# tudoroancea/ihm2

Measured on AMD Instinct MI355X. Metric: NMPC RTI solves/s (batch), N=40, nx=8 (6-DOF bicycle), fkin6, higher is better.
Workload: dtype f64

## Files before the change

ihm2_amd/csrc/api.hip:

```cpp
#include <hip/hip_runtime.h>

#include <algorithm>
#include <cmath>
#include <cstdarg>
#include <cstdio>
#include <cstdlib>
#include <cstring>
#include <memory>
#include <string>
#include <vector>

#include "ihm2mpc_internal.h"
#include "qp_catalogue.hpp"
#include "sqp_body.hpp"

static thread_local std::string g_err;

int ihm2_fail(const char *fmt, ...)
{
    char buf[512];
    va_list ap;
    va_start(ap, fmt);
    vsnprintf(buf, sizeof buf, fmt, ap);
    va_end(ap);
    g_err = buf;
    return -1;
}

namespace {

#define fail(...) ihm2_fail(__VA_ARGS__)

#define HIP_TRY(expr)                                                                          \
    do {                                                                                       \
        hipError_t e_ = (expr);                                                                \
        if (e_ != hipSuccess) return fail("%s failed: %s (%s:%d)", #expr, hipGetErrorString(e_), __FILE__, __LINE__); \
    } while (0)

#define CHECK_H(h)                                        \
    do {                                                  \
        if (!(h)) return fail("null handle");             \
        HIP_TRY(hipSetDevice((h)->cfg.device));           \
    } while (0)

int alloc_all() { return 0; }

template <typename T, typename... Rest>
int alloc_all(DevBuf<T> &b, size_t n, Rest &&...rest)
{
    HIP_TRY(b.alloc(n));
    if (alloc_all(rest...)) { b.reset(); return -1; }
    return 0;
}

int upload(ihm2mpc_handle *h, const double *host, double *dev, int elems)
{
    HIP_TRY(hipMemcpyAsync(dev, host, (size_t)h->B * elems * sizeof(double), hipMemcpyHostToDevice, h->stream));
    HIP_TRY(hipStreamSynchronize(h->stream));
    return 0;
}

int download(ihm2mpc_handle *h, const double *dev, double *host, int elems)
{
    HIP_TRY(hipMemcpyAsync(host, dev, (size_t)h->B * elems * sizeof(double), hipMemcpyDeviceToHost, h->stream));
    HIP_TRY(hipStreamSynchronize(h->stream));
    return 0;
}

int upload_shared(ihm2mpc_handle *h, const double *host, double *dev, size_t n)
{
    HIP_TRY(hipMemcpyAsync(dev, host, n * sizeof(double), hipMemcpyHostToDevice, h->stream));
    HIP_TRY(hipStreamSynchronize(h->stream));
    return 0;
}

const char *row_name(int c)
{
    static const char *names[NC] = {"lbx/ubx[0]", "lbx/ubx[1]", "lbx/ubx[2]", "lbx/ubx[3]", "lbx/ubx[4]", "lbx/ubx[5]", "lbx/ubx[6]", "lbx/ubx[7]",
                                    "lbu/ubu[0]", "lbu/ubu[1]", "lg/ug[0]", "lg/ug[1]", "lh/uh[0]", "lh/uh[1]"};
    return (c >= 0 && c < NC) ? names[c] : "?";
}

int check_instance_pattern(const ihm2mpc_handle *h, const double *il, const double *iu)
{
    const ihm2::PatternMismatch m = ihm2::find_pattern_mismatch(h->rows, h->B, il, iu);
    if (!m.found) return 0;
    return fail("instance %d, stage %d, row %d (%s): the finite sides (%s, %s) differ from the batch-shared table's (%s, %s)", m.b, m.k, m.c,
                row_name(m.c), m.lower ? "lower" : "-", m.upper ? "upper" : "-", m.shared_lower ? "lower" : "-", m.shared_upper ? "upper" : "-");
}

int scatter_instance_bounds(ihm2mpc_handle *h)
{
    const int B = h->B;
    h->inst_b_ok = false;
    if (check_instance_pattern(h, h->ih_lb.data(), h->ih_ub.data())) return -1;
    const size_t n = h->slots.entries();
    if ((size_t)B * n > h->i_slot_lb.size()) {
        HIP_TRY(hipStreamSynchronize(h->stream));
        h->i_slot_lb.reset(); h->i_slot_ub.reset();
        if (alloc_all(h->i_slot_lb, (size_t)B * n, h->i_slot_ub, (size_t)B * n)) return -1;
    }
    std::vector<double> slb, sub, stl, stu;
    ihm2::scatter_slot_bounds(h->slots, B, h->NS, h->ih_lb.data(), h->ih_ub.data(), slb, sub);
    ihm2::scatter_stage_bounds(h->rows, B, h->ih_lb.data(), h->ih_ub.data(), stl, stu);
    if (n && (upload_shared(h, slb.data(), h->i_slot_lb, slb.size()) || upload_shared(h, sub.data(), h->i_slot_ub, sub.size()))) return -1;
    if (upload_shared(h, stl.data(), h->i_st_lb, stl.size()) || upload_shared(h, stu.data(), h->i_st_ub, stu.size())) return -1;
    h->inst_b_ok = true;
    return 0;
}

const QpTable qp_catalogue[] = {ihm2_qp_set0(), ihm2_qp_set1(), ihm2_qp_set2(), ihm2_qp_set3(), ihm2_qp_set4(), ihm2_qp_set5(), ihm2_qp_set6()};

int path_class(const ihm2mpc_handle *h) { return h->rows.alat_on ? 2 : h->path_on ? 1 : 0; }

const QpInst *find_inst(const QpKey &want)
{
    for (const QpTable &t : qp_catalogue)
        for (const QpInst *e = t.inst; e < t.inst + t.n; e++) {
            const QpKey &k = e->key;
            if (k.kind == want.kind && k.nsoft == want.nsoft && k.path == want.path && k.uni == want.uni && k.sqp == want.sqp &&
                k.irk == want.irk && k.dyn == want.dyn && k.sens == want.sens && k.nf == want.nf && k.nslot >= want.nslot)
                return e;
        }
    return nullptr;
}

int factor_form(const ihm2mpc_handle *h)
{
    static const int limit = [] { const char *e = getenv("IHM2MPC_QP_FORM"); return (e && e[0] == '0') ? 0 : (e && e[0] == '1') ? 1 : 2; }();
    if (limit == 0 || h->cfg.model == IHM2MPC_MODEL_FDYN6 || h->slots.m_act == 0) return 0;
    return (h->N == 40 && limit == 2) ? 40 : -1;
}

const QpInst *find_form(const ihm2mpc_handle *h, QpKey want)
{
    for (int nf = factor_form(h); nf != 0; nf = (nf > 0) ? -1 : 0) {
        want.nf = nf;
        if (const QpInst *e = find_inst(want)) return e;
    }
    want.nf = 0;
    return find_inst(want);
}

ihm2::QpLds qp_layout(const ihm2mpc_handle *h) { return ihm2::qp_lds(h->N, ihm2::qp_lds_class(path_class(h), h->uniform_H && h->uniform_CD)); }
size_t qp_lds_bytes(const ihm2mpc_handle *h) { return sizeof(double) * (size_t)qp_layout(h).total; }
ihm2::StepsLds steps_lds(const ihm2mpc_handle *h, int sens)
{
    const bool dyn_rk4 = h->cfg.model != IHM2MPC_MODEL_FKIN6 && h->cfg.integrator_type == IHM2MPC_INTEG_ERK;
    return ihm2::steps_lds_doubles(qp_layout(h).total, sens ? (int)(ihm2_sens_lds_bytes(h) / sizeof(double)) : 0, dyn_rk4);
}

const QpInst *select_qp(const ihm2mpc_handle *h, size_t lds)
{
    if (lds > 160 * 1024) return nullptr;
    const int uni = h->uniform_H && h->uniform_CD;
    if (h->block_qp && !h->inst_b && h->slots.per_blk >= 1 && h->B <= h->n_cu && h->slots.per_lane * 64 <= (h->N + 1) * 12)
        if (const QpInst *e = find_inst({QP_BLOCK, h->slots.per_blk, h->slots.nsoft, path_class(h), uni, 0, 0, 0})) return e;
    return find_form(h, {QP_WAVE, h->slots.per_lane, h->slots.nsoft, path_class(h), uni, 0, 0, 0});
}

const QpInst *select_steps(const ihm2mpc_handle *h, int sens = 0)
{
    const ihm2::StepsLds lds = steps_lds(h, sens);
    const bool sqp = h->cfg.nlp_solver_type == IHM2MPC_SQP;
    const int irk = ihm2_is_irk(h->cfg.integrator_type) ? 1 : (h->cfg.integrator_type == IHM2MPC_INTEG_ERK_LAG) ? 2 : 0;
    const bool dyn = h->cfg.model != IHM2MPC_MODEL_FKIN6;
    if (irk == 1 && (!h->irk_tab || (sqp && h->sqp_globalization && !h->ls_phi))) return nullptr;
    if (h->cfg.sim_integrator_type == IHM2MPC_INTEG_ERK_LAG && irk != 2) return nullptr;
    if (sqp && !h->ls_x) return nullptr;
    if (lds.total() * sizeof(double) > 160 * 1024) return nullptr;
    if (!lds.guests_fit()) return nullptr;
    if (sqp && !ihm2::qp_sweeps_inside(qp_layout(h), h->N, false, 0, 0)) return nullptr;
    return find_form(h, {QP_STEPS, h->slots.per_lane, h->slots.nsoft, path_class(h), h->uniform_H && h->uniform_CD, sqp, irk, dyn, sens});
}

void note_launch(ihm2mpc_handle *h, const QpKey &k, int per_step = 0)
{
    int32_t *r = h->launch_rec;
    const int form = (k.nf > 0) ? 2 : (k.nf < 0) ? 1 : 0;
    if (k.kind != QP_STEPS) {
        r[0] = k.kind; r[1] = k.nslot; r[2] = k.nsoft; r[3] = k.path; r[4] = k.uni;
        r[15] = (r[15] & ~0x300) | (form << 8);
    } else {
        r[15] = (r[15] & ~0x3000) | ((per_step ? 0 : form) << 12);
        r[5] = per_step ? 2 : 1; r[6] = k.nslot; r[7] = k.nsoft; r[8] = k.path; r[9] = k.uni; r[10] = k.sqp; r[11] = k.irk; r[12] = k.dyn;
        r[13] = per_step; r[14] = k.sens;
    }
}

QpArgs qp_args(ihm2mpc_handle *h)
{
    QpArgs a;
    a.B = h->B; a.N = h->N; a.iter_max = h->cfg.ipm_iter_max; a.nslots = h->slots.per_lane * 64; a.m_act = h->slots.m_act;
    a.nslots_can = h->slots.per_lane * 64;
    a.tol = h->cfg.ipm_tol; a.mu0 = h->cfg.ipm_mu0; a.tau0 = h->cfg.ipm_tau0;
    a.Hs = h->Hs; a.Gy = h->Gy; a.CD = h->CD; a.slot_lb = h->slot_lb; a.slot_ub = h->slot_ub; a.slot_kc = h->slot_kc;
    a.hs_bs = 0; a.hs_te = h->N * 100; a.gy_bs = 0; a.gy_te = h->N * 120; a.sl_bs = 0;
    if (h->inst_w) { a.Hs = h->iHs; a.Gy = h->iGy; a.hs_bs = 200; a.hs_te = 100; a.gy_bs = 240; a.gy_te = 120; }
    if (h->inst_b) { a.sl_bs = h->slots.per_lane * 64; a.slot_lb = h->i_slot_lb; a.slot_ub = h->i_slot_ub; }
    a.x = h->x; a.u = h->u; a.x0 = h->x0; a.yref = h->yref; a.yref_e = h->yref_e;
    a.pi = h->pi; a.lam = h->lam; a.res = h->res; a.qp_res = h->qp_res; a.u0 = h->u0; a.status = h->status; a.qp_iter = h->qp_iter;
    a.lin = h->lin; a.g = h->q_g; a.rg = h->q_rg; a.P = h->q_P; a.M = h->q_M + (size_t)QM_PAD * 64;
    a.slot_zw = h->slot_zw; a.slot_Zw = h->slot_Zw; a.slk = h->slk;
    a.track_id = h->track_id; a.widths = h->widths; a.car_L = h->car_L; a.car_W = h->car_W;
    a.lam_a = h->lam_a; a.slk_a = h->slk_a;
    a.symmetrize = (h->cfg.model == IHM2MPC_MODEL_FDYN6) ? 1 : 0;
    return a;
}

void launch_inst(ihm2mpc_handle *h, const QpInst *e, void **args, size_t lds)
{
    (void)hipFuncSetAttribute(e->kernel, hipFuncAttributeMaxDynamicSharedMemorySize, (int)lds);
    (void)hipLaunchKernel(e->kernel, dim3(h->B), dim3(e->threads), args, lds, h->stream);
    note_launch(h, e->key);
}

int launch_qp(ihm2mpc_handle *h)
{
    const size_t lds = qp_lds_bytes(h);
    const QpInst *e = select_qp(h, lds);
    if (!e) return 1;
    QpArgs a = qp_args(h);
    if (e->key.kind == QP_BLOCK) { a.slot_kc = h->slot_kc_blk; a.slot_lb = h->slot_lb_blk; a.slot_ub = h->slot_ub_blk; a.nslots = h->slots.per_blk * 256; }
    void *args[] = {&a};
    launch_inst(h, e, args, lds);
    return 0;
}

int launch_steps(ihm2mpc_handle *h, int model, int M_sim, double s_target, int n_steps, int freeze, double lap_stop, int sens = 0)
{
    const size_t lds = sizeof(double) * (size_t)steps_lds(h, sens).total();
    const QpInst *e = select_steps(h, sens);
    if (!e) return 1;
    const bool irk_plant = ihm2_is_irk(h->cfg.sim_integrator_type);
    if (irk_plant && ihm2_upload_sim_irk_tab(h, M_sim)) return 1;
    const bool sqp = e->key.sqp;
    QpArgs a = qp_args(h);
    StepArgs s;
    s.ocp_model = h->cfg.model;
    s.n_steps = n_steps; s.model = model; s.M_sim = M_sim; s.M = h->cfg.M; s.nknots = h->cfg.nknots; s.lap_wrap = h->lap_wrap ? 1 : 0;
    s.freeze = freeze; s.s_target = s_target; s.dt = h->cfg.dt; s.lap_stop = lap_stop;
    s.sqp_iters = sqp ? (h->cfg.nlp_solver_max_iter > 0 ? h->cfg.nlp_solver_max_iter : 1) : 0;
    s.s_ref = h->s_ref; s.kappa_ref = h->kappa_ref;
    s.x0 = h->x0; s.yref = h->yref; s.yref_e = h->yref_e; s.lin = h->lin;
    s.active = (freeze || h->active_set) ? h->active.get() : nullptr;
    s.hist_u0 = h->hist_u0; s.hist_x0 = h->hist_x0; s.hist_st = h->hist_st; s.hist_it = h->hist_it;
    s.irk_tab = h->irk_tab;
    s.sim_irk_tab = irk_plant ? h->sim_irk_tab.get() : nullptr;
    s.sens = sens ? (const SensArgs *)h->sens_args.get() : nullptr;
    s.sim_lag = h->cfg.sim_integrator_type == IHM2MPC_INTEG_ERK_LAG;
    std::memset(s.lag, 0, sizeof s.lag);
    if (e->key.irk == 2) {
        const LagFac lo = ihm2_lag_factors(h->cfg.dt / h->cfg.M), lp = ihm2_lag_factors(h->cfg.dt / M_sim);
        std::memcpy(s.lag[0], lo.f, sizeof lo.f); std::memcpy(s.lag[1], lp.f, sizeof lp.f);
    }
    static_assert(sizeof(StepArgs) <= 48 * sizeof(double), "step_args holds 384 bytes");
    static_assert(sizeof(ihm2::LsArgs) <= 64 * sizeof(double), "ls_args holds 512 bytes");
    static_assert(sizeof(SensArgs) <= 64 * sizeof(double), "sens_args holds 512 bytes");
    const int slot = (h->args_idx++) & 1;
    if (hipEventSynchronize(h->args_ev[slot]) != hipSuccess) return 1;
    char *stage = (char *)h->args_host[slot];
    std::memcpy(stage, &s, sizeof(StepArgs));
    if (hipMemcpyAsync(h->step_args, stage, sizeof(StepArgs), hipMemcpyHostToDevice, h->stream) != hipSuccess) return 1;
    if (sqp) {
        ihm2::LsArgs ls_host = ihm2::make_ls_args(h);
        if (e->key.irk) ls_host.phase = 3;
        std::memcpy(stage + 512, &ls_host, sizeof(ihm2::LsArgs));
        if (hipMemcpyAsync(h->ls_args, stage + 512, sizeof(ihm2::LsArgs), hipMemcpyHostToDevice, h->stream) != hipSuccess) return 1;
    }
    if (sens) {
        SensArgs sa;
        ihm2_sens_args(h, &sa);
        sa.hist = h->hist_k; sa.sweep_step = n_steps - 1;
        std::memcpy(stage + 512, &sa, sizeof(SensArgs));
        if (hipMemcpyAsync(h->sens_args, stage + 512, sizeof(SensArgs), hipMemcpyHostToDevice, h->stream) != hipSuccess) return 1;
    }
    if (hipEventRecord(h->args_ev[slot], h->stream) != hipSuccess) return 1;
    const StepArgs *sdev = (const StepArgs *)h->step_args.get();
    const ihm2::LsArgs *ls = (const ihm2::LsArgs *)h->ls_args.get();
    void *args[] = {&sdev, &a, &ls};
    launch_inst(h, e, args, lds);
    return 0;
}

int sens_snapshot(ihm2mpc_handle *h)
{
    if (!h->sens_mode || h->sens_quiet) return 0;
    HIP_TRY(hipMemcpyAsync(h->sens_xbar, h->x, (size_t)h->B * h->NS * NX * sizeof(double), hipMemcpyDeviceToDevice, h->stream));
    HIP_TRY(hipMemcpyAsync(h->sens_ubar, h->u, (size_t)h->B * h->N * NU * sizeof(double), hipMemcpyDeviceToDevice, h->stream));
    return 0;
}

void sens_after_qp(ihm2mpc_handle *h)
{
    if (!h->sens_mode || h->sens_quiet) return;
    ihm2_launch_sens(h);
    h->sens_state = 1;
}

int sens_readable(const ihm2mpc_handle *h)
{
    if (!h->sens_mode) return fail("x0 sensitivities are off: ihm2mpc_set_x0_sensitivities(h, 1 or 2) before the solve");
    if (h->sens_state == 2)
        return fail("the last step came from ihm2mpc_run_steps, which computes no x0 sensitivities (the persistent loop is left as it is): "
                    "call ihm2mpc_run_steps_sens, ihm2mpc_solve, ihm2mpc_compute_control or ihm2mpc_step");
    if (h->sens_state != 1) return fail("no solve has run since x0 sensitivities were set to mode %d: nothing to read yet", h->sens_mode);
    return 0;
}

int ready(ihm2mpc_handle *h)
{
    if (!h->tracks_set) return fail("ihm2mpc_set_tracks has not been called");
    if (!h->weights_set) return fail("ihm2mpc_set_weights has not been called");
    if (!h->bounds_set) return fail("ihm2mpc_set_bounds has not been called");
    if (h->inst_w && !h->uniform_CD) return fail("per-instance weights need stage-independent general rows C, D (the QP keeps one copy of them)");
    if (h->inst_b && !h->inst_b_ok) return fail("the per-instance bounds do not fit the batch-shared constraint pattern any more: set them again, or pass NULL");
    if (!h->slots_fit) {
        std::string hard = "none", soft;
        for (const auto &[S, NSL] : ihm2::slot_limits(path_class(h)))
            if (S == 0) hard = std::to_string(NSL);
            else soft += (soft.empty() ? "" : " or ") + std::to_string(NSL) + " of which " + std::to_string(S) + " soft";
        static const char *rows[3] = {"without track rows", "with track rows", "with track rows and the lateral-acceleration row"};
        return fail("the constraint rows fit no QP kernel: %s a lane of 64 takes at most %s slots when all sides are hard; with soft sides, %s "
                    "(a two-sided hard row is one slot, a row with a soft side two; a lane's one-sided slots lead it)", rows[path_class(h)],
                    hard.c_str(), soft.empty() ? "none" : soft.c_str());
    }
    if (h->rows.alat_on) {
        if (h->cfg.model != IHM2MPC_MODEL_FKIN6) return fail("the lateral-acceleration row is a row of the kinematic model (old/generate_acaods_interface.py:206: `[] if is_dynamic else [a_lat]`)");
        if (!h->path_on) return fail("the lateral-acceleration row comes with the track rows: enable ihm2mpc_set_path_constraints first");
        if (h->cfg.nlp_solver_type != IHM2MPC_SQP_RTI) return fail("the lateral-acceleration row is implemented for SQP_RTI (old/generate.py:21)");
        if (!(h->uniform_H && h->uniform_CD)) return fail("the lateral-acceleration row needs stage-independent weights and general rows (the reference's OCP has them)");
    }
    return 0;
}

struct FieldInfo { double *base; int per_stage; int nstages; };

int field_info(ihm2mpc_handle *h, const char *field, FieldInfo *fi)
{
    const std::string f(field ? field : "");
    if (f == "x") *fi = {h->x, NX, h->NS};
    else if (f == "u") *fi = {h->u, NU, h->N};
    else if (f == "yref") *fi = {h->yref, NY, h->N};
    else if (f == "yref_e") *fi = {h->yref_e, NX, 1};
    else if (f == "pi") *fi = {h->pi, NX, h->NS};
    else if (f == "lam") *fi = {h->lam, NLAM, h->NS};
    else if (f == "lbx" || f == "ubx" || f == "x0") *fi = {h->x0, NX, 1};
    else return fail("unknown field '%s'", f.c_str());
    return 0;
}

}

ihm2mpc_handle::~ihm2mpc_handle()
{
    for (hipStream_t s : {stream, stream2}) if (s) (void)hipStreamSynchronize(s);
    (void)ihm2mpc_comm_free(this);
    for (hipEvent_t e : {ev_fork, ev_join, ev[0], ev[1], ev[2], ev[3], args_ev[0], args_ev[1]}) if (e) (void)hipEventDestroy(e);
    for (void *p : args_host) if (p) (void)hipHostFree(p);
    for (hipStream_t s : {stream, stream2}) if (s) (void)hipStreamDestroy(s);
}

static bool rk4_unstable(double dt, int M) { return dt / M / 1e-3 >= 2.78; }
static int check_sim_substeps(const ihm2mpc_handle *h, int M_sim, const char *lags)
{
    if (M_sim < 1) return fail("M_sim must be >= 1");
    if (h->cfg.sim_integrator_type == IHM2MPC_INTEG_ERK && rk4_unstable(h->cfg.dt, M_sim))
        return fail("RK4 with M_sim = %d sub-steps of dt = %g is unstable on the %s: use M_sim >= %d", M_sim, h->cfg.dt, lags,
                    (int)ceil(h->cfg.dt / (2.78 * 1e-3)));
    return 0;
}
static int check_plant(const ihm2mpc_handle *h, int model, int M_sim)
{
    if (check_sim_substeps(h, M_sim, "actuator lags")) return -1;
    if (model < -2 || model > IHM2MPC_MODEL_FDYN6U) return fail("unknown plant model %d", model);
    if (h->cfg.sim_integrator_type != IHM2MPC_INTEG_ERK_LAG || model == IHM2MPC_MODEL_FKIN6) return 0;
    return fail("the plant integrator ERK_LAG (closed-form actuator lags) is implemented for the kinematic plant (model 0) only, not for plant "
                "model %d: create the handle with another sim_integrator_type", model);
}

extern "C" {

const char *ihm2mpc_last_error(void) { return g_err.c_str(); }
const char *ihm2mpc_version(void) { return "ihm2mpc 0.1 (gfx950)"; }

int ihm2mpc_lag_stage_factors(double h, double tau, double *out4)
{
    if (!out4) return fail("null argument");
    if (!(h > 0.0) || !(tau > 0.0) || !std::isfinite(h) || !std::isfinite(tau)) return fail("h and tau must be positive and finite");
    const double r = h / tau, e = exp(-r);
    double p1, p2;
    if (r < 1.0) {
        p1 = 0.0; p2 = 0.0;
        double t = 0.5;
        for (int k = 2; k < 40; k++) {
            p1 += ((k & 1) ? -1.0 : 1.0) * (k - 1) * t;
            if (k >= 3) p2 += ((k & 1) ? 1.0 : -1.0) * (double)((k - 1) * (k - 2)) * t / r;
            t *= r / (k + 1);
        }
    } else {
        p1 = (1.0 - e * (1.0 + r)) / (r * r);
        p2 = 2.0 * (1.0 - e * (1.0 + r + 0.5 * r * r)) / (r * r * r);
    }
    const double E1 = 6.0 * (p1 - p2), E2 = 12.0 * p2 - 6.0 * p1;
    out4[0] = 6.0 * (-expm1(-r) / r) - 4.0 * E1 - E2;
    out4[1] = E1;
    out4[2] = E2;
    out4[3] = e;
    return 0;
}

int ihm2mpc_create(const ihm2mpc_config *cfg, ihm2mpc_handle **out)
{
    if (!cfg || !out) return fail("null argument");
    if (cfg->batch < 1) return fail("batch must be >= 1");
    if (cfg->N < 2 || cfg->N > IHM2MPC_NMAX) return fail("N must be in [2, %d]", IHM2MPC_NMAX);
    if (cfg->M < 1) return fail("M must be >= 1");
    if (cfg->integrator_type < IHM2MPC_INTEG_ERK || cfg->integrator_type > IHM2MPC_INTEG_ERK_LAG || cfg->sim_integrator_type < IHM2MPC_INTEG_ERK ||
        cfg->sim_integrator_type > IHM2MPC_INTEG_ERK_LAG)
        return fail("unknown integrator type (%d, %d)", cfg->integrator_type, cfg->sim_integrator_type);
    if (cfg->integrator_type == IHM2MPC_INTEG_ERK_LAG && cfg->model != IHM2MPC_MODEL_FKIN6)
        return fail("the integrator ERK_LAG (closed-form actuator lags) is implemented for the kinematic OCP model IHM2MPC_MODEL_FKIN6 only, not for "
                    "the dynamic models (model %d): use ERK or IRK", cfg->model);
    if (cfg->integrator_type == IHM2MPC_INTEG_ERK_LAG && cfg->nlp_solver_type != IHM2MPC_SQP_RTI)
        return fail("the integrator ERK_LAG (closed-form actuator lags) is implemented for IHM2MPC_SQP_RTI only: the SQP mode's line-search "
                    "rollouts have no such integrator; use ERK or IRK");
    if (ihm2_is_irk(cfg->integrator_type) && cfg->M != 1)
        return fail("the IRK integrator of the shooting intervals takes one step per interval (sim_method_num_steps = 1, python/main.py:236); M = %d", cfg->M);
    if (cfg->integrator_type == IHM2MPC_INTEG_ERK && rk4_unstable(cfg->dt, cfg->M))
        return fail("RK4 with %d sub-step(s) of dt = %g is unstable on the actuator lags (t_T = 1e-3 s, t_delta = 0.02 s: |z| = dt / (M t) must stay "
                    "below 2.78): use M >= %d (the reference's sim_method_num_steps = 1 belongs to its IRK integrator, python/main.py:234-236)",
                    cfg->M, cfg->dt, (int)ceil(cfg->dt / (2.78 * 1e-3)));
    if (cfg->model < IHM2MPC_MODEL_FKIN6 || cfg->model > IHM2MPC_MODEL_FDYN6U) return fail("unknown OCP model %d", cfg->model);
    if (cfg->ntracks < 1 || cfg->nknots < 2) return fail("need at least one track table with >= 2 knots");
    if (!(cfg->dt > 0.0)) return fail("dt must be positive");
    int ndev = 0;
    HIP_TRY(hipGetDeviceCount(&ndev));
    if (cfg->device < 0 || cfg->device >= ndev) return fail("device %d out of range (%d devices)", cfg->device, ndev);
    HIP_TRY(hipSetDevice(cfg->device));
    hipDeviceProp_t prop;
    HIP_TRY(hipGetDeviceProperties(&prop, cfg->device));
    if (strncmp(prop.gcnArchName, "gfx950", 6) != 0)
        return fail("libihm2mpc is built for gfx950 (MI355X) only; device %d is %s", cfg->device, prop.gcnArchName);

    auto h = std::make_unique<ihm2mpc_handle>();
    h->cfg = *cfg;
    h->B = cfg->batch;
    h->N = cfg->N;
    h->NS = cfg->N + 1;
    h->n_cu = prop.multiProcessorCount;
    { const char *e = getenv("IHM2MPC_BLOCK_QP"); h->block_qp = !(e && e[0] == '0'); }
    const size_t B = h->B, N = h->N, NS = h->NS, nt = (size_t)cfg->ntracks * cfg->nknots;
    HIP_TRY(hipStreamCreateWithFlags(&h->stream, hipStreamNonBlocking));
    HIP_TRY(hipStreamCreateWithFlags(&h->stream2, hipStreamNonBlocking));
    HIP_TRY(hipEventCreateWithFlags(&h->ev_fork, hipEventDisableTiming));
    HIP_TRY(hipEventCreateWithFlags(&h->ev_join, hipEventDisableTiming));
    for (int i = 0; i < 4; i++) HIP_TRY(hipEventCreate(&h->ev[i]));
    for (int i = 0; i < 2; i++) {
        HIP_TRY(hipHostMalloc(&h->args_host[i], 1024, hipHostMallocDefault));
        HIP_TRY(hipEventCreateWithFlags(&h->args_ev[i], hipEventDisableTiming));
    }
    if (alloc_all(h->s_ref, nt, h->kappa_ref, nt, h->track_id, B, h->Hs, NS * 100, h->Gy, NS * 120, h->lbx, NS * 8, h->ubx, NS * 8,
                  h->lbu, N * 2, h->ubu, N * 2, h->CD, N * 20, h->lg, N * 2, h->ug, N * 2, h->slot_kc_blk, 1024, h->slot_lb_blk, 1024,
                  h->slot_ub_blk, 1024, h->slot_kc, MAX_SLOTS, h->slot_lb, MAX_SLOTS, h->slot_ub, MAX_SLOTS, h->slot_zw, MAX_SLOTS,
                  h->slot_Zw, MAX_SLOTS, h->slk, B * NS * NLAM, h->widths, (size_t)cfg->ntracks * 2, h->lam_a, B * NS * 2, h->slk_a, B * NS * 2,
                  h->X_ref, nt, h->Y_ref, nt, h->phi_ref, nt, h->xc, B * 8, h->s_guess, B, h->step_args, 48, h->Wd, N * 144 + 64,
                  h->st_lb, NS * NC, h->st_ub, NS * NC, h->st_sz, NS * NLAM, h->st_sZ, NS * NLAM, h->x, B * NS * 8, h->u, B * N * 2, h->x0, B * 8,
                  h->yref, B * N * 12, h->yref_e, B * 8, h->pi, B * NS * 8, h->lam, B * NS * NLAM, h->res, B * 4, h->qp_res, B * 4, h->status, B,
                  h->qp_iter, B, h->active, B, h->u0, B * 2,
                  h->lin, (B * N + B) * LIN_REC,
                  h->q_g, B * NS * 10, h->q_rg, B * NS * 10, h->q_P, B * NS * 64, h->q_M, (B * N + 2 * QM_PAD) * 64, h->scratch, B * 24))
        return -1;
    h->slots_fit = true;
    h->sqp_globalization = 0; h->sqp_use_suff = 0; h->sqp_full_step_dual = 0;
    h->sqp_alpha_min = 0.05; h->sqp_alpha_red = 0.7; h->sqp_eps = 1e-4;
    for (int i = 0; i < 4; i++) h->sqp_tol[i] = cfg->nlp_tol;
    h->rows = ihm2::ConstraintRows((int)NS);
    if (ihm2_upload_irk_tab(h.get())) return fail("could not upload the collocation tableau");
    *out = h.release();
    return 0;
}

int ihm2mpc_free(ihm2mpc_handle *h)
{
    if (!h) return 0;
    (void)hipSetDevice(h->cfg.device);
    delete h;
    return 0;
}

int ihm2mpc_synchronize(ihm2mpc_handle *h)
{
    CHECK_H(h);
    HIP_TRY(hipStreamSynchronize(h->stream));
    return 0;
}

int ihm2mpc_get_stream(ihm2mpc_handle *h, void **stream)
{
    CHECK_H(h);
    if (!stream) return fail("null argument");
    *stream = (void *)h->stream;
    return 0;
}

int ihm2mpc_set_tracks(ihm2mpc_handle *h, const double *s_ref, const double *kappa_ref)
{
    CHECK_H(h);
    if (!s_ref || !kappa_ref) return fail("null argument");
    const size_t n = (size_t)h->cfg.ntracks * h->cfg.nknots;
    for (int t = 0; t < h->cfg.ntracks; t++)
        for (int i = 1; i < h->cfg.nknots; i++)
            if (!(s_ref[(size_t)t * h->cfg.nknots + i] > s_ref[(size_t)t * h->cfg.nknots + i - 1]))
                return fail("s_ref of track %d is not strictly increasing at knot %d", t, i);
    if (upload_shared(h, s_ref, h->s_ref, n) || upload_shared(h, kappa_ref, h->kappa_ref, n)) return -1;
    h->tracks_set = true;
    return 0;
}

int ihm2mpc_build_tracks(ihm2mpc_handle *h, int32_t max_seg, const int32_t *nseg, const double *coeffs_X, const double *coeffs_Y)
{
    CHECK_H(h);
    if (!nseg || !coeffs_X || !coeffs_Y) return fail("null argument");
    if (h->cfg.nknots % 3 != 0) return fail("nknots = %d is not three laps of samples", h->cfg.nknots);
    if (max_seg < 2) return fail("max_seg must be >= 2");
    for (int t = 0; t < h->cfg.ntracks; t++)
        if (nseg[t] < 2 || nseg[t] > max_seg) return fail("track %d has %d spline segments (2 .. max_seg = %d)", t, nseg[t], max_seg);
    const size_t nc = (size_t)h->cfg.ntracks * max_seg;
    DevBuf<double> dev;
    DevBuf<int32_t> dseg;
    HIP_TRY(dev.alloc(nc * 9));
    if (dseg.alloc(h->cfg.ntracks) != hipSuccess) return fail("out of device memory");
    double *cX = dev, *cY = dev + nc * 4, *work = dev + nc * 8;
    if (hipMemcpyAsync(cX, coeffs_X, nc * 4 * sizeof(double), hipMemcpyHostToDevice, h->stream) != hipSuccess ||
        hipMemcpyAsync(cY, coeffs_Y, nc * 4 * sizeof(double), hipMemcpyHostToDevice, h->stream) != hipSuccess ||
        hipMemcpyAsync(dseg, nseg, h->cfg.ntracks * sizeof(int32_t), hipMemcpyHostToDevice, h->stream) != hipSuccess) return fail("upload of the spline coefficients failed");
    ihm2_launch_build_tracks(h, max_seg, dseg, cX, cY, work);
    if (hipGetLastError() != hipSuccess || hipStreamSynchronize(h->stream) != hipSuccess) return fail("track-table kernels failed");
    h->tracks_set = true; h->geometry_set = true;
    return 0;
}

int ihm2mpc_fit_tracks(ihm2mpc_handle *h, int32_t max_pts, const int32_t *npts, const double *xy, double curv_weight, double *coeffs_X, double *coeffs_Y)
{
    CHECK_H(h);
    if (!npts || !xy || !coeffs_X || !coeffs_Y) return fail("null argument");
    if (!(curv_weight >= 0.0)) return fail("curv_weight must be >= 0");
    if (max_pts < 3 || 7 * max_pts + 2 > 1280) return fail("max_pts must be in 3 .. 182 (the elimination lists the non-zeros of a row in LDS)");
    const int nt = h->cfg.ntracks;
    for (int t = 0; t < nt; t++)
        if (npts[t] < 3 || npts[t] > max_pts) return fail("track %d has %d centre-line points (3 .. max_pts = %d)", t, npts[t], max_pts);
    const size_t m = 7 * (size_t)max_pts, nwork = (size_t)nt * m * (m + 2), nxy = (size_t)nt * max_pts * 2, nc = (size_t)nt * max_pts * 4;
    DevBuf<double> dev;
    DevBuf<int32_t> di;
    HIP_TRY(dev.alloc(nwork + nxy + 2 * nc));
    if (di.alloc(2 * (size_t)nt) != hipSuccess) return fail("out of device memory");
    double *work = dev, *dxy = dev + nwork, *cX = dxy + nxy, *cY = cX + nc;
    std::vector<int32_t> flags(nt, 1);
    if (hipMemcpyAsync(dxy, xy, nxy * sizeof(double), hipMemcpyHostToDevice, h->stream) != hipSuccess ||
        hipMemcpyAsync(di, npts, nt * sizeof(int32_t), hipMemcpyHostToDevice, h->stream) != hipSuccess) return fail("upload of the centre lines failed");
    ihm2_launch_track_fit(h, max_pts, di, dxy, curv_weight, work, cX, cY, di + nt);
    if (hipGetLastError() != hipSuccess ||
        hipMemcpyAsync(coeffs_X, cX, nc * sizeof(double), hipMemcpyDeviceToHost, h->stream) != hipSuccess ||
        hipMemcpyAsync(coeffs_Y, cY, nc * sizeof(double), hipMemcpyDeviceToHost, h->stream) != hipSuccess ||
        hipMemcpyAsync(flags.data(), di + nt, nt * sizeof(int32_t), hipMemcpyDeviceToHost, h->stream) != hipSuccess ||
        hipStreamSynchronize(h->stream) != hipSuccess) return fail("spline-fit kernel failed");
    for (int t = 0; t < nt; t++)
        if (flags[t]) return fail("the spline fit of track %d is singular (coincident centre-line points?)", t);
    return 0;
}

int ihm2mpc_get_tracks(ihm2mpc_handle *h, double *s_ref, double *kappa_ref, double *X_ref, double *Y_ref, double *phi_ref)
{
    CHECK_H(h);
    if (!h->tracks_set) return fail("no track tables yet");
    const size_t n = (size_t)h->cfg.ntracks * h->cfg.nknots * sizeof(double);
    const double *src[5] = {h->s_ref, h->kappa_ref, h->X_ref, h->Y_ref, h->phi_ref};
    double *dst[5] = {s_ref, kappa_ref, X_ref, Y_ref, phi_ref};
    for (int i = 0; i < 5; i++)
        if (dst[i]) {
            if (i >= 2 && !h->geometry_set) return fail("ihm2mpc_set_track_geometry / ihm2mpc_build_tracks has not been called");
            HIP_TRY(hipMemcpyAsync(dst[i], src[i], n, hipMemcpyDeviceToHost, h->stream));
        }
    HIP_TRY(hipStreamSynchronize(h->stream));
    return 0;
}

int ihm2mpc_set_track_id(ihm2mpc_handle *h, const int32_t *track_id)
{
    CHECK_H(h);
    if (!track_id) return fail("null argument");
    for (int b = 0; b < h->B; b++)
        if (track_id[b] < 0 || track_id[b] >= h->cfg.ntracks) return fail("track_id[%d] = %d out of range", b, track_id[b]);
    HIP_TRY(hipMemcpyAsync(h->track_id, track_id, (size_t)h->B * sizeof(int32_t), hipMemcpyHostToDevice, h->stream));
    HIP_TRY(hipStreamSynchronize(h->stream));
    return 0;
}

int ihm2mpc_set_weights(ihm2mpc_handle *h, const double *W, const double *W_e)
{
    CHECK_H(h);
    if (!W || !W_e) return fail("null argument");
    const int N = h->N, NS = h->NS;
    std::vector<double> Hs((size_t)NS * 100, 0.0), Gy((size_t)NS * 120, 0.0);
    const double cs = h->cfg.cost_scale_stage;
    for (int k = 0; k < N; k++) ihm2::stage_weight_tables(W + (size_t)k * NY * NY, cs, &Hs[(size_t)k * 100], &Gy[(size_t)k * 120]);
    ihm2::terminal_weight_tables(W_e, &Hs[(size_t)N * 100], &Gy[(size_t)N * 120]);
    for (int k = 0; k < NS; k++)
        if (!ihm2::symmetric10(&Hs[(size_t)k * 100])) return fail("weight matrix of stage %d is not symmetric", k);
    const bool uni = ihm2::stages_equal(Hs.data(), N, 100) && ihm2::stages_equal(Gy.data(), N, 120);
    if (upload_shared(h, Hs.data(), h->Hs, Hs.size()) || upload_shared(h, Gy.data(), h->Gy, Gy.size())) return -1;
    if (upload_shared(h, W, h->Wd, (size_t)N * 144) || upload_shared(h, W_e, h->Wd + (size_t)N * 144, 64)) return -1;
    h->shared_uniform_H = uni;
    h->uniform_H = h->inst_w || uni;
    h->weights_set = true;
    return 0;
}

int ihm2mpc_set_instance_weights(ihm2mpc_handle *h, const double *W, const double *W_e)
{
    CHECK_H(h);
    if (!W && !W_e) {
        h->iHs.reset(); h->iGy.reset(); h->iWd.reset();
        h->inst_w = false;
        h->uniform_H = h->shared_uniform_H;
        return 0;
    }
    if (!W || !W_e) return fail("W and W_e must both be given, or both be NULL (batch-shared weights again)");
    if (!h->weights_set) return fail("ihm2mpc_set_weights has not been called (the batch-shared weights come first)");
    if (h->bounds_set && !h->uniform_CD) return fail("per-instance weights need stage-independent general rows C, D");
    const int B = h->B;
    std::vector<double> Hs((size_t)B * 200, 0.0), Gy((size_t)B * 240, 0.0), Wd((size_t)B * 208);
    const double cs = h->cfg.cost_scale_stage;
    for (int b = 0; b < B; b++) {
        const double *Wb = W + (size_t)b * 144, *Web = W_e + (size_t)b * 64;
        for (int i = 0; i < 144; i++) if (Wb[i] != Wb[i]) return fail("instance %d: W[%d][%d] is NaN", b, i / 12, i % 12);
        for (int i = 0; i < 64; i++) if (Web[i] != Web[i]) return fail("instance %d: W_e[%d][%d] is NaN", b, i / 8, i % 8);
        double *Hb = &Hs[(size_t)b * 200], *Gb = &Gy[(size_t)b * 240];
        ihm2::stage_weight_tables(Wb, cs, Hb, Gb);
        ihm2::terminal_weight_tables(Web, Hb + 100, Gb + 120);
        if (!ihm2::symmetric10(Hb)) return fail("instance %d: the weight matrix of the stages 0..%d is not symmetric", b, h->N - 1);
        if (!ihm2::symmetric10(Hb + 100)) return fail("instance %d: the weight matrix of stage %d (terminal) is not symmetric", b, h->N);
        std::memcpy(&Wd[(size_t)b * 208], Wb, 144 * sizeof(double));
        std::memcpy(&Wd[(size_t)b * 208 + 144], Web, 64 * sizeof(double));
    }
    if (!h->iHs && alloc_all(h->iHs, (size_t)B * 200, h->iGy, (size_t)B * 240, h->iWd, (size_t)B * 208)) return -1;
    if (upload_shared(h, Hs.data(), h->iHs, Hs.size()) || upload_shared(h, Gy.data(), h->iGy, Gy.size()) ||
        upload_shared(h, Wd.data(), h->iWd, Wd.size()))
        return -1;
    h->inst_w = true;
    h->uniform_H = true;
    return 0;
}

static int rebuild_slots(ihm2mpc_handle *h)
{
    ihm2::SlotTable t = ihm2::lay_out_slots(h->rows, ihm2::slot_limits(path_class(h)));
    h->slots_fit = t.fit;
    if (!t.fit) return 0;
    h->slots = std::move(t);
    const ihm2::SlotTable &s = h->slots;
    const ihm2::ConstraintRows &r = h->rows;
    if (s.per_blk) {
        HIP_TRY(hipMemcpyAsync(h->slot_kc_blk, s.kc_blk.data(), s.kc_blk.size() * sizeof(int32_t), hipMemcpyHostToDevice, h->stream));
        HIP_TRY(hipStreamSynchronize(h->stream));
        if (upload_shared(h, s.lb_blk.data(), h->slot_lb_blk, s.lb_blk.size()) || upload_shared(h, s.ub_blk.data(), h->slot_ub_blk, s.ub_blk.size())) return -1;
    }
    if (upload_shared(h, r.lb.data(), h->st_lb, r.lb.size()) || upload_shared(h, r.ub.data(), h->st_ub, r.ub.size()) ||
        upload_shared(h, r.sz.data(), h->st_sz, r.sz.size()) || upload_shared(h, r.sZ.data(), h->st_sZ, r.sZ.size()))
        return -1;
    if (const size_t n = s.entries()) {
        HIP_TRY(hipMemcpyAsync(h->slot_kc, s.kc.data(), n * sizeof(int32_t), hipMemcpyHostToDevice, h->stream));
        HIP_TRY(hipStreamSynchronize(h->stream));
        if (upload_shared(h, s.lb.data(), h->slot_lb, n) || upload_shared(h, s.ub.data(), h->slot_ub, n) ||
            upload_shared(h, s.zw.data(), h->slot_zw, n) || upload_shared(h, s.Zw.data(), h->slot_Zw, n))
            return -1;
    }
    if (h->inst_b) return scatter_instance_bounds(h);
    return 0;
}

int ihm2mpc_set_bounds(ihm2mpc_handle *h, const double *lbx, const double *ubx, const double *lbu, const double *ubu,
                       const double *C, const double *D, const double *lg, const double *ug)
{
    CHECK_H(h);
    if (!lbx || !ubx || !lbu || !ubu || !C || !D || !lg || !ug) return fail("null argument");
    const int N = h->N, NS = h->NS;
    for (int i = 0; i < NS * NX; i++) if (lbx[i] > ubx[i]) return fail("lbx > ubx at flat index %d", i);
    for (int i = 0; i < N * NU; i++) if (lbu[i] > ubu[i]) return fail("lbu > ubu at flat index %d", i);
    for (int i = 0; i < N * NG; i++) if (lg[i] > ug[i]) return fail("lg > ug at flat index %d", i);
    std::vector<double> CD((size_t)N * 20);
    for (int k = 0; k < N; k++)
        for (int r = 0; r < NG; r++) {
            for (int j = 0; j < NX; j++) CD[((size_t)k * 2 + r) * 10 + j] = C[((size_t)k * 2 + r) * NX + j];
            for (int j = 0; j < NU; j++) CD[((size_t)k * 2 + r) * 10 + 8 + j] = D[((size_t)k * 2 + r) * NU + j];
        }
    h->uniform_CD = ihm2::stages_equal(CD.data(), N, 20);
    h->rows.set_box_rows(lbx, ubx, lbu, ubu, lg, ug);
    if (rebuild_slots(h)) return -1;
    if (upload_shared(h, lbx, h->lbx, (size_t)NS * 8) || upload_shared(h, ubx, h->ubx, (size_t)NS * 8) ||
        upload_shared(h, lbu, h->lbu, (size_t)N * 2) || upload_shared(h, ubu, h->ubu, (size_t)N * 2) ||
        upload_shared(h, CD.data(), h->CD, CD.size()) || upload_shared(h, lg, h->lg, (size_t)N * 2) ||
        upload_shared(h, ug, h->ug, (size_t)N * 2))
        return -1;
    h->bounds_set = true;
    return 0;
}

int ihm2mpc_set_instance_bounds(ihm2mpc_handle *h, const double *lbx, const double *ubx, const double *lbu, const double *ubu,
                                const double *lg, const double *ug)
{
    CHECK_H(h);
    const bool none = !lbx && !ubx && !lbu && !ubu && !lg && !ug;
    if (none) {
        h->i_slot_lb.reset(); h->i_slot_ub.reset(); h->i_st_lb.reset(); h->i_st_ub.reset();
        h->i_lbu.reset(); h->i_ubu.reset(); h->i_lg.reset(); h->i_ug.reset();
        h->ih_lb = std::vector<double>(); h->ih_ub = std::vector<double>();
        h->inst_b = false; h->inst_b_ok = false;
        return 0;
    }
    if (!lbx || !ubx || !lbu || !ubu || !lg || !ug) return fail("lbx, ubx, lbu, ubu, lg, ug must all be given, or all be NULL (batch-shared bounds again)");
    if (!h->bounds_set) return fail("ihm2mpc_set_bounds has not been called (the batch-shared table gives the pattern)");
    const int B = h->B, N = h->N, NS = h->NS;
    std::vector<double> il((size_t)B * NS * 12), iu((size_t)B * NS * 12);
    for (int b = 0; b < B; b++) {
        const double *xl = lbx + (size_t)b * NS * 8, *xu = ubx + (size_t)b * NS * 8, *ul = lbu + (size_t)b * N * 2, *uu = ubu + (size_t)b * N * 2;
        const double *gl = lg + (size_t)b * N * 2, *gu = ug + (size_t)b * N * 2;
        for (int k = 0; k < NS; k++)
            for (int c = 0; c < 12; c++) {
                const auto [lb, ub] = ihm2::box_row(N, k, c, xl, xu, ul, uu, gl, gu);
                if (lb != lb || ub != ub) return fail("instance %d, stage %d, row %d (%s): bound is NaN", b, k, c, row_name(c));
                if (lb > ub) return fail("instance %d, stage %d, row %d (%s): lower bound %g > upper bound %g", b, k, c, row_name(c), lb, ub);
            }
        ihm2::box_rows(N, xl, xu, ul, uu, gl, gu, &il[(size_t)b * NS * 12], &iu[(size_t)b * NS * 12], 12);
    }
    if (check_instance_pattern(h, il.data(), iu.data())) return -1;
    const size_t nb = (size_t)B;
    if (!h->i_st_lb && alloc_all(h->i_st_lb, nb * NS * NC, h->i_st_ub, nb * NS * NC, h->i_lbu, nb * N * 2, h->i_ubu, nb * N * 2,
                                 h->i_lg, nb * N * 2, h->i_ug, nb * N * 2))
        return -1;
    h->ih_lb = std::move(il); h->ih_ub = std::move(iu);
    if (upload_shared(h, lbu, h->i_lbu, (size_t)B * N * 2) || upload_shared(h, ubu, h->i_ubu, (size_t)B * N * 2) ||
        upload_shared(h, lg, h->i_lg, (size_t)B * N * 2) || upload_shared(h, ug, h->i_ug, (size_t)B * N * 2))
        return -1;
    h->inst_b = true;
    if (scatter_instance_bounds(h)) return -1;
    return 0;
}

int ihm2mpc_set_soft(ihm2mpc_handle *h, const double *soft_z, const double *soft_Z)
{
    CHECK_H(h);
    const int n = h->NS * NLAM;
    if ((soft_z == nullptr) != (soft_Z == nullptr)) return fail("soft_z and soft_Z must both be given or both be NULL");
    for (int i = 0; i < n; i++) {
        const double Z = soft_Z ? soft_Z[i] : -1.0, z = soft_z ? soft_z[i] : 0.0;
        if (Z >= 0.0 && !(z >= 0.0)) return fail("soft_z < 0 at flat index %d (the slack penalty must be non-decreasing)", i);
        if (Z >= 0.0 && !(Z + z > 0.0)) return fail("soft side %d has neither a linear nor a quadratic penalty", i);
        h->rows.sz[i] = z; h->rows.sZ[i] = Z;
    }
    HIP_TRY(hipMemsetAsync(h->slk, 0, (size_t)h->B * h->NS * NLAM * sizeof(double), h->stream));
    if (h->bounds_set && rebuild_slots(h)) return -1;
    return 0;
}

int ihm2mpc_set_path_constraints(ihm2mpc_handle *h, int32_t enable, double car_length, double car_width, const double *widths,
                                 const double *lh, const double *uh)
{
    CHECK_H(h);
    if (enable) {
        if (!widths || !lh || !uh) return fail("null argument");
        if (!(car_length >= 0.0) || !(car_width >= 0.0)) return fail("car_length and car_width must be non-negative");
        for (int i = 0; i < NH; i++) if (lh[i] > uh[i]) return fail("lh > uh at row %d", i);
        for (int t = 0; t < h->cfg.ntracks * 2; t++) if (!(widths[t] > 0.0)) return fail("track width %d is not positive", t);
        if (upload_shared(h, widths, h->widths, (size_t)h->cfg.ntracks * 2)) return -1;
        h->car_L = car_length; h->car_W = car_width;
    }
    h->path_on = enable ? 1 : 0;
    h->rows.set_track_rows(enable != 0, lh, uh);
    if (h->bounds_set && rebuild_slots(h)) return -1;
    return 0;
}

int ihm2mpc_set_alat_constraint(ihm2mpc_handle *h, int32_t enable, double a_lat_min, double a_lat_max, const double *soft_z, const double *soft_Z)
{
    CHECK_H(h);
    if (enable) {
        if (a_lat_min != a_lat_min || a_lat_max != a_lat_max) return fail("a_lat bound is not a number");
        if (a_lat_min > a_lat_max) return fail("a_lat_min > a_lat_max");
        for (int i = 0; i < 2; i++) {
            const double z = soft_z ? soft_z[i] : 0.0, Z = soft_Z ? soft_Z[i] : -1.0;
            if (z != z || Z != Z) return fail("soft penalty of the a_lat row is not a number");
            if (Z >= 0.0 && !(z >= 0.0)) return fail("soft_z < 0 on the a_lat row (the slack penalty must be non-decreasing)");
            if (Z >= 0.0 && !(Z + z > 0.0)) return fail("a soft side of the a_lat row has neither a linear nor a quadratic penalty");
            h->rows.alat_sz[i] = z; h->rows.alat_sZ[i] = Z;
        }
        h->rows.alat_lb = ihm2::bound_or(a_lat_min, -INFINITY);
        h->rows.alat_ub = ihm2::bound_or(a_lat_max, INFINITY);
    }
    h->rows.alat_on = enable ? 1 : 0;
    HIP_TRY(hipMemsetAsync(h->lam_a, 0, (size_t)h->B * h->NS * 2 * sizeof(double), h->stream));
    HIP_TRY(hipMemsetAsync(h->slk_a, 0, (size_t)h->B * h->NS * 2 * sizeof(double), h->stream));
    if (h->bounds_set && rebuild_slots(h)) return -1;
    return 0;
}

int ihm2mpc_set_alat_multipliers(ihm2mpc_handle *h, const double *lam, const double *slk)
{
    CHECK_H(h);
    if (lam) { if (upload(h, lam, h->lam_a, h->NS * 2)) return -1; }
    else HIP_TRY(hipMemsetAsync(h->lam_a, 0, (size_t)h->B * h->NS * 2 * sizeof(double), h->stream));
    if (slk) { if (upload(h, slk, h->slk_a, h->NS * 2)) return -1; }
    else HIP_TRY(hipMemsetAsync(h->slk_a, 0, (size_t)h->B * h->NS * 2 * sizeof(double), h->stream));
    return 0;
}

int ihm2mpc_get_alat_multipliers(ihm2mpc_handle *h, double *lam, double *slk)
{
    CHECK_H(h);
    if (lam && download(h, h->lam_a, lam, h->NS * 2)) return -1;
    if (slk && download(h, h->slk_a, slk, h->NS * 2)) return -1;
    return 0;
}

#define SETTER(name, field, elems)                                   \
    int ihm2mpc_set_##name(ihm2mpc_handle *h, const double *v)       \
    {                                                                \
        CHECK_H(h);                                                  \
        if (!v) return fail("null argument");                        \
        return upload(h, v, h->field, (elems));                      \
    }
SETTER(x0, x0, NX)
SETTER(x, x, h->NS * NX)
SETTER(u, u, h->N * NU)
SETTER(yref, yref, h->N * NY)
SETTER(yref_e, yref_e, NX)
#undef SETTER

int ihm2mpc_set_multipliers(ihm2mpc_handle *h, const double *pi, const double *lam)
{
    CHECK_H(h);
    if (pi) { if (upload(h, pi, h->pi, h->NS * NX)) return -1; }
    else HIP_TRY(hipMemsetAsync(h->pi, 0, (size_t)h->B * h->NS * NX * sizeof(double), h->stream));
    if (lam) { if (upload(h, lam, h->lam, h->NS * NLAM)) return -1; }
    else {
        HIP_TRY(hipMemsetAsync(h->lam, 0, (size_t)h->B * h->NS * NLAM * sizeof(double), h->stream));
        HIP_TRY(hipMemsetAsync(h->lam_a, 0, (size_t)h->B * h->NS * 2 * sizeof(double), h->stream));
    }
    return 0;
}

int ihm2mpc_set_slacks(ihm2mpc_handle *h, const double *sl)
{
    CHECK_H(h);
    if (sl) return upload(h, sl, h->slk, h->NS * NLAM);
    HIP_TRY(hipMemsetAsync(h->slk, 0, (size_t)h->B * h->NS * NLAM * sizeof(double), h->stream));
    HIP_TRY(hipMemsetAsync(h->slk_a, 0, (size_t)h->B * h->NS * 2 * sizeof(double), h->stream));
    return 0;
}

int ihm2mpc_set_stage(ihm2mpc_handle *h, int32_t instance, int32_t stage, const char *field, const double *value, int32_t n)
{
    CHECK_H(h);
    FieldInfo fi;
    if (field_info(h, field, &fi)) return -1;
    if (!value) return fail("null argument");
    if (instance < 0 || instance >= h->B) return fail("instance %d out of range", instance);
    const std::string f(field);
    if ((f == "lbx" || f == "ubx") && stage != 0)
        return fail("per-instance '%s' exists at stage 0 only (the initial state); stage bounds are shared: ihm2mpc_set_bounds", field);
    if (f == "yref_e") stage = 0;
// ... 634 lines not shown
```

ihm2_amd/csrc/ihm2mpc_internal.h:

```cpp
#pragma once

#include <hip/hip_runtime.h>
#include <stdint.h>

#include <vector>

#include "../../include/ihm2mpc.h"
#include "ihm2_dims.h"

#pragma clang fp contract(fast)

#include "qp_tables.hpp"

#define QM_PAD 24
#define LIN_REC 96

static inline bool ihm2_is_irk(int type) { return type == IHM2MPC_INTEG_IRK_GL4 || type == IHM2MPC_INTEG_IRK_RADAU4; }
struct LagFac { double f[8]; };
LagFac ihm2_lag_factors(double h);

struct ihm2mpc_comm;
namespace ihm2 { struct IrkTab; }

template <typename T>
class DevBuf {
public:
    DevBuf() = default;
    DevBuf(const DevBuf &) = delete;
    DevBuf &operator=(const DevBuf &) = delete;
    ~DevBuf() { reset(); }
    hipError_t alloc(size_t n)
    {
        reset();
        void *q = nullptr;
        hipError_t e = hipMalloc(&q, n * sizeof(T));
        if (e == hipSuccess) e = hipMemset(q, 0, n * sizeof(T));
        if (e == hipSuccess) e = hipStreamSynchronize(nullptr);
        if (e != hipSuccess) { (void)hipFree(q); return e; }
        p_ = (T *)q; n_ = n;
        return hipSuccess;
    }
    void reset()
    {
        if (p_) (void)hipFree(p_);
        p_ = nullptr; n_ = 0;
    }
    size_t size() const { return n_; }
    T *get() const { return p_; }
    operator T *() const { return p_; }
private:
    T *p_ = nullptr;
    size_t n_ = 0;
};

struct ihm2mpc_handle {
    ~ihm2mpc_handle();

    ihm2mpc_config cfg;
    ihm2mpc_comm *comm;
    int B, N, NS;
    int n_cu;
    hipStream_t stream;
    hipStream_t stream2;
    hipEvent_t ev_fork, ev_join;
    hipEvent_t ev[4];
    bool tracks_set, weights_set, bounds_set;
    bool uniform_H, uniform_CD;

    DevBuf<double> s_ref, kappa_ref;
    DevBuf<int32_t> track_id;
    DevBuf<double> Hs;
    DevBuf<double> Gy;
    DevBuf<double> lbx, ubx;
    DevBuf<double> lbu, ubu;
    DevBuf<double> CD;
    DevBuf<double> lg, ug;
    ihm2::ConstraintRows rows;
    ihm2::SlotTable slots;
    bool slots_fit;
    DevBuf<int32_t> slot_kc;
    DevBuf<double> slot_lb, slot_ub;
    DevBuf<double> slot_zw, slot_Zw;
    DevBuf<int32_t> slot_kc_blk;
    DevBuf<double> slot_lb_blk, slot_ub_blk;
    bool block_qp;
    int path_on;
    double car_L, car_W, lh[NH], uh[NH];
    DevBuf<double> widths;
    bool geometry_set;
    DevBuf<double> X_ref, Y_ref, phi_ref;
    DevBuf<double> xc;
    DevBuf<double> s_guess;

    DevBuf<double> x;
    DevBuf<double> u;
    DevBuf<double> x0;
    DevBuf<double> yref;
    DevBuf<double> yref_e;
    DevBuf<double> pi;
    DevBuf<double> lam;
    DevBuf<double> slk;
    DevBuf<double> lam_a, slk_a;
    DevBuf<double> res;
    DevBuf<double> ls_phi;
    DevBuf<ihm2::IrkTab> irk_tab;
    DevBuf<ihm2::IrkTab> sim_irk_tab;
    int sim_irk_M;
    DevBuf<double> dyn10;
    DevBuf<double> qp_res;
    DevBuf<int32_t> status, qp_iter;
    DevBuf<int32_t> active;
    bool active_set;
    bool freeze_armed;
    bool lap_wrap;
    DevBuf<double> u0;

    DevBuf<double> lin;
    DevBuf<double> q_g;
    DevBuf<double> q_rg;
    DevBuf<double> q_P;
    DevBuf<double> q_M;
    DevBuf<double> scratch;

    int sqp_globalization, sqp_use_suff, sqp_full_step_dual;
    double sqp_alpha_min, sqp_alpha_red, sqp_eps, sqp_tol[4];
    DevBuf<double> Wd;
    DevBuf<double> st_lb, st_ub;
    DevBuf<double> st_sz, st_sZ;
    DevBuf<double> ls_x, ls_u, ls_pi, ls_lam, ls_slk, ls_wpi, ls_wlam, ls_alpha;
    DevBuf<int32_t> ls_done, ls_status, ls_iter, ls_qp_acc;
    DevBuf<int32_t> ls_pending;
    DevBuf<double> ls_args;
    DevBuf<double> step_args;
    void *args_host[2];
    hipEvent_t args_ev[2];
    int args_idx;

    bool inst_w, inst_b;
    bool inst_b_ok;
    bool shared_uniform_H;
    DevBuf<double> iHs, iGy, iWd;
    std::vector<double> ih_lb, ih_ub;
    DevBuf<double> i_slot_lb, i_slot_ub;
    DevBuf<double> i_st_lb, i_st_ub;
    DevBuf<double> i_lbu, i_ubu, i_lg, i_ug;

    DevBuf<double> hist_u0, hist_x0;
    DevBuf<int32_t> hist_st, hist_it;

    int32_t launch_rec[16];

    int sens_mode;
    int sens_state;
    bool sens_quiet;
    DevBuf<double> sens_xbar, sens_ubar;
    DevBuf<double> sens_u0;
    DevBuf<double> sens_args;
    DevBuf<double> sens_x, sens_u;
    DevBuf<double> hist_k;

    DevBuf<double> adj_sx, adj_su;
    DevBuf<double> adj_gx0, adj_gy, adj_gye;
    DevBuf<double> adj_gW, adj_gWe;
};

void ihm2_launch_prepare(ihm2mpc_handle *h, double s_target, int mode, hipStream_t stream);
void ihm2_launch_build_tracks(ihm2mpc_handle *h, int max_seg, const int32_t *nseg, const double *cX, const double *cY, double *work);
void ihm2_launch_track_fit(ihm2mpc_handle *h, int max_pts, const int32_t *npts, const double *xy, double curv_weight, double *work, double *cX, double *cY,
                           int32_t *fail_flag);
void ihm2_launch_sim_dyn10(ihm2mpc_handle *h, int M, const double *x, const double *u, double *xn, hipStream_t stream);
void ihm2_launch_sim_dyn10_irk(ihm2mpc_handle *h, int integ, int M, int newton_iter, const double *x, const double *u, double *xn, hipStream_t stream);
void ihm2_launch_wrap_lap(ihm2mpc_handle *h);
void ihm2_launch_init_guess(ihm2mpc_handle *h, double v_ref_scale, int only_failed);
void ihm2_launch_linearize(ihm2mpc_handle *h);
void ihm2_launch_linearize_irk(ihm2mpc_handle *h);
int ihm2_upload_sim_irk_tab(ihm2mpc_handle *h, int M_sim);
int ihm2_upload_irk_tab(ihm2mpc_handle *h);
void ihm2_launch_rollout_irk(ihm2mpc_handle *h, int j_begin, int j_end, double *phi, const int32_t *pending);
void ihm2_launch_sim_irk(ihm2mpc_handle *h, int model, int M_sim, const double *x, const double *u, double *xn, hipStream_t stream,
                         const int32_t *active);
void ihm2_launch_copy_iterate(ihm2mpc_handle *h);
void ihm2_launch_line_search(ihm2mpc_handle *h, int it, int last, int phase = 0, int j_limit = 0);
void ihm2_launch_sim(ihm2mpc_handle *h, int model, int M_sim, const double *x, const double *u, double *xn, hipStream_t stream,
                     const int32_t *active);
void ihm2_launch_sim_cart(ihm2mpc_handle *h, int model, int M, double dt, int n_steps, double v_dyn, const double *x, const double *u,
                          double *xn, hipStream_t stream);
void ihm2_launch_project(ihm2mpc_handle *h, double s_tol, const double *xc, double *s_guess, double *xf, hipStream_t stream);
void ihm2_launch_sens(ihm2mpc_handle *h);
size_t ihm2_sens_lds_bytes(const ihm2mpc_handle *h);
void ihm2_launch_adj(ihm2mpc_handle *h, int n_seeds, const double *seed_x, const double *seed_u, int unit_u0, int weights);

namespace {

struct QpArgs {
    int B, N, iter_max, nslots, m_act;
    int nslots_can;
    double tol, mu0, tau0;
    const double *Hs, *Gy, *CD, *slot_lb, *slot_ub, *slot_zw, *slot_Zw;
    const int32_t *slot_kc;
    int hs_bs, hs_te, gy_bs, gy_te, sl_bs;
    double *x, *u;
    const double *x0, *yref, *yref_e;
    double *pi, *lam, *res, *qp_res, *u0;
    int32_t *status, *qp_iter;
    const double *lin;
    double *g, *rg, *P, *M, *slk;
    const int32_t *track_id;
    const double *widths;
    double car_L, car_W;
    double *lam_a, *slk_a;
    int symmetrize;
};

struct SensArgs {
    int B, N, mode, nslots, path, alat;
    double tau;
    const double *Hs;
    int hs_bs, hs_te, hs_ks;
    const double *CD;
    const int32_t *slot_kc;
    const double *slot_lb, *slot_ub, *slot_zw, *slot_Zw;
    int sl_bs;
    const int32_t *track_id;
    const double *widths;
    double car_L, car_W;
    const double *lin, *xbar, *ubar, *x, *u, *lam, *slk, *lam_a, *slk_a;
    const int32_t *status;
    double *sens_u0, *sens_x, *sens_u;
    double *hist;
    int sweep_step;
};

struct StepArgs {
    int n_steps, model, M_sim, M, nknots, lap_wrap, freeze;
    int ocp_model;
    int sqp_iters;
    double s_target, dt, lap_stop;
    const double *s_ref, *kappa_ref;
    double *x0, *yref, *yref_e, *lin;
    int32_t *active;
    double *hist_u0, *hist_x0;
    int32_t *hist_st, *hist_it;
    const ihm2::IrkTab *irk_tab;
    const ihm2::IrkTab *sim_irk_tab;
    const SensArgs *sens;
    double lag[2][8];
    int sim_lag;
};

}

void ihm2_sens_args(const ihm2mpc_handle *h, void *out);

enum { QP_WAVE = 1, QP_BLOCK = 2, QP_STEPS = 3 };
struct QpKey { int kind, nslot, nsoft, path, uni, sqp, irk, dyn, sens, nf; };
struct QpInst { QpKey key; int threads; const void *kernel; };
struct QpTable { const QpInst *inst; int n; };
QpTable ihm2_qp_set0(), ihm2_qp_set1(), ihm2_qp_set2(), ihm2_qp_set3(), ihm2_qp_set4(), ihm2_qp_set5(), ihm2_qp_set6();
```

ihm2_amd/csrc/kernels_qp.hip:

```cpp
#include <cstring>

#include "ihm2mpc_internal.h"
#include "device_steps.hpp"
#include "sqp_body.hpp"
#include "irk_body.hpp"
#include "riccati_mfma.hpp"
#include "sens_body.hpp"
#include "qp_lds.hpp"
#include "qp_catalogue.hpp"
#include "wave_sync.hpp"

using namespace ihm2;

namespace {

#define INF_BOUND 1e20
#ifndef RIC_RING
#define RIC_RING 4
#endif
#ifndef SWEEP_RING
#define SWEEP_RING 4
#endif
#define SWEEP_DL ((SWEEP_RING >= 8) ? 4 : 2)

__device__ __forceinline__ bool fin(double v) { return fabs(v) < INF_BOUND; }

template <typename OP>
__device__ __forceinline__ double wave_reduce(double v, OP op)
{
    v = op(v, dpp_mov<0xB1>(v));
    v = op(v, dpp_mov<0x4E>(v));
    v = op(v, dpp_mov<0x141>(v));
    v = op(v, dpp_mov<0x128>(v));
    int lo = __double2loint(v), hi = __double2hiint(v);
    auto a16 = __builtin_amdgcn_permlane16_swap(lo, lo, false, false);
    auto b16 = __builtin_amdgcn_permlane16_swap(hi, hi, false, false);
    v = op(__hiloint2double(b16[0], a16[0]), __hiloint2double(b16[1], a16[1]));
    lo = __double2loint(v); hi = __double2hiint(v);
    auto a32 = __builtin_amdgcn_permlane32_swap(lo, lo, false, false);
    auto b32 = __builtin_amdgcn_permlane32_swap(hi, hi, false, false);
    return op(__hiloint2double(b32[0], a32[0]), __hiloint2double(b32[1], a32[1]));
}
__device__ __forceinline__ double nanmax(double a, double b) { return (a != a || b != b) ? NAN : fmax(a, b); }
__device__ __forceinline__ double wave_max(double v) { return wave_reduce(v, [](double a, double b) { return fmax(a, b); }); }
__device__ __forceinline__ double wave_min(double v) { return wave_reduce(v, [](double a, double b) { return fmin(a, b); }); }
__device__ __forceinline__ double wave_sum(double v) { return wave_reduce(v, [](double a, double b) { return a + b; }); }
__device__ __forceinline__ double wave_nanmax(double v) { return wave_reduce(v, [](double a, double b) { return nanmax(a, b); }); }

__device__ __forceinline__ double sum8(double v)
{
    v += dpp_mov<0xB1>(v);
    v += dpp_mov<0x4E>(v);
    v += dpp_mov<0x141>(v);
    return v;
}

__device__ __forceinline__ double sum_stride8(double v)
{
    v += dpp_mov<0x128>(v);
    int lo = __double2loint(v), hi = __double2hiint(v);
    auto a16 = __builtin_amdgcn_permlane16_swap(lo, lo, false, false);
    auto b16 = __builtin_amdgcn_permlane16_swap(hi, hi, false, false);
    v = __hiloint2double(b16[0], a16[0]) + __hiloint2double(b16[1], a16[1]);
    lo = __double2loint(v); hi = __double2hiint(v);
    auto a32 = __builtin_amdgcn_permlane32_swap(lo, lo, false, false);
    auto b32 = __builtin_amdgcn_permlane32_swap(hi, hi, false, false);
    return __hiloint2double(b32[0], a32[0]) + __hiloint2double(b32[1], a32[1]);
}

template <int DIR, int D, int DL, bool BUF = true, typename P, typename F>
__device__ __forceinline__ void stream_rows(const double *rows, int N, int e_even, int e_odd, P &&pre, F &&body)
{
    static_assert(D % 2 == 0 && DL % 2 == 0 && D % DL == 0 && 3 * D <= QM_PAD, "the element index alternates with the step parity");
    double r[2][D], x0[DL], x1[DL];
    const __amdgpu_buffer_rsrc_t rsrc = __builtin_amdgcn_make_buffer_rsrc(const_cast<double *>(rows) - (size_t)QM_PAD * 64, 0, (N + 2 * QM_PAD) * 512, 0x00020000);
    const unsigned ve = (unsigned)e_even * 8u, vo = (unsigned)e_odd * 8u;
    typedef unsigned int u2_t __attribute__((ext_vector_type(2)));
    const double *p_even = rows + (size_t)((DIR < 0) ? N - 1 : 0) * 64 + e_even, *p_odd = rows + (size_t)((DIR < 0) ? N - 1 : 0) * 64 + e_odd;
    auto load_row = [&](const int step, const bool odd) -> double {
        if constexpr (BUF) {
            const int row = (DIR < 0) ? N - 1 - step : step;
            const u2_t v = __builtin_amdgcn_raw_buffer_load_b64(rsrc, odd ? vo : ve, (QM_PAD + row) * 512, 0);
            return __hiloint2double((int)v.y, (int)v.x);
        } else
            return (odd ? p_odd : p_even)[(ptrdiff_t)DIR * step * 64];
    };
#pragma unroll
    for (int d = 0; d < D; d++) {
        r[0][d] = load_row(d, (d & 1) != 0);
        __builtin_amdgcn_sched_barrier(0);
        if (d < DL) pre((DIR < 0) ? N - 1 - d : d, (d & 1) != 0, x0[d], x1[d]);
    }
    for (int s0 = 0; s0 < N; s0 += 2 * D) {
#pragma unroll
        for (int h = 0; h < 2; h++) {
#pragma unroll
            for (int d = 0; d < D; d++) {
                const int s = s0 + h * D + d;
                const int k = (DIR < 0) ? N - 1 - s : s;
                const double v = r[h][d], y0 = x0[d % DL], y1 = x1[d % DL];
                r[h ^ 1][d] = load_row(s + D, (d & 1) != 0);
                pre((DIR < 0) ? k - DL : k + DL, (d & 1) != 0, x0[d % DL], x1[d % DL]);
                if (s < N) body(k, v, (d & 1) != 0, y0, y1);
            }
        }
    }
}
template <int DIR, int D, int DL, typename P, typename F>
__device__ __forceinline__ void stream_rows_v1(const double *rows, int N, int e_even, int e_odd, P &&pre, F &&body)
{
    stream_rows<DIR, D, DL, false>(rows, N, e_even, e_odd, pre, body);
}

template <int NSLOT, int NSOFT, int PATH, int UNI, int NW = 1, int LEAN = 1, int NF = 0>
__device__ __forceinline__ void qp_wave_body(const QpArgs &a, const int b, double *sm, const bool want_res = true)
{
    static_assert(NF == 0 || NW == 1, "the straight-line factor sweep parks its idle lanes' stores in the tile the block reductions use");
    constexpr int NT = 64 * NW;
    const int tid = threadIdx.x, lane = tid & 63, wv = tid >> 6;
#define BSYNC() do { if (NW == 1) WSYNC(); else __syncthreads(); } while (0)
    const int N = (NF > 0) ? NF : a.N, NS = N + 1;
    constexpr QpLdsClass CLS = qp_lds_class(PATH, UNI != 0);
    constexpr int NCK = CLS.nck;
    const double *Hs0 = a.Hs + (size_t)b * a.hs_bs, *HsT = Hs0 + a.hs_te;
    const double *Gy0 = a.Gy + (size_t)b * a.gy_bs, *GyT = Gy0 + a.gy_te;
    const double *slot_lbb = a.slot_lb + (size_t)b * a.sl_bs, *slot_ubb = a.slot_ub + (size_t)b * a.sl_bs;
    constexpr bool ALAT = PATH == 2;
    constexpr bool HL = CLS.hl, CL = CLS.cl;
    static_assert(qp_factor_inside(qp_lds(40, CLS), 40, NCK) && qp_factor_inside(qp_lds(2, CLS), 2, NCK), "factor stage / block reductions leave their LDS");
    static_assert(qp_sweeps_inside(qp_lds(40, CLS), 40, LEAN != 0, SWEEP_RING, SWEEP_DL) && (LEAN == 0 || qp_sweeps_inside(qp_lds(2, CLS), 2, true, SWEEP_RING, SWEEP_DL)),
                  "the sweeps' unclamped LDS prefetch leaves the block (the earlier form does below N = 4: api.hip refuses those launches)");
    static_assert(NW <= 4, "qp_factor_inside checks the block reductions for four waves");
#define LEN(id) qp_lds_len(id, N, NS, CLS)
    double *z = sm, *gt = z + LEN(QP_Z), *pi = gt + LEN(QP_GT), *pv = pi + LEN(QP_PI), *rb = pv + LEN(QP_PV), *gam = rb + LEN(QP_RB), *cf = gam + LEN(QP_GAM), *dz = cf + LEN(QP_CF);
    double *kff = dz + LEN(QP_DZ), *Kl = kff + LEN(QP_KFF), *Ginv = Kl + LEN(QP_KL), *Prb = Ginv + LEN(QP_GINV), *tile = Prb + LEN(QP_PRB), *hc = tile + LEN(QP_TILE), *ha = hc + LEN(QP_HC);
    double *Hl = ha + LEN(QP_HA), *CDl = Hl + LEN(QP_HL), *spv = CDl + LEN(QP_CDL);
    int *spc = reinterpret_cast<int *>(spv + 60);
#undef LEN
#define HS(k, i, l) (HL ? Hl[(((k) == N) ? 100 : 0) + (i) * 10 + (l)] : ((k) == N ? HsT : Hs0 + (UNI ? 0 : (k)) * 100)[(i) * 10 + (l)])
#define CDV(k, r, j) (CL ? CDl[(r) * 10 + (j)] : a.CD[((k) * 2 + (r)) * 10 + (j)])

    auto blk_reduce = [&](double v, auto op) -> double {
        v = wave_reduce(v, op);
        if (NW > 1) {
            __syncthreads();
            if (lane == 0) tile[wv] = v;
            __syncthreads();
            v = tile[0];
#pragma unroll
            for (int w = 1; w < NW; w++) v = op(v, tile[w]);
        }
        return v;
    };
    auto blk_max = [&](double v) { return blk_reduce(v, [](double x, double y) { return fmax(x, y); }); };
    auto blk_min = [&](double v) { return blk_reduce(v, [](double x, double y) { return fmin(x, y); }); };
    auto blk_sum = [&](double v) { return blk_reduce(v, [](double x, double y) { return x + y; }); };
    auto blk_nanmax = [&](double v) { return blk_reduce(v, [](double x, double y) { return nanmax(x, y); }); };

    const double *xb = a.x + (size_t)b * NS * 8;
    const double *ub = a.u + (size_t)b * N * 2;
    const double *linb = a.lin + (size_t)b * N * LIN_REC;
    double *gb = a.g + (size_t)b * NS * 10;
    double *rgb = a.rg + (size_t)b * NS * 10;
    double *Pg = a.P + (size_t)b * NS * 64;
    double *Mg = a.M + (size_t)b * N * 64;
    double *pib = a.pi + (size_t)b * NS * 8;
    double *lamb = a.lam + (size_t)b * NS * 28;
    double *slkb = a.slk + (size_t)b * NS * 28;
    double *lamab = ALAT ? a.lam_a + (size_t)b * NS * 2 : nullptr;
    double *slkab = ALAT ? a.slk_a + (size_t)b * NS * 2 : nullptr;
    auto alat_slot = [](int j) -> int { return (j == 3) ? 0 : (j == 4) ? 1 : (j == 6) ? 2 : (j == 7) ? 3 : -1; };

    if (HL) for (int e = tid; e < 200; e += NT) Hl[e] = (e < 100) ? Hs0[e] : HsT[e - 100];
    if (CL && tid < 20) CDl[tid] = a.CD[tid];
    if (UNI) BSYNC();
    bool h_sparse = false;
    if (HL) {
        int cnt = 0;
        if (tid < 20) {
#pragma unroll
            for (int l = 0; l < 10; l++) {
                const double v = Hl[tid * 10 + l];
                if (v != 0.0) { if (cnt < 3) { spv[tid * 3 + cnt] = v; spc[tid * 3 + cnt] = l; } cnt++; }
            }
            for (int q = cnt; q < 3; q++) { spv[tid * 3 + q] = 0.0; spc[tid * 3 + q] = 0; }
        }
        h_sparse = __ballot(cnt > 3) == 0ull;
        if (NW > 1) h_sparse = blk_max((wv == 0 && !h_sparse) ? 1.0 : 0.0) == 0.0;
        BSYNC();
    }
    double sg = 1.0, sb = 1.0, r_stat = 0.0, r_eq = 0.0;
    double w_R = 0.0, w_L = 0.0;
    if (PATH) {
        const int trk = a.track_id[b];
        w_R = a.widths[trk * 2 + 0]; w_L = a.widths[trk * 2 + 1];
        for (int k = tid; k < NS; k += NT) {
            const double psi = xb[k * 8 + 2], sgn = (psi > 0.0) - (psi < 0.0);
            const double dfoot = -0.5 * a.car_L * cos(fabs(psi)) * sgn, dlat = -0.5 * a.car_W * sin(psi);
            hc[k * 2 + 0] = (k >= 1) ? dfoot + dlat : 0.0;
            hc[k * 2 + 1] = (k >= 1) ? -dfoot + dlat : 0.0;
            if (ALAT) {
                double g4[4];
                alat_eval(xb[k * 8 + 3], xb[k * 8 + 4], xb[k * 8 + 6], xb[k * 8 + 7], g4);
#pragma unroll
                for (int q = 0; q < 4; q++) ha[k * 4 + q] = (k >= 1 && k < N) ? g4[q] : 0.0;
            }
        }
        BSYNC();
    }
    for (int e = tid; e < NS * 10; e += NT) {
        const int k = e / 10, j = e % 10;
        double acc = 0.0;
#pragma unroll
        for (int l = 0; l < 8; l++) acc = fma(HS(k, j, l), xb[k * 8 + l], acc);
        if (k < N) {
            acc = fma(HS(k, j, 8), ub[k * 2 + 0], acc);
            acc = fma(HS(k, j, 9), ub[k * 2 + 1], acc);
            const double *yr = a.yref + ((size_t)b * N + k) * 12;
#pragma unroll
            for (int l = 0; l < 12; l++) acc = fma(-Gy0[((UNI ? 0 : k) * 10 + j) * 12 + l], yr[l], acc);
        } else {
            const double *yr = a.yref_e + (size_t)b * 8;
#pragma unroll
            for (int l = 0; l < 8; l++) acc = fma(-GyT[j * 12 + l], yr[l], acc);
        }
        gb[e] = acc;
        const bool counted = !((k == 0 && j < 8) || (k == N && j >= 8));
        if (j < 8 || k < N) sg = fmax(sg, fabs(acc));
        if (!want_res) continue;
        double st = acc;
        if (k < N) {
            const double *rec = linb + (size_t)k * LIN_REC;
#pragma unroll
            for (int l = 0; l < 8; l++) st = fma((j < 8) ? rec[l * 8 + j] : rec[64 + l * 2 + (j - 8)], pib[(k + 1) * 8 + l], st);
        }
        if (j < 8) st -= pib[k * 8 + j];
        st -= lamb[k * 28 + j] - lamb[k * 28 + 14 + j];
        if (k < N) {
            st = fma(-CDV(k, 0, j), lamb[k * 28 + 10] - lamb[k * 28 + 24], st);
            st = fma(-CDV(k, 1, j), lamb[k * 28 + 11] - lamb[k * 28 + 25], st);
        }
        if (PATH && (j == 1 || j == 2)) {
            const double l12 = lamb[k * 28 + 12] - lamb[k * 28 + 26], l13 = lamb[k * 28 + 13] - lamb[k * 28 + 27];
            st -= (j == 1) ? l12 - l13 : hc[k * 2] * l12 + hc[k * 2 + 1] * l13;
        }
        if (ALAT && alat_slot(j) >= 0) st -= ha[k * 4 + alat_slot(j)] * (lamab[k * 2] - lamab[k * 2 + 1]);
        if (counted) r_stat = fmax(r_stat, fabs(st));
    }
    for (int e = tid; e < N * 8; e += NT) {
        const double bl = linb[(size_t)(e / 8) * LIN_REC + 80 + (e % 8)];
        sb = fmax(sb, fabs(bl));
        r_eq = fmax(r_eq, fabs(bl));
    }
    if (tid < 8) {
        const double d = a.x0[(size_t)b * 8 + tid] - xb[tid];
        sb = fmax(sb, fabs(d));
        r_eq = fmax(r_eq, fabs(d));
    }
    sg = blk_max(sg); sb = blk_max(sb);

    int s_kc[NSLOT];
    double s_dl[NSLOT], s_du[NSLOT];
    double lam_l[NSLOT], lam_u[NSLOT], t_l[NSLOT], t_u[NSLOT];
    constexpr int NSO = (NSOFT > 0) ? NSOFT : 1;
    double so_zw[NSO], so_Zw[NSO], so_s[NSO], so_ls[NSO], so_rs[NSO], so_ds[NSO], so_dls[NSO], so_pa[NSO];
#pragma unroll
    for (int r = 0; r < NSO; r++) { so_zw[r] = 0.0; so_Zw[r] = -1.0; so_s[r] = 1.0; so_ls[r] = 0.0; so_rs[r] = 0.0; so_ds[r] = so_dls[r] = so_pa[r] = 0.0; }
#define IS_SOFT(r) ((r) < NSOFT && so_Zw[(r) < NSOFT ? (r) : 0] >= 0.0)
#define ONE_SIDED(r) (NSOFT > 0 && PATH != 2 && (r) < NSOFT)
#define HAS_L(r) (ONE_SIDED(r) ? true : fin(s_dl[r]))
#define HAS_U(r) (ONE_SIDED(r) ? false : fin(s_du[r]))
#define ROW_DOT(r, v) (ONE_SIDED(r) ? s_sg[(r) < NSOFT ? (r) : 0] * row_dot(s_kc[r], (v)) : row_dot(s_kc[r], (v)))
#define ROW_SIGN(r, c) (ONE_SIDED(r) ? s_sg[(r) < NSOFT ? (r) : 0] * (c) : (c))
    double s_sg[NSO];
#pragma unroll
    for (int r = 0; r < NSO; r++) s_sg[r] = 1.0;
#define SLOT_ACC(dst, v) do { if (NSOFT > 0) (dst) += (v); else (dst) = (v); } while (0)
    double r_ineq = 0.0, r_comp = 0.0;
#pragma unroll
    for (int r = 0; r < NSLOT; r++) {
        const int s = tid + NT * r;
        s_kc[r] = -1; s_dl[r] = -INFINITY; s_du[r] = INFINITY;
        lam_l[r] = lam_u[r] = 0.0; t_l[r] = t_u[r] = 1.0;
        const int kc = (s < a.nslots) ? a.slot_kc[s] : -1;
        if (kc >= 0) {
            const int k = kc >> 4, c = kc & 15;
            s_kc[r] = k * NCK + c;
            double cz;
            if (c < 8) cz = xb[k * 8 + c];
            else if (c < 10) cz = ub[k * 2 + c - 8];
            else if (ALAT && c == 14) {
                double g4[4];
                cz = alat_eval(xb[k * 8 + 3], xb[k * 8 + 4], xb[k * 8 + 6], xb[k * 8 + 7], g4);
            } else if (c >= 12) {
                const double n = xb[k * 8 + 1], psi = xb[k * 8 + 2];
                const double foot = -0.5 * a.car_L * sin(fabs(psi)), lat = 0.5 * a.car_W * cos(psi);
                cz = (c == 12) ? n + foot + lat - w_R : -n - foot + lat - w_L;
            } else {
                cz = 0.0;
#pragma unroll
                for (int j = 0; j < 8; j++) cz = fma(CDV(k, c - 10, j), xb[k * 8 + j], cz);
                cz = fma(CDV(k, c - 10, 8), ub[k * 2 + 0], cz);
                cz = fma(CDV(k, c - 10, 9), ub[k * 2 + 1], cz);
            }
            const double lb = slot_lbb[s], ubd = slot_ubb[s];
            bool soft = false;
            if (r < NSOFT) { so_zw[r < NSOFT ? r : 0] = a.slot_zw[s]; so_Zw[r < NSOFT ? r : 0] = a.slot_Zw[s]; soft = a.slot_Zw[s] >= 0.0; }
#define LAM_IN(up) ((ALAT && c == 14) ? lamab[k * 2 + (up)] : lamb[k * 28 + 14 * (up) + c])
            if (fin(lb)) { s_dl[r] = lb - cz; if (want_res && !soft) { r_ineq = fmax(r_ineq, s_dl[r]); r_comp = fmax(r_comp, fabs(LAM_IN(0) * s_dl[r])); } }
            if (fin(ubd)) { s_du[r] = ubd - cz; if (want_res && !soft) { r_ineq = fmax(r_ineq, -s_du[r]); r_comp = fmax(r_comp, fabs(LAM_IN(1) * s_du[r])); } }
#undef LAM_IN
            if (ONE_SIDED(r) && fin(ubd)) { s_sg[r < NSOFT ? r : 0] = -1.0; s_dl[r] = -s_du[r]; }
        }
    }
    if (want_res) { r_stat = blk_max(r_stat); r_eq = blk_max(r_eq); r_ineq = blk_max(r_ineq); r_comp = blk_max(r_comp); }
    if (want_res && tid == 0) {
        double *rs = a.res + (size_t)b * 4;
        rs[0] = r_stat; rs[1] = r_eq; rs[2] = r_ineq; rs[3] = r_comp;
    }

    const double tol_g = a.tol * sg, tol_b = a.tol * sb, tol_d = a.tol * sb, tol_m = a.tol * sg;
    const double mu_floor = 0.1 * tol_m;
    const double mu0 = a.mu0 * sg;
    const double inv_m = (a.m_act > 0) ? 1.0 / a.m_act : 0.0;

    auto row_dot = [&](int kc, const double *v) -> double {
        const int k = kc / NCK, c = kc % NCK;
        if (c < 10) return v[k * 10 + c];
        if (ALAT && c == 14) return ha[k * 4] * v[k * 10 + 3] + ha[k * 4 + 1] * v[k * 10 + 4] + ha[k * 4 + 2] * v[k * 10 + 6] + ha[k * 4 + 3] * v[k * 10 + 7];
        if (PATH && c >= 12) return (c == 12) ? v[k * 10 + 1] + hc[k * 2] * v[k * 10 + 2] : -v[k * 10 + 1] + hc[k * 2 + 1] * v[k * 10 + 2];
        double acc = 0.0;
#pragma unroll
        for (int j = 0; j < 10; j++) acc = fma(CDV(k, c - 10, j), v[k * 10 + j], acc);
        return acc;
    };

    for (int e = tid; e < NS * 10; e += NT) z[e] = (e < 8) ? a.x0[(size_t)b * 8 + e] - xb[e] : 0.0;
    for (int e = tid; e < NS * 8; e += NT) pi[e] = 0.0;
    BSYNC();
#pragma unroll
    for (int r = 0; r < NSLOT; r++) {
        if (s_kc[r] < 0) continue;
        const double rz = ROW_DOT(r, z);
        const bool al = HAS_L(r), au = HAS_U(r);
        double tau_c = a.tau0;
        if (al && au) tau_c = fmin(a.tau0, 0.25 * (s_du[r] - s_dl[r]));
        if (IS_SOFT(r)) {
            const double slack = al ? rz - s_dl[r] : s_du[r] - rz;
            const double s0 = fmax(a.tau0, a.tau0 - slack);
            so_s[r < NSOFT ? r : 0] = s0;
            so_ls[r < NSOFT ? r : 0] = mu0 / s0;
            if (al) { t_l[r] = slack + s0; lam_l[r] = mu0 / t_l[r]; } else { t_u[r] = slack + s0; lam_u[r] = mu0 / t_u[r]; }
            continue;
        }
        if (al) { t_l[r] = fmax(rz - s_dl[r], tau_c); lam_l[r] = mu0 / t_l[r]; }
        if (au) { t_u[r] = fmax(s_du[r] - rz, tau_c); lam_u[r] = mu0 / t_u[r]; }
    }

    int qstatus = 1, it = 0;
    bool exact_mode = false;
    double res_g = 0, res_b = 0, res_d = 0, res_m = 0, mu = 0;
    double fol_g = 0.0, fol_b = 0.0;
    double rd_l[NSLOT], rd_u[NSLOT], dlam_l[NSLOT], dlam_u[NSLOT], dt_l[NSLOT], dt_u[NSLOT];
    double pa_l[NSLOT], pa_u[NSLOT];
    for (it = 0;; it++) {
        bool exact = (it == 0) || exact_mode, finished = false;
        auto multipliers_to_cf = [&]() {
            for (int e = tid; e < NS * NCK; e += NT) cf[e] = 0.0;
            BSYNC();
#pragma unroll
            for (int r = 0; r < NSLOT; r++) {
                if (s_kc[r] < 0) continue;
                const bool al = HAS_L(r), au = HAS_U(r);
                SLOT_ACC(cf[s_kc[r]], ROW_SIGN(r, (al ? lam_l[r] : 0.0) - (au ? lam_u[r] : 0.0)));
            }
            BSYNC();
        };
        if (LEAN != 0) { if (exact) multipliers_to_cf(); }
        else {
            for (int e = tid; e < NS * NCK; e += NT) cf[e] = 0.0;
            BSYNC();
        }
        double mu_acc = 0.0, res_gs = 0.0;
        res_d = 0.0; res_m = 0.0;
#pragma unroll
        for (int r = 0; r < NSLOT; r++) {
            rd_l[r] = rd_u[r] = 0.0;
            if (s_kc[r] < 0) continue;
            const double rz = ROW_DOT(r, z);
            const bool al = HAS_L(r), au = HAS_U(r);
            const double sv = IS_SOFT(r) ? so_s[r < NSOFT ? r : 0] : 0.0;
            double pl = 0.0, pu = 0.0;
            if (al) { rd_l[r] = rz - t_l[r] - s_dl[r] + sv; pl = __dmul_rn(lam_l[r], t_l[r]); res_m = nanmax(res_m, fabs(pl)); }
            if (au) { rd_u[r] = s_du[r] - rz - t_u[r] + sv; pu = __dmul_rn(lam_u[r], t_u[r]); res_m = nanmax(res_m, fabs(pu)); }
            mu_acc = __dadd_rn(mu_acc, __dadd_rn(pl, pu));
            res_d = nanmax(res_d, nanmax(fabs(rd_l[r]), fabs(rd_u[r])));
            if (IS_SOFT(r)) {
                const int q = r < NSOFT ? r : 0;
                so_rs[q] = so_Zw[q] * so_s[q] + so_zw[q] - (al ? lam_l[r] : lam_u[r]) - so_ls[q];
                res_gs = nanmax(res_gs, fabs(so_rs[q]));
                mu_acc += so_ls[q] * so_s[q]; res_m = nanmax(res_m, fabs(so_ls[q] * so_s[q]));
            }
            if (LEAN == 0) SLOT_ACC(cf[s_kc[r]], ROW_SIGN(r, (al ? lam_l[r] : 0.0) - (au ? lam_u[r] : 0.0)));
        }
        if constexpr (NW > 1) {
#pragma unroll
            for (int r = 0; r < NSLOT; r++) {
                const int sidx = tid + NT * r;
                if (sidx >= a.nslots_can) continue;
                const bool on = s_kc[r] >= 0;
                gam[sidx] = __dadd_rn((on && fin(s_dl[r])) ? __dmul_rn(lam_l[r], t_l[r]) : 0.0, (on && fin(s_du[r])) ? __dmul_rn(lam_u[r], t_u[r]) : 0.0);
            }
            __syncthreads();
            mu_acc = 0.0;
            for (int sidx = lane; sidx < a.nslots_can; sidx += 64) mu_acc = __dadd_rn(mu_acc, gam[sidx]);
            __syncthreads();
        }
        if (LEAN == 0) BSYNC();
        for (int rpass = 0; rpass < 2; rpass++) {
            if (exact) {
                for (int e = tid; e < NS * 10; e += NT) {
                    const int k = e / 10, j = e % 10;
                    double acc = gb[e];
                    if (HL && h_sparse) {
                        const int row = ((k == N) ? 10 : 0) + j;
#pragma unroll
                        for (int q = 0; q < 3; q++) acc = fma(spv[row * 3 + q], z[k * 10 + spc[row * 3 + q]], acc);
                    } else {
#pragma unroll
                        for (int l = 0; l < 10; l++) acc = fma(HS(k, j, l), z[k * 10 + l], acc);
                    }
                    if (k < N) {
                        acc = fma(-CDV(k, 0, j), cf[k * NCK + 10], acc);
                        acc = fma(-CDV(k, 1, j), cf[k * NCK + 11], acc);
                    }
                    if (j < 8) acc -= pi[k * 8 + j];
                    acc -= cf[k * NCK + j];
                    if (PATH && (j == 1 || j == 2)) {
                        const double l12 = cf[k * NCK + 12], l13 = cf[k * NCK + 13];
                        acc -= (j == 1) ? l12 - l13 : hc[k * 2] * l12 + hc[k * 2 + 1] * l13;
                    }
                    if (ALAT && alat_slot(j) >= 0) acc -= ha[k * 4 + alat_slot(j)] * cf[k * NCK + 14];
                    gt[e] = acc;
                }
                BSYNC();
                dyn_residual<4, NT>(N, tid, const_cast<double *>(linb), z, pi, gt, rb, LIN_REC);
                BSYNC();
            }
            res_g = 0.0; res_b = 0.0;
            if (exact || LEAN == 0) {
                for (int e = tid; e < NS * 10; e += NT) {
                    const int k = e / 10, j = e % 10;
                    double v = gt[e];
                    if ((k == 0 && j < 8) || (k == N && j >= 8)) { v = 0.0; gt[e] = 0.0; }
                    if (exact) rgb[e] = v;
                    res_g = nanmax(res_g, fabs(v));
                }
                for (int e = tid; e < N * 8; e += NT) res_b = nanmax(res_b, fabs(rb[e]));
            } else { res_g = fol_g; res_b = fol_b; }
            res_g = nanmax(res_g, res_gs);
            res_g = blk_nanmax(res_g); res_b = blk_nanmax(res_b);
            if (rpass == 0) { res_d = blk_nanmax(res_d); res_m = blk_nanmax(res_m); mu = ((NW == 1) ? blk_sum(mu_acc) : wave_sum(mu_acc)) * inv_m; }
            if (!(res_g == res_g) || !(res_b == res_b) || !(res_d == res_d) || !(res_m == res_m)) { qstatus = (it == 0) ? 3 : 4; finished = true; break; }
            const bool conv = res_g <= tol_g && res_b <= tol_b && res_d <= tol_d && res_m <= tol_m;
            if (conv && exact) { qstatus = 0; finished = true; break; }
            if ((conv || it >= a.iter_max) && !exact) {
                exact = true; exact_mode = true;
                if (LEAN != 0) multipliers_to_cf();
                continue;
            }
            break;
        }
        if (finished) break;
        if (it >= a.iter_max) { qstatus = 1; break; }
        BSYNC();
        double alpha = 1.0, alpha_d = 1.0, sigma = 0.0;
        auto slot_coeffs = [&](int pass) {
            for (int e = tid; e < NS * NCK; e += NT) { cf[e] = 0.0; if (pass == 0) gam[e] = 0.0; }
            BSYNC();
            const double mu_t = fmax(sigma * mu, mu_floor);
#pragma unroll
            for (int r = 0; r < NSLOT; r++) {
                if (s_kc[r] < 0) continue;
                const bool al = HAS_L(r), au = HAS_U(r);
                double c = 0.0;
                if (IS_SOFT(r)) {
                    const int q = r < NSOFT ? r : 0;
                    const double lm = al ? lam_l[r] : lam_u[r], tt = al ? t_l[r] : t_u[r], rdv = al ? rd_l[r] : rd_u[r];
                    const double gm = lm / tt, gs = so_ls[q] / so_s[q], D = so_Zw[q] + gm + gs;
                    double c1, c2, rsv;
                    if (pass == 0) { c1 = (lm * tt + lm * rdv) / tt; c2 = so_ls[q]; rsv = so_rs[q]; gam[s_kc[r]] += gm * (so_Zw[q] + gs) / D; }
                    else { c1 = ((al ? pa_l[r] : pa_u[r]) - mu_t) / tt; c2 = (so_pa[q] - mu_t) / so_s[q]; rsv = 0.0; }
                    c = c1 - gm * (rsv + c1 + c2) / D;
                    cf[s_kc[r]] += ONE_SIDED(r) ? ROW_SIGN(r, c) : (al ? c : -c);
                    continue;
                }
                if (pass == 0) {
                    const double gl = al ? lam_l[r] / t_l[r] : 0.0, gu = au ? lam_u[r] / t_u[r] : 0.0;
                    if (al) c += fma(gl, rd_l[r], lam_l[r]);
                    if (au) c -= fma(gu, rd_u[r], lam_u[r]);
                    SLOT_ACC(gam[s_kc[r]], gl + gu);
                } else {
                    if (al) c += (pa_l[r] - mu_t) / t_l[r];
                    if (au) c -= (pa_u[r] - mu_t) / t_u[r];
                }
                SLOT_ACC(cf[s_kc[r]], ROW_SIGN(r, c));
            }
            BSYNC();
        };
        auto add_coeffs = [&]() {
            for (int e = tid; e < NS * 10; e += NT) {
                const int k = e / 10, j = e % 10;
                double acc = gt[e] + cf[k * NCK + j];
                if (k < N) {
                    acc = fma(CDV(k, 0, j), cf[k * NCK + 10], acc);
                    acc = fma(CDV(k, 1, j), cf[k * NCK + 11], acc);
                }
                if (PATH && (j == 1 || j == 2)) {
                    const double c12 = cf[k * NCK + 12], c13 = cf[k * NCK + 13];
                    acc += (j == 1) ? c12 - c13 : hc[k * 2] * c12 + hc[k * 2 + 1] * c13;
                }
                if (ALAT && alat_slot(j) >= 0) acc += ha[k * 4 + alat_slot(j)] * cf[k * NCK + 14];
                gt[e] = acc;
            }
            BSYNC();

        };
        slot_coeffs(0);
        add_coeffs();
        __builtin_amdgcn_s_waitcnt(0x0F70);
        if (wv == 0) {
            RicLds L;
            const QpRic o = qp_lds_ric(N, NS, NCK);
            L.gt = o.gt; L.pv = o.pv; L.gam = o.gam; L.dz = o.dz; L.kff = o.kff; L.Kl = o.Kl;
            L.Ginv = o.Ginv; L.hv = o.Prb; L.tile = o.tile; L.hc = o.hc; L.ha = o.ha;
            if constexpr (NF != 0)
                riccati_sweep_mfma<NCK, PATH != 0, UNI != 0, RIC_RING, ALAT, true, (NF > 0) ? NF : 0>(N, lane, linb, Hs0, HsT, a.CD, L, Pg, Mg, LIN_REC, false, false);
            else
            riccati_sweep_mfma<NCK, PATH != 0, UNI != 0, RIC_RING, ALAT>(N, lane, linb, Hs0, HsT, a.CD, L, Pg, Mg, LIN_REC, a.m_act == 0, a.symmetrize != 0);
            if (lane < 8) dz[lane] = 0.0;
        }
        BSYNC();
        for (int pass = 0; pass < 2; pass++) {
            const double mu_t = fmax(sigma * mu, mu_floor);
            if (pass == 1) slot_coeffs(1);
            if (pass == 1) {
            add_coeffs();
            for (int e = tid; e < NS * 8; e += NT) {
                const int k = e >> 3, j = e & 7;
                double v = gt[k * 10 + j];
                if (k < N) v -= Kl[k * 16 + j] * gt[k * 10 + 8] + Kl[k * 16 + 8 + j] * gt[k * 10 + 9];
                pv[e] = v;
            }
            BSYNC();
            if constexpr (LEAN != 0) {
            if (wv == 0) {
                const int g = lane >> 3, w = lane & 7;
                double pw = pv[N * 8 + w], pg = 0.0;
                const int se2 = (w == 0) ? 16 : 0, so2 = (g == 0) ? 16 : 0;
                const double *be = (w == 0) ? pv + (N - 1) * 8 + g : dz, *bo = (g == 0) ? pv + (N - 2) * 8 + w : dz;
                const double *qe = Prb + (N - 1) * 8 + w, *qo = Prb + (N - 2) * 8 + g;
                double *oe = pv + (N - 1) * 8 + g, *oo = pv + (N - 2) * 8 + w;
                stream_rows<-1, SWEEP_RING, SWEEP_DL>(Mg, N, RIC_IDX(w, g), RIC_IDX(g, w),
                    [&](int k, bool odd, double &prb, double &base) {
                        if (odd) { prb = *qo; qo -= 16; base = *bo; bo -= so2; } else { prb = *qe; qe -= 16; base = *be; be -= se2; }
                    },
                    [&](int k, double m, bool odd, double prb, double base) {
                        if (!odd) {
                            pg = sum8(fma(m, pw, fma(m, prb, base)));
                            *oe = pg; oe -= 16;
                        } else {
                            pw = sum_stride8(fma(m, pg, fma(m, prb, base)));
                            *oo = pw; oo -= 16;
                        }
                    });
            }
            } else {
            if (wv == 0) {
                const int g = lane >> 3, w = lane & 7;
                double pw = pv[N * 8 + w], pg = 0.0;
                stream_rows_v1<-1, QP_V1_RING, QP_V1_DL>(Mg, N, RIC_IDX(w, g), RIC_IDX(g, w),
                    [&](int k, bool odd, double &prb, double &base) { prb = Prb[k * 8 + (odd ? g : w)]; base = pv[k * 8 + (odd ? w : g)]; },
                    [&](int k, double m, bool odd, double prb, double base) {
                        if (!odd) {
                            const double off = fma(m, prb, (w == 0) ? base : 0.0);
                            pg = sum8(fma(m, pw, off));
                            if (w == 0) pv[k * 8 + g] = pg;
                        } else {
                            const double off = fma(m, prb, (g == 0) ? base : 0.0);
                            pw = sum_stride8(fma(m, pg, off));
                            if (g == 0) pv[k * 8 + w] = pw;
                        }
                    });
            }
            }
            BSYNC();
            for (int k = tid; k < N; k += NT) {
                const double *rec = linb + (size_t)k * LIN_REC;
                double g0 = gt[k * 10 + 8], g1 = gt[k * 10 + 9];
                double Bk[16];
#pragma unroll
                for (int l = 0; l < 16; l++) Bk[l] = rec[64 + l];
#pragma unroll
                for (int l = 0; l < 8; l++) {
                    const double h = Prb[k * 8 + l] + pv[(k + 1) * 8 + l];
                    g0 = fma(Bk[l * 2 + 0], h, g0);
                    g1 = fma(Bk[l * 2 + 1], h, g1);
                }
                const double kf0 = Ginv[k * 8 + 0] * g0 + Ginv[k * 8 + 1] * g1;
                const double kf1 = Ginv[k * 8 + 1] * g0 + Ginv[k * 8 + 2] * g1;
                kff[k * 4 + 0] = kf0;
                kff[k * 4 + 1] = kf1;
#pragma unroll
                for (int i = 0; i < 8; i++) dz[(k + 1) * 10 + i] = rb[k * 8 + i] - Bk[i * 2] * kf0 - Bk[i * 2 + 1] * kf1;
            }
            if (tid < 8) dz[tid] = 0.0;
            BSYNC();
            }

            if constexpr (LEAN != 0) {
            if (wv == 0) {
                const int g = lane >> 3, w = lane & 7;
                double dxw = dz[w], dxg = 0.0;
                const int se2 = (w == 0) ? 20 : 0, so2 = (g == 0) ? 20 : 0;
                const double *ce = (w == 0) ? dz + 10 + g : dz, *co = (g == 0) ? dz + 20 + w : dz;
                stream_rows<+1, SWEEP_RING, SWEEP_DL>(Mg, N, RIC_IDX(g, w), RIC_IDX(w, g),
                    [&](int k, bool odd, double &c, double &unused) {
                        if (odd) { c = *co; co += so2; } else { c = *ce; ce += se2; }
                        unused = 0.0;
                    },
                    [&](int k, double m, bool odd, double c, double) {
                        if (!odd) {
                            dxg = sum8(fma(m, dxw, c));
                            dz[(k + 1) * 10 + g] = dxg;
                        } else {
                            dxw = sum_stride8(fma(m, dxg, c));
                            dz[(k + 1) * 10 + w] = dxw;
                        }
                    });
            }
            } else {
            if (wv == 0) {
                const int g = lane >> 3, w = lane & 7;
                double dxw = dz[w], dxg = 0.0;
                stream_rows_v1<+1, QP_V1_RING, QP_V1_DL>(Mg, N, RIC_IDX(g, w), RIC_IDX(w, g),
                    [&](int k, bool odd, double &c, double &unused) { c = dz[(k + 1) * 10 + (odd ? w : g)]; unused = 0.0; },
                    [&](int k, double m, bool odd, double c, double) {
                        if (!odd) {
                            dxg = sum8(fma(m, dxw, (w == 0) ? c : 0.0));
                            if (w == 0) dz[(k + 1) * 10 + g] = dxg;
                        } else {
                            dxw = sum_stride8(fma(m, dxg, (g == 0) ? c : 0.0));
                            if (g == 0) dz[(k + 1) * 10 + w] = dxw;
                        }
                    });
            }
            }
            BSYNC();
            const bool want_dpi = (pass == 1) || (a.m_act == 0);
            for (int e = tid; e < NS * 2; e += NT) {
                const int k = e >> 1, aa = e & 1;
                double acc = 0.0;
                if (k < N) {
                    acc = -kff[k * 4 + aa];
#pragma unroll
                    for (int l = 0; l < 8; l++) acc = fma(-Kl[k * 16 + aa * 8 + l], dz[k * 10 + l], acc);
                }
                dz[k * 10 + 8 + aa] = acc;
            }
            if (want_dpi) {
                const int n = NS * 8;
                for (int base = 0; base < n; base += 3 * NT) {
                    double2 pr[3][4];
#pragma unroll
                    for (int q = 0; q < 3; q++) {
                        const int e = min(base + NT * q + tid, n - 1), k = e >> 3, i = e & 7;
#pragma unroll
                        for (int l = 0; l < 4; l++) pr[q][l] = *reinterpret_cast<const double2 *>(Pg + (size_t)k * 64 + RIC_IDX(l, i));
                    }
#pragma unroll
                    for (int q = 0; q < 3; q++) {
                        const int e = base + NT * q + tid, ec = min(e, n - 1), k = ec >> 3;
                        double acc = pv[ec];
#pragma unroll
                        for (int l = 0; l < 4; l++) { acc = fma(pr[q][l].x, dz[k * 10 + l], acc); acc = fma(pr[q][l].y, dz[k * 10 + l + 4], acc); }
                        if (e < n) pv[e] = acc;
                    }
                }
            }
            BSYNC();

            double amax = 1.0, amax_d = 1.0, mu_aff = 0.0, rmax = 1.0, rmax_d = 1.0;
#pragma unroll
            for (int r = 0; r < NSLOT; r++) {
                dlam_l[r] = dlam_u[r] = dt_l[r] = dt_u[r] = 0.0;
                if (s_kc[r] < 0) continue;
                const double drz = ROW_DOT(r, dz);
                if (IS_SOFT(r)) {
                    const int q = r < NSOFT ? r : 0;
                    const bool al = HAS_L(r);
                    const double lm = al ? lam_l[r] : lam_u[r], tt = al ? t_l[r] : t_u[r], rdv = al ? rd_l[r] : rd_u[r];
                    const double y = al ? drz : -drz;
                    const double gm = lm / tt, gs = so_ls[q] / so_s[q], D = so_Zw[q] + gm + gs;
                    const double rm1 = (pass == 0) ? lm * tt : lm * tt + (al ? pa_l[r] : pa_u[r]) - mu_t;
                    const double rm2 = (pass == 0) ? so_ls[q] * so_s[q] : so_ls[q] * so_s[q] + so_pa[q] - mu_t;
                    const double c1 = (rm1 + lm * rdv) / tt, c2 = rm2 / so_s[q];
                    const double dsv = -(so_rs[q] + c1 + c2) / D - gm / D * y;
                    const double dlsv = -(rm2 + so_ls[q] * dsv) / so_s[q];
                    const double dtv = y + dsv + rdv;
                    const double dlv = -(rm1 + lm * dtv) / tt;
                    so_ds[q] = dsv; so_dls[q] = dlsv;
                    if (al) { dt_l[r] = dtv; dlam_l[r] = dlv; } else { dt_u[r] = dtv; dlam_u[r] = dlv; }
                    if (dsv < 0.0) amax = fmin(amax, -so_s[q] / dsv);
                    if (dlsv < 0.0) amax_d = fmin(amax_d, -so_ls[q] / dlsv);
                    if (dtv < 0.0) amax = fmin(amax, -tt / dtv);
                    if (dlv < 0.0) amax_d = fmin(amax_d, -lm / dlv);
                    continue;
                }
                if (HAS_L(r)) {
                    const double rm = (pass == 0) ? lam_l[r] * t_l[r] : lam_l[r] * t_l[r] + pa_l[r] - mu_t;
                    dt_l[r] = drz + rd_l[r];
                    if (NSOFT == 0) {
                        const double it = 1.0 / t_l[r];
                        dlam_l[r] = -(rm + lam_l[r] * dt_l[r]) * it;
                        rmax = fmax(rmax, -dt_l[r] * it);
                        rmax_d = fmax(rmax_d, -dlam_l[r] / lam_l[r]);
                    } else {
                        dlam_l[r] = -(rm + lam_l[r] * dt_l[r]) / t_l[r];
                        if (dt_l[r] < 0.0) amax = fmin(amax, -t_l[r] / dt_l[r]);
                        if (dlam_l[r] < 0.0) amax_d = fmin(amax_d, -lam_l[r] / dlam_l[r]);
                    }
                }
                if (HAS_U(r)) {
                    const double rm = (pass == 0) ? lam_u[r] * t_u[r] : lam_u[r] * t_u[r] + pa_u[r] - mu_t;
                    dt_u[r] = -drz + rd_u[r];
                    if (NSOFT == 0) {
                        const double it = 1.0 / t_u[r];
                        dlam_u[r] = -(rm + lam_u[r] * dt_u[r]) * it;
                        rmax = fmax(rmax, -dt_u[r] * it);
                        rmax_d = fmax(rmax_d, -dlam_u[r] / lam_u[r]);
                    } else {
                        dlam_u[r] = -(rm + lam_u[r] * dt_u[r]) / t_u[r];
                        if (dt_u[r] < 0.0) amax = fmin(amax, -t_u[r] / dt_u[r]);
                        if (dlam_u[r] < 0.0) amax_d = fmin(amax_d, -lam_u[r] / dlam_u[r]);
                    }
                }
            }
            if (NSOFT == 0) { amax = fmin(amax, 1.0 / rmax); amax_d = fmin(amax_d, 1.0 / rmax_d); }
            amax = blk_min(amax); amax_d = blk_min(amax_d);
            if (pass == 0) {
                if (a.m_act == 0) { alpha = alpha_d = 1.0; break; }
#pragma unroll
                for (int r = 0; r < NSLOT; r++) {
                    pa_l[r] = dlam_l[r] * dt_l[r]; pa_u[r] = dlam_u[r] * dt_u[r];
                    if (s_kc[r] < 0) continue;
                    mu_aff = __dadd_rn(mu_aff, __dadd_rn(HAS_L(r) ? __dmul_rn(fma(amax_d, dlam_l[r], lam_l[r]), fma(amax, dt_l[r], t_l[r])) : 0.0,
                                                         HAS_U(r) ? __dmul_rn(fma(amax_d, dlam_u[r], lam_u[r]), fma(amax, dt_u[r], t_u[r])) : 0.0));
                    if (IS_SOFT(r)) {
                        const int q = r < NSOFT ? r : 0;
                        so_pa[q] = so_dls[q] * so_ds[q];
                        mu_aff += (so_ls[q] + amax_d * so_dls[q]) * (so_s[q] + amax * so_ds[q]);
                    }
                }
                if constexpr (NW > 1) {
#pragma unroll
                    for (int r = 0; r < NSLOT; r++) {
                        const int sidx = tid + NT * r;
                        if (sidx >= a.nslots_can) continue;
                        const bool on = s_kc[r] >= 0;
                        gam[sidx] = __dadd_rn((on && fin(s_dl[r])) ? __dmul_rn(fma(amax_d, dlam_l[r], lam_l[r]), fma(amax, dt_l[r], t_l[r])) : 0.0,
                                              (on && fin(s_du[r])) ? __dmul_rn(fma(amax_d, dlam_u[r], lam_u[r]), fma(amax, dt_u[r], t_u[r])) : 0.0);
                    }
                    __syncthreads();
                    mu_aff = 0.0;
                    for (int sidx = lane; sidx < a.nslots_can; sidx += 64) mu_aff = __dadd_rn(mu_aff, gam[sidx]);
                    __syncthreads();
                    mu_aff = wave_sum(mu_aff) * inv_m;
                } else
                mu_aff = blk_sum(mu_aff) * inv_m;
                const double ratio = (mu > 0.0) ? mu_aff / mu : 0.0;
                sigma = ratio * ratio * ratio;
            } else {
                alpha = fmin(1.0, IHM2MPC_IPM_STEP_FRACTION * amax); alpha_d = fmin(1.0, IHM2MPC_IPM_STEP_FRACTION * amax_d);
            }
            BSYNC();
        }
        if (fmin(alpha, alpha_d) < 1e-12) { qstatus = 2; break; }
        if (!exact_mode) {
            const double cd = 1.0 - alpha_d, cp = alpha - alpha_d, cb = 1.0 - alpha;
            const int n10 = NS * 10;
            fol_g = 0.0; fol_b = 0.0;
            for (int base = 0; base < n10; base += 4 * NT) {
                double ro[4];
#pragma unroll
                for (int q = 0; q < 4; q++) ro[q] = rgb[min(base + NT * q + tid, n10 - 1)];
#pragma unroll
                for (int q = 0; q < 4; q++) {
                    const int e = base + NT * q + tid, ec = min(e, n10 - 1), k = ec / 10, j = ec % 10;
                    double hdz = 0.0;
                    if (HL && h_sparse) {
                        const int row = ((k == N) ? 10 : 0) + j;
#pragma unroll
                        for (int l = 0; l < 3; l++) hdz = fma(spv[row * 3 + l], dz[k * 10 + spc[row * 3 + l]], hdz);
                    } else {
#pragma unroll
                        for (int l = 0; l < 10; l++) hdz = fma(HS(k, j, l), dz[k * 10 + l], hdz);
                    }
                    const bool masked = (k == 0 && j < 8) || (k == N && j >= 8);
                    const double v = masked ? 0.0 : fma(cp, hdz, cd * ro[q]);
                    if (e < n10) { rgb[e] = v; gt[e] = v; if (LEAN != 0) fol_g = nanmax(fol_g, fabs(v)); }
                }
            }
            for (int e = tid; e < N * 8; e += NT) {
                const double v = cb * rb[e];
                rb[e] = v;
                if (LEAN != 0) fol_b = nanmax(fol_b, fabs(v));
                const_cast<double *>(linb)[(size_t)(e >> 3) * LIN_REC + RIC_REC_RB + (e & 7)] = v;
            }
        }
        for (int e = tid; e < NS * 10; e += NT) z[e] = fma(alpha, dz[e], z[e]);
        for (int e = tid; e < NS * 8; e += NT) pi[e] = fma(alpha_d, pv[e], pi[e]);
#pragma unroll
        for (int r = 0; r < NSLOT; r++) {
            if (s_kc[r] < 0) continue;
            if (HAS_L(r)) { lam_l[r] = fma(alpha_d, dlam_l[r], lam_l[r]); t_l[r] = fma(alpha, dt_l[r], t_l[r]); }
            if (HAS_U(r)) { lam_u[r] = fma(alpha_d, dlam_u[r], lam_u[r]); t_u[r] = fma(alpha, dt_u[r], t_u[r]); }
            if (IS_SOFT(r)) { const int q = r < NSOFT ? r : 0; so_s[q] = fma(alpha, so_ds[q], so_s[q]); so_ls[q] = fma(alpha_d, so_dls[q], so_ls[q]); }
        }
        BSYNC();
    }
    if (qstatus == 1 && !(res_g <= 1e4 * tol_g && res_b <= 1e4 * tol_b && res_d <= 1e4 * tol_d && res_m <= 1e4 * tol_m)) qstatus = 4;

    int st = 0;
    if (qstatus == 3) st = 1;
    else if (qstatus == 2 || qstatus == 4) st = 4;
    BSYNC();
    if (st == 0) {
        double bad = 0.0;
        for (int e = tid; e < NS * 10; e += NT) bad = fmax(bad, isfinite(z[e]) ? 0.0 : 1.0);
        if (blk_max(bad) > 0.0) st = 1;
    }
    double *xw = a.x + (size_t)b * NS * 8, *uw = a.u + (size_t)b * N * 2;
    if (NSOFT > 0) {
        for (int e = tid; e < NS * 28; e += NT) slkb[e] = 0.0;
        if (ALAT) for (int e = tid; e < NS * 2; e += NT) slkab[e] = 0.0;
    }
    if (st == 0) {
        for (int e = tid; e < NS * 10; e += NT) {
            const int k = e / 10, j = e % 10;
            if (j < 8) xw[k * 8 + j] += z[e];
            else if (k < N) uw[k * 2 + j - 8] += z[e];
        }
        for (int e = tid; e < NS * 8; e += NT) pib[e] = (e < 8) ? 0.0 : pi[e];
        for (int e = tid; e < NS * 28; e += NT) lamb[e] = 0.0;
        if (ALAT) for (int e = tid; e < NS * 2; e += NT) lamab[e] = 0.0;
        __syncthreads();
#pragma unroll
        for (int r = 0; r < NSLOT; r++) {
            if (s_kc[r] < 0) continue;
            const int k = s_kc[r] / NCK, c = s_kc[r] % NCK;
            if (ONE_SIDED(r)) {
                const int up = (s_sg[r < NSOFT ? r : 0] < 0.0) ? 1 : 0;
                if (ALAT && c == 14) { lamab[k * 2 + up] = lam_l[r]; if (IS_SOFT(r)) slkab[k * 2 + up] = so_s[r < NSOFT ? r : 0]; }
                else { lamb[k * 28 + 14 * up + c] = lam_l[r]; if (IS_SOFT(r)) slkb[k * 28 + 14 * up + c] = so_s[r < NSOFT ? r : 0]; }
                continue;
            }
            if (ALAT && c == 14) {
                if (fin(s_dl[r])) lamab[k * 2] = lam_l[r];
                if (fin(s_du[r])) lamab[k * 2 + 1] = lam_u[r];
                if (IS_SOFT(r)) slkab[k * 2 + (fin(s_dl[r]) ? 0 : 1)] = so_s[r < NSOFT ? r : 0];
                continue;
            }
            if (fin(s_dl[r])) lamb[k * 28 + c] = lam_l[r];
            if (fin(s_du[r])) lamb[k * 28 + 14 + c] = lam_u[r];
            if (IS_SOFT(r)) slkb[k * 28 + (fin(s_dl[r]) ? c : 14 + c)] = so_s[r < NSOFT ? r : 0];
        }
    }
    __syncthreads();
    if (tid < 2) a.u0[(size_t)b * 2 + tid] = uw[tid];
    if (tid == 0) {
        a.status[b] = st; a.qp_iter[b] = it;
        double *q = a.qp_res + (size_t)b * 4;
        q[0] = res_g / tol_g * a.tol; q[1] = res_b / tol_b * a.tol; q[2] = res_d / tol_d * a.tol; q[3] = res_m / tol_m * a.tol;
    }
}

#undef BSYNC

template <int NSLOT, int NSOFT, int PATH, int UNI, int NF = 0>
__global__ __launch_bounds__(64) void k_qp_wave(QpArgs a)
{
    extern __shared__ double sm[];
    if ((int)blockIdx.x >= a.B) return;
    if (NF > 0 && a.N != NF) return;
    qp_wave_body<NSLOT, NSOFT, PATH, UNI, 1, 1, NF>(a, blockIdx.x, sm);
}

template <int NSLOT, int UNI, int NW>
__global__ __launch_bounds__(64 * NW) void k_qp_block(QpArgs a)
{
    extern __shared__ double sm[];
    if ((int)blockIdx.x >= a.B) return;
    qp_wave_body<NSLOT, 0, 0, UNI, NW>(a, blockIdx.x, sm);
}

__device__ __noinline__ void call_integrate_fkin6(const double *xk, const double *uk, const double *x_next, int tid, int M, double dt, int nknots,
                                                  const double *s_ref, const double *kappa_ref, double *rec, double *xn_out)
{
    dev_integrate_sens_fkin6(xk, uk, x_next, tid, M, dt, nknots, s_ref, kappa_ref, rec, xn_out);
}
__device__ __noinline__ void call_integrate_fkin6_lag(const double *xk, const double *uk, const double *x_next, int tid, int M, double dt, int nknots,
                                                      const double *s_ref, const double *kappa_ref, double *rec, double *xn_out, const double *lagf)
{
    dev_integrate_sens_fkin6_lag(xk, uk, x_next, tid, M, dt, nknots, s_ref, kappa_ref, rec, xn_out, lagf);
}
template <int MODEL>
__device__ __noinline__ void call_integrate_dyn(const double *xk, const double *uk, const double *x_next, int tid, int M, double dt, int nknots,
                                                const double *s_ref, const double *kappa_ref, double *rec, double *Sl)
{
    dev_integrate_sens_dyn<MODEL>(xk, uk, x_next, tid, M, dt, nknots, s_ref, kappa_ref, rec, Sl);
}
template <int MODEL>
__device__ __noinline__ void call_linearize_irk(const IrkTab *tab, int b, int base, int N, int nknots, const double *s_ref, const double *kappa_ref, int tid,
                                                const double *x, const double *u, double *lin)
{
    const int st = threadIdx.x & 3, q = base + ((int)threadIdx.x >> 2), k = min(q, N - 1);
    const IrkRows rows = irk_rows_from(tab, st);
    irk_linearize_quad<MODEL>(st, rows, x + ((size_t)b * (N + 1) + k) * 8, u + ((size_t)b * N + k) * 2, tid, nknots, s_ref, kappa_ref,
                              lin + ((size_t)b * N + k) * LIN_REC, q < N);
}
__device__ __noinline__ void call_sim_step(int b, int q, int model, int M, double dt, int nknots, const double *s_ref, const double *kappa_ref,
                                           const int32_t *track_id, const double *xs, const double *us, double *xn)
{
    dev_sim_step(b, q, model, M, dt, nknots, s_ref, kappa_ref, track_id, xs, us, xn, nullptr);
}

__device__ __noinline__ void call_sim_irk(const IrkTab *tab, int b, int model, int M, int nknots, const double *s_ref, const double *kappa_ref,
                                          const int32_t *track_id, const double *u0, double *x0)
{
    const int st = threadIdx.x & 3;
    double x[8];
#pragma unroll
    for (int a = 0; a < 8; a++) x[a] = x0[(size_t)b * 8 + a];
    const double u_T = u0[(size_t)b * 2], u_d = u0[(size_t)b * 2 + 1];
    const int tid = track_id[b];
    TrackSeg trk;
    trk.init(s_ref + (size_t)tid * nknots, kappa_ref + (size_t)tid * nknots, nknots, x[0]);
    const IrkRows rows = irk_rows_from(tab, st);
    irk_sim_quad(st, rows, model, M, x, u_T, u_d, trk);
    __syncthreads();
    if (threadIdx.x == 0)
#pragma unroll
        for (int a = 0; a < 8; a++) x0[(size_t)b * 8 + a] = x[a];
}

template <int MODEL, bool ROLL>
__device__ __noinline__ void call_line_search(const LsArgs &ls, int b, int it, int last)
{
    line_search_body<MODEL, ROLL>(ls, b, it, last);
}

template <int NSLOT, int NSOFT, int PATH, int UNI, int SQP, int IRK = 0, int DYN = 0, int SENS = 0, int NF = 0>
__global__ __launch_bounds__(64) void k_steps(const StepArgs *sp, QpArgs a, const LsArgs *lsp)
{
    static_assert(DYN == 0 || s_count(1) == QP_DYN_RK4_WORDS, "the dynamic models' RK4 integrator parks s_count(1) words per lane in the QP's LDS (qp_lds.hpp: steps_lds_doubles)");
    const StepArgs &s = *sp;
    const LsArgs &ls = *lsp;
    extern __shared__ double sm[];
    const int b = blockIdx.x, lane = threadIdx.x;
    if (b >= a.B) return;
    if (NF > 0 && a.N != NF) return;
    const int N = (NF > 0) ? NF : a.N;
    const size_t B = a.B;
    auto stop_from = [&](int step) {
        if (s.active && lane == 0) s.active[b] = 0;
        for (int t = step; t < s.n_steps; t++) {
            if (s.hist_u0 && lane < 2) s.hist_u0[((size_t)t * B + b) * 2 + lane] = 0.0;
            if (s.hist_x0 && lane < 8) s.hist_x0[((size_t)t * B + b) * 8 + lane] = s.x0[(size_t)b * 8 + lane];
            if (s.hist_st && lane == 0) s.hist_st[(size_t)t * B + b] = a.status[b];
            if (s.hist_it && lane == 0) s.hist_it[(size_t)t * B + b] = 0;
        }
        if constexpr (SENS != 0) {
            const SensArgs &sa = *s.sens;
            const int NS = N + 1;
            if (sa.hist && lane < 16)
                for (int t = step; t < s.n_steps; t++) sa.hist[((size_t)t * B + b) * 16 + lane] = NAN;
            if (lane < 16) sa.sens_u0[(size_t)b * 16 + lane] = NAN;
            if (sa.mode == 2) {
                for (int e = lane; e < NS * 64; e += 64) sa.sens_x[(size_t)b * NS * 64 + e] = NAN;
                for (int e = lane; e < N * 16; e += 64) sa.sens_u[(size_t)b * N * 16 + e] = NAN;
            }
        }
    };
    for (int step = 0; step < s.n_steps; step++) {
        bool act = s.active ? s.active[b] != 0 : true;
        if (s.freeze && act) {
            const int st = a.status[b];
            if (st != 0 && st != 2) act = false;
        }
        if (!act && s.freeze) { stop_from(step); return; }
        if (s.lap_wrap) { dev_wrap_lap(b, lane, N, s.nknots, s.s_ref, a.track_id, s.x0, a.x); __syncthreads(); }
        const double x_old = (lane < 8) ? s.x0[(size_t)b * 8 + lane] : 0.0;
        const bool irk_plant = s.sim_irk_tab != nullptr;
        const bool kin_plant = (IRK == 2 ? s.sim_lag != 0 : !IRK) && !irk_plant && s.model == IHM2MPC_MODEL_FKIN6;
        double *spare = s.lin + (size_t)B * N * LIN_REC;
        if (!kin_plant && act) {
            if (irk_plant) call_sim_irk(s.sim_irk_tab, b, s.model, s.M_sim, s.nknots, s.s_ref, s.kappa_ref, a.track_id, a.u0, s.x0);
            else if (lane < 4) call_sim_step(b, lane, s.model, s.M_sim, s.dt, s.nknots, s.s_ref, s.kappa_ref, a.track_id, s.x0, a.u0, s.x0);
            __syncthreads();
        }
        dev_prepare(b, lane, N, s.s_target, 2, s.x0, a.x, a.u, s.yref, s.yref_e);
        const int n_it = SQP ? s.sqp_iters : 1;
        if (SQP && lane == 0) { ls.done[b] = 0; ls.sqp_iter[b] = 0; ls.qp_acc[b] = 0; }
        __syncthreads();
        for (int it = 0; it < n_it; it++) {
            if (SQP) {
                const int NS = N + 1;
                for (int e = lane; e < NS * 8; e += 64) {
                    ((double *)ls.xp)[(size_t)b * NS * 8 + e] = a.x[(size_t)b * NS * 8 + e];
                    ((double *)ls.pip)[(size_t)b * NS * 8 + e] = a.pi[(size_t)b * NS * 8 + e];
                }
                for (int e = lane; e < N * 2; e += 64) ((double *)ls.up)[(size_t)b * N * 2 + e] = a.u[(size_t)b * N * 2 + e];
                for (int e = lane; e < NS * 28; e += 64) {
                    ((double *)ls.lamp)[(size_t)b * NS * 28 + e] = a.lam[(size_t)b * NS * 28 + e];
                    ((double *)ls.slkp)[(size_t)b * NS * 28 + e] = a.slk[(size_t)b * NS * 28 + e];
                }
            }
            {
                const int tid = a.track_id[b];
                const bool with_plant = kin_plant && it == 0 && act;
                const int om = DYN ? s.ocp_model : IHM2MPC_MODEL_FKIN6;
                if (IRK == 1) {
                    for (int base = 0; base < N; base += 16) {
                        if constexpr (!DYN) call_linearize_irk<IHM2MPC_MODEL_FKIN6>(s.irk_tab, b, base, N, s.nknots, s.s_ref, s.kappa_ref, tid, a.x, a.u, s.lin);
                        else {
                            if (om == IHM2MPC_MODEL_FDYN6U) call_linearize_irk<IHM2MPC_MODEL_FDYN6U>(s.irk_tab, b, base, N, s.nknots, s.s_ref, s.kappa_ref, tid, a.x, a.u, s.lin);
                            else call_linearize_irk<IHM2MPC_MODEL_FDYN6>(s.irk_tab, b, base, N, s.nknots, s.s_ref, s.kappa_ref, tid, a.x, a.u, s.lin);
                        }
                    }
                } else
                for (int k = lane; k < N + (with_plant ? 1 : 0); k += 64) {
                    const bool plant = k == N;
                    const double *xk = plant ? s.x0 + (size_t)b * 8 : a.x + ((size_t)b * (N + 1) + k) * 8;
                    const double *uk = plant ? a.u0 + (size_t)b * 2 : a.u + ((size_t)b * N + k) * 2;
                    double *rec = plant ? spare + (size_t)b * LIN_REC : s.lin + ((size_t)b * N + k) * LIN_REC;
                    if constexpr (IRK == 2)
                        call_integrate_fkin6_lag(xk, uk, plant ? xk : xk + 8, tid, plant ? s.M_sim : s.M, s.dt, s.nknots, s.s_ref, s.kappa_ref, rec,
                                                 plant ? s.x0 + (size_t)b * 8 : nullptr, s.lag[plant ? 1 : 0]);
                    else if (!DYN || plant)
                        call_integrate_fkin6(xk, uk, plant ? xk : xk + 8, tid, plant ? s.M_sim : s.M, s.dt, s.nknots, s.s_ref, s.kappa_ref, rec,
                                             plant ? s.x0 + (size_t)b * 8 : nullptr);
                    else if constexpr (DYN != 0) {
                        if (om == IHM2MPC_MODEL_FDYN6U)
                            call_integrate_dyn<IHM2MPC_MODEL_FDYN6U>(xk, uk, xk + 8, tid, s.M, s.dt, s.nknots, s.s_ref, s.kappa_ref, rec, sm + lane);
                        else
                            call_integrate_dyn<IHM2MPC_MODEL_FDYN6>(xk, uk, xk + 8, tid, s.M, s.dt, s.nknots, s.s_ref, s.kappa_ref, rec, sm + lane);
                    }
                }
            }
            __syncthreads();
            if constexpr (SENS != 0) {
                const SensArgs &sa = *s.sens;
                const int NS = N + 1;
                for (int e = lane; e < NS * 8; e += 64) ((double *)sa.xbar)[(size_t)b * NS * 8 + e] = a.x[(size_t)b * NS * 8 + e];
                for (int e = lane; e < N * 2; e += 64) ((double *)sa.ubar)[(size_t)b * N * 2 + e] = a.u[(size_t)b * N * 2 + e];
            }
            if (it == 0) {
                if (s.freeze) {
                    const double v = (lane < 8) ? s.x0[(size_t)b * 8 + lane] : 0.0;
                    if (__any(v != v)) {
                        if (lane < 8) s.x0[(size_t)b * 8 + lane] = x_old;
                        __syncthreads();
                        stop_from(step);
                        return;
                    }
                }
                dev_prepare(b, lane, N, s.s_target, 1, s.x0, a.x, a.u, s.yref, s.yref_e);
                __syncthreads();
            }
            qp_wave_body<NSLOT, NSOFT, PATH, UNI, 1, SQP ? 0 : 1, NF>(a, b, sm, SQP || step + 1 == s.n_steps);
            __syncthreads();
            if constexpr (SENS != 0) {
                sens_body(*s.sens, b, sm, step);
                __syncthreads();
            }
            if (SQP) {
                const int last = it == n_it - 1;
                if constexpr (!DYN) call_line_search<IHM2MPC_MODEL_FKIN6, IRK != 0>(ls, b, it, last);
                else {
                    if (s.ocp_model == IHM2MPC_MODEL_FDYN6U) call_line_search<IHM2MPC_MODEL_FDYN6U, IRK != 0>(ls, b, it, last);
                    else call_line_search<IHM2MPC_MODEL_FDYN6, IRK != 0>(ls, b, it, last);
                }
                __syncthreads();
            }
        }
        if (s.hist_u0 && lane < 2) s.hist_u0[((size_t)step * B + b) * 2 + lane] = a.u0[(size_t)b * 2 + lane];
        if (s.hist_x0 && lane < 8) s.hist_x0[((size_t)step * B + b) * 8 + lane] = s.x0[(size_t)b * 8 + lane];
        if (s.hist_st && lane == 0) s.hist_st[(size_t)step * B + b] = a.status[b];
        if (s.hist_it && lane == 0) s.hist_it[(size_t)step * B + b] = a.qp_iter[b];
        if (s.freeze && s.x0[(size_t)b * 8] > s.lap_stop) {
            if (s.active && lane == 0) s.active[b] = 0;
            __syncthreads();
        }
    }
}

}

#ifndef QP_SET
#error "compile with -DQP_SET=0 (all-hard instantiations), -DQP_SET=1 (soft / track-row instantiations), -DQP_SET=2 (dynamic OCP models in the persistent loop), -DQP_SET=3 (the persistent loop with x0 sensitivities), -DQP_SET=4 (the benchmarked all-hard pair with the straight-line factor sweep), -DQP_SET=5 or -DQP_SET=6 (the all-hard RTI loops with the closed-form actuator lags: general form / straight-line factor sweep)"
#endif
#define QP_INSTANCES_(n) QP_INSTANCES_##n
#define QP_INSTANCES_OF(n) QP_INSTANCES_(n)
#define QP_INSTANCES QP_INSTANCES_OF(QP_SET)

#if QP_SET == 4 || QP_SET == 6
#define WAVE(NS, NO, PT, UN)                                                                          \
    {{QP_WAVE, NS, NO, PT, UN, 0, 0, 0, 0, 40}, 64, (const void *)k_qp_wave<NS, NO, PT, UN, 40>},     \
    {{QP_WAVE, NS, NO, PT, UN, 0, 0, 0, 0, -1}, 64, (const void *)k_qp_wave<NS, NO, PT, UN, -1>},
#define STEPS(NS, NO, PT, UN, IR, DY)                                                                                    \
    {{QP_STEPS, NS, NO, PT, UN, 0, IR, DY, 0, 40}, 64, (const void *)k_steps<NS, NO, PT, UN, 0, IR, DY, 0, 40>},         \
    {{QP_STEPS, NS, NO, PT, UN, 0, IR, DY, 0, -1}, 64, (const void *)k_steps<NS, NO, PT, UN, 0, IR, DY, 0, -1>},
#else
#define WAVE(NS, NO, PT, UN) {{QP_WAVE, NS, NO, PT, UN, 0, 0, 0}, 64, (const void *)k_qp_wave<NS, NO, PT, UN>},
#define BLOCK(NS, UN, NW) {{QP_BLOCK, NS, 0, 0, UN, 0, 0, 0}, 64 * NW, (const void *)k_qp_block<NS, UN, NW>},
#if QP_SET == 3
#define STEPS(NS, NO, PT, UN, IR, DY) {{QP_STEPS, NS, NO, PT, UN, 0, IR, DY, 1}, 64, (const void *)k_steps<NS, NO, PT, UN, 0, IR, DY, 1>},
#elif QP_SET == 5
#define STEPS(NS, NO, PT, UN, IR, DY) {{QP_STEPS, NS, NO, PT, UN, 0, IR, DY}, 64, (const void *)k_steps<NS, NO, PT, UN, 0, IR, DY>},
#else
#define STEPS(NS, NO, PT, UN, IR, DY)                                                                  \
    {{QP_STEPS, NS, NO, PT, UN, 0, IR, DY}, 64, (const void *)k_steps<NS, NO, PT, UN, 0, IR, DY>}, \
    {{QP_STEPS, NS, NO, PT, UN, 1, IR, DY}, 64, (const void *)k_steps<NS, NO, PT, UN, 1, IR, DY>},
#endif
#endif
#define QP_TABLE_(n) ihm2_qp_set##n
#define QP_TABLE(n) QP_TABLE_(n)
QpTable QP_TABLE(QP_SET)()
{
    static const QpInst inst[] = {QP_INSTANCES(WAVE, BLOCK, STEPS)};
    return {inst, (int)(sizeof(inst) / sizeof(inst[0]))};
}
```

ihm2_amd/csrc/qp_catalogue.hpp:

```cpp
#pragma once

#include <utility>
#include <vector>

#define QP_INSTANCES_0(WAVE, BLOCK, STEPS)                                                                                                \
    BLOCK(2, 0, 4) BLOCK(2, 1, 4)                                                                                                         \
    WAVE(5, 0, 0, 0) WAVE(5, 0, 0, 1) WAVE(8, 0, 0, 0) WAVE(8, 0, 0, 1) WAVE(10, 0, 0, 0) WAVE(10, 0, 0, 1)                               \
    STEPS(5, 0, 0, 0, 0, 0) STEPS(5, 0, 0, 1, 0, 0) STEPS(5, 0, 0, 1, 1, 0)                                                               \
    STEPS(8, 0, 0, 0, 0, 0) STEPS(8, 0, 0, 1, 0, 0) STEPS(8, 0, 0, 1, 1, 0)                                                               \
    STEPS(10, 0, 0, 1, 0, 0) STEPS(10, 0, 0, 1, 1, 0)
#define QP_INSTANCES_1(WAVE, BLOCK, STEPS)                                                                                                \
    WAVE(8, 2, 0, 0) WAVE(8, 2, 0, 1) WAVE(10, 4, 0, 0) WAVE(10, 4, 0, 1)                                                                 \
    WAVE(8, 0, 1, 0) WAVE(8, 0, 1, 1) WAVE(8, 3, 1, 0) WAVE(8, 3, 1, 1) WAVE(10, 4, 1, 0) WAVE(10, 4, 1, 1)                               \
    WAVE(8, 0, 2, 1) WAVE(10, 4, 2, 1)                                                                                                    \
    STEPS(8, 2, 0, 1, 0, 0) STEPS(8, 2, 0, 1, 1, 0) STEPS(10, 4, 0, 1, 0, 0) STEPS(10, 4, 0, 1, 1, 0)                                     \
    STEPS(8, 0, 1, 1, 0, 0) STEPS(8, 0, 1, 1, 1, 0) STEPS(8, 3, 1, 1, 0, 0) STEPS(8, 3, 1, 1, 1, 0)                                       \
    STEPS(10, 4, 1, 1, 0, 0) STEPS(10, 4, 1, 1, 1, 0)
#define QP_INSTANCES_2(WAVE, BLOCK, STEPS)                                                                                                \
    STEPS(5, 0, 0, 1, 0, 1) STEPS(5, 0, 0, 1, 1, 1) STEPS(8, 0, 0, 1, 0, 1) STEPS(8, 0, 0, 1, 1, 1)                                       \
    STEPS(8, 2, 0, 1, 0, 1) STEPS(8, 2, 0, 1, 1, 1) STEPS(10, 4, 0, 1, 0, 1) STEPS(10, 4, 0, 1, 1, 1)                                     \
    STEPS(8, 0, 1, 1, 0, 1) STEPS(8, 0, 1, 1, 1, 1) STEPS(8, 3, 1, 1, 0, 1) STEPS(8, 3, 1, 1, 1, 1)                                       \
    STEPS(10, 4, 1, 1, 0, 1) STEPS(10, 4, 1, 1, 1, 1)
#define QP_INSTANCES_3(WAVE, BLOCK, STEPS)                                                                                                \
    STEPS(5, 0, 0, 0, 0, 0) STEPS(5, 0, 0, 1, 0, 0) STEPS(5, 0, 0, 1, 1, 0)                                                               \
    STEPS(8, 0, 0, 0, 0, 0) STEPS(8, 0, 0, 1, 0, 0) STEPS(8, 0, 0, 1, 1, 0)                                                               \
    STEPS(10, 0, 0, 1, 0, 0) STEPS(10, 0, 0, 1, 1, 0)                                                                                     \
    STEPS(8, 2, 0, 1, 0, 0) STEPS(8, 2, 0, 1, 1, 0) STEPS(10, 4, 0, 1, 0, 0) STEPS(10, 4, 0, 1, 1, 0)                                     \
    STEPS(8, 0, 1, 1, 0, 0) STEPS(8, 0, 1, 1, 1, 0) STEPS(8, 3, 1, 1, 0, 0) STEPS(8, 3, 1, 1, 1, 0)                                       \
    STEPS(10, 4, 1, 1, 0, 0) STEPS(10, 4, 1, 1, 1, 0)
#define QP_INSTANCES_4(WAVE, BLOCK, STEPS) WAVE(5, 0, 0, 1) STEPS(5, 0, 0, 1, 0, 0)
#define QP_INSTANCES_5(WAVE, BLOCK, STEPS)                                                                                                \
    STEPS(5, 0, 0, 0, 2, 0) STEPS(5, 0, 0, 1, 2, 0) STEPS(8, 0, 0, 0, 2, 0) STEPS(8, 0, 0, 1, 2, 0) STEPS(10, 0, 0, 1, 2, 0)
#define QP_INSTANCES_6(WAVE, BLOCK, STEPS) STEPS(5, 0, 0, 1, 2, 0)

namespace ihm2 {

inline std::vector<std::pair<int, int>> slot_limits(int path)
{
    struct Wave { int nslot, nsoft, path; };
#define IHM2_CATALOGUE_WAVE(NS, NO, PT, UN) {NS, NO, PT},
#define IHM2_CATALOGUE_SKIP(...)
#define IHM2_CATALOGUE_SET(n) QP_INSTANCES_##n(IHM2_CATALOGUE_WAVE, IHM2_CATALOGUE_SKIP, IHM2_CATALOGUE_SKIP)
    static const Wave waves[] = {IHM2_CATALOGUE_SET(0) IHM2_CATALOGUE_SET(1) IHM2_CATALOGUE_SET(2) IHM2_CATALOGUE_SET(3)
                                 IHM2_CATALOGUE_SET(4) IHM2_CATALOGUE_SET(5) IHM2_CATALOGUE_SET(6)};
#undef IHM2_CATALOGUE_SET
#undef IHM2_CATALOGUE_SKIP
#undef IHM2_CATALOGUE_WAVE
    std::vector<std::pair<int, int>> v;
    for (const Wave &w : waves) {
        if (w.path != path) continue;
        auto p = v.begin();
        while (p != v.end() && p->first != w.nsoft) ++p;
        if (p == v.end()) v.push_back({w.nsoft, w.nslot});
        else if (w.nslot > p->second) p->second = w.nslot;
    }
    return v;
}

}
```

ihm2_amd/csrc/qp_lds.hpp:

```cpp
#pragma once

#ifdef __HIPCC__
#define QP_LDS_FN __host__ __device__ constexpr
#else
#define QP_LDS_FN constexpr
#endif

namespace ihm2 {

constexpr int QP_TILE_ROW = 17, QP_TILE_WORDS = 8 * QP_TILE_ROW;
constexpr int QP_V1_RING = 8, QP_V1_DL = 4;
constexpr int QP_DYN_RK4_WORDS = 55;

struct QpLdsClass { int nck; bool hc, ha, hl, cl; };
QP_LDS_FN QpLdsClass qp_lds_class(int path, bool uni) { return {path == 2 ? 15 : path ? 14 : 12, path != 0, path == 2, uni && !path, uni}; }

struct QpArr {
    int off, len;
    QP_LDS_FN operator int() const { return off; }
    QP_LDS_FN int end() const { return off + len; }
};

struct QpLds {
    QpArr z;
    QpArr gt;
    QpArr pi;
    QpArr pv;
    QpArr rb;
    QpArr gam;
    QpArr cf;
    QpArr dz;
    QpArr kff;
    QpArr Kl;
    QpArr Ginv;
    QpArr Prb;
    QpArr tile;
    QpArr hc;
    QpArr ha;
    QpArr Hl;
    QpArr CDl;
    QpArr spv;
    QpArr spc;
    int total;
};
constexpr int QP_LDS_ARRAYS = 19;
QP_LDS_FN QpArr qp_lds_array(const QpLds &l, int i)
{
    const QpArr a[QP_LDS_ARRAYS] = {l.z, l.gt, l.pi, l.pv, l.rb, l.gam, l.cf, l.dz, l.kff, l.Kl, l.Ginv, l.Prb, l.tile, l.hc, l.ha, l.Hl, l.CDl, l.spv, l.spc};
    return a[i];
}

enum QpArrId { QP_Z, QP_GT, QP_PI, QP_PV, QP_RB, QP_GAM, QP_CF, QP_DZ, QP_KFF, QP_KL, QP_GINV, QP_PRB, QP_TILE, QP_HC, QP_HA, QP_HL, QP_CDL, QP_SPV, QP_SPC };
QP_LDS_FN int qp_lds_len(int id, int N, int NS, QpLdsClass c)
{
    switch (id) {
    case QP_Z: case QP_GT: case QP_DZ: return NS * 10;
    case QP_PI: case QP_PV: return NS * 8;
    case QP_GAM: case QP_CF: return NS * c.nck;
    case QP_RB: case QP_GINV: case QP_PRB: return N * 8;
    case QP_KFF: return N * 4;
    case QP_KL: return N * 16;
    case QP_TILE: return QP_TILE_WORDS;
    case QP_HC: return c.hc ? NS * 2 : 0;
    case QP_HA: return c.ha ? NS * 4 : 0;
    case QP_HL: return c.hl ? 200 : 0;
    case QP_CDL: return c.cl ? 20 : 0;
    case QP_SPV: return c.hl ? 60 : 0;
    default: return c.hl ? 30 : 0;
    }
}

QP_LDS_FN QpLds qp_lds(int N, QpLdsClass c)
{
    QpLds l = {};
    QpArr *const a[QP_LDS_ARRAYS] = {&l.z, &l.gt, &l.pi, &l.pv, &l.rb, &l.gam, &l.cf, &l.dz, &l.kff, &l.Kl, &l.Ginv, &l.Prb, &l.tile, &l.hc, &l.ha, &l.Hl, &l.CDl, &l.spv, &l.spc};
    for (int id = 0; id < QP_LDS_ARRAYS; id++) {
        *a[id] = {l.total, qp_lds_len(id, N, N + 1, c)};
        l.total += a[id]->len;
    }
    return l;
}

struct QpRic { int gt, pv, gam, dz, kff, Kl, Ginv, Prb, tile, hc, ha; };
QP_LDS_FN QpRic qp_lds_ric(int N, int NS, int nck)
{
    QpRic L = {};
    L.gt = NS * 10; L.pv = NS * 28; L.gam = NS * 36 + N * 8; L.dz = L.gam + 2 * NS * nck; L.kff = L.dz + NS * 10; L.Kl = L.kff + N * 4;
    L.Ginv = L.Kl + N * 16; L.Prb = L.Ginv + N * 8; L.tile = L.Prb + N * 8; L.hc = L.tile + QP_TILE_WORDS; L.ha = L.hc + NS * 2;
    return L;
}
QP_LDS_FN bool qp_lds_ric_agrees(int N, QpLdsClass c)
{
    const QpLds l = qp_lds(N, c);
    const QpRic o = qp_lds_ric(N, N + 1, c.nck);
    return o.gt == l.gt && o.pv == l.pv && o.gam == l.gam && o.dz == l.dz && o.kff == l.kff && o.Kl == l.Kl && o.Ginv == l.Ginv && o.Prb == l.Prb &&
           o.tile == l.tile && o.hc == l.hc && (!c.hc || o.ha == l.ha);
}
QP_LDS_FN bool qp_lds_ric_agrees(int N)
{
    return qp_lds_ric_agrees(N, qp_lds_class(0, false)) && qp_lds_ric_agrees(N, qp_lds_class(0, true)) && qp_lds_ric_agrees(N, qp_lds_class(1, false)) &&
           qp_lds_ric_agrees(N, qp_lds_class(1, true)) && qp_lds_ric_agrees(N, qp_lds_class(2, true));
}
static_assert(qp_lds_ric_agrees(40) && qp_lds_ric_agrees(2), "the factor sweep's offsets are not the layout's");

struct QpReach { int lo, hi; };
QP_LDS_FN bool qp_inside(QpReach r, int lo, int hi) { return lo <= r.lo && r.lo <= r.hi && r.hi <= hi; }

QP_LDS_FN int qp_sweep_fetches(int N, int d, int dl) { return dl + (N + 2 * d - 1) / (2 * d) * 2 * d; }
QP_LDS_FN QpReach qp_reach_lean_vector(const QpLds &l, int N, int d, int dl)
{
    return {l.pv + (N - 2) * 8 - 16 * (qp_sweep_fetches(N, d, dl) / 2 - 1), l.Prb + N * 8};
}
QP_LDS_FN QpReach qp_reach_lean_forward(const QpLds &l, int N, int d, int dl)
{
    return {l.dz, l.dz + 20 + 20 * (qp_sweep_fetches(N, d, dl) / 2 - 1) + 8};
}
QP_LDS_FN QpReach qp_reach_v1_vector(const QpLds &l, int N)
{
    return {l.pv + (N - qp_sweep_fetches(N, QP_V1_RING, QP_V1_DL)) * 8, l.Prb + N * 8};
}
QP_LDS_FN QpReach qp_reach_v1_forward(const QpLds &l, int N)
{
    return {l.dz, l.dz + qp_sweep_fetches(N, QP_V1_RING, QP_V1_DL) * 10 + 8};
}
QP_LDS_FN QpReach qp_reach_plain_parking(const QpLds &l) { return {l.tile, l.tile + 63 + 4 + 1}; }
QP_LDS_FN QpReach qp_reach_plain_operand(const QpLds &l, int N, int nck) { return {l.gt - 10, l.gam + N * nck}; }
QP_LDS_FN QpReach qp_reach_block_reduce(const QpLds &l, int nw) { return {l.tile, l.tile + nw}; }

QP_LDS_FN bool qp_sweeps_inside(const QpLds &l, int N, bool lean, int d, int dl)
{
    return lean ? qp_inside(qp_reach_lean_vector(l, N, d, dl), 0, l.total) && qp_inside(qp_reach_lean_forward(l, N, d, dl), 0, l.total)
                : qp_inside(qp_reach_v1_vector(l, N), 0, l.total) && qp_inside(qp_reach_v1_forward(l, N), 0, l.total);
}
QP_LDS_FN bool qp_factor_inside(const QpLds &l, int N, int nck)
{
    return qp_inside(qp_reach_plain_parking(l), l.tile, l.tile.end()) && qp_inside(qp_reach_block_reduce(l, 4), l.tile, l.tile.end()) &&
           qp_inside(qp_reach_plain_operand(l, N, nck), 0, l.total);
}

struct StepsLds {
    int qp, sens, dyn_rk4;
    QP_LDS_FN int total() const { return qp > sens ? qp : sens; }
    QP_LDS_FN bool guests_fit() const { return dyn_rk4 <= total(); }
};
QP_LDS_FN StepsLds steps_lds_doubles(int qp_total, int sens_doubles, bool dyn_rk4) { return {qp_total, sens_doubles, dyn_rk4 ? QP_DYN_RK4_WORDS * 64 : 0}; }

}
```

ihm2_amd/csrc/qp_tables.hpp:

```cpp
#pragma once

#include <algorithm>
#include <cmath>
#include <cstddef>
#include <cstdint>
#include <cstring>
#include <utility>
#include <vector>

#include "ihm2_dims.h"

namespace ihm2 {


inline double bound_or(double v, double absent) { return (std::fabs(v) < 1e20) ? v : absent; }

struct Bounds { double lb, ub; };
inline Bounds box_row(int N, int k, int c, const double *lbx, const double *ubx, const double *lbu, const double *ubu, const double *lg, const double *ug)
{
    if (c < 8) return (k >= 1) ? Bounds{lbx[k * 8 + c], ubx[k * 8 + c]} : Bounds{-INFINITY, INFINITY};
    if (k >= N) return {-INFINITY, INFINITY};
    return (c < 10) ? Bounds{lbu[k * 2 + c - 8], ubu[k * 2 + c - 8]} : Bounds{lg[k * 2 + c - 10], ug[k * 2 + c - 10]};
}

// ... 19 lines not shown
    explicit ConstraintRows(int ns) : NS(ns), lb(ns * NC, -INFINITY), ub(ns * NC, INFINITY), sz(ns * NLAM, 0.0), sZ(ns * NLAM, -1.0) {}

    void set_box_rows(const double *lbx, const double *ubx, const double *lbu, const double *ubu, const double *lg, const double *ug)
    {
        box_rows(NS - 1, lbx, ubx, lbu, ubu, lg, ug, lb.data(), ub.data(), NC);
    }
    void set_track_rows(bool enable, const double *lh, const double *uh)
    {
        for (int k = 0; k < NS; k++)
            for (int i = 0; i < NH; i++) {
                const bool on = enable && k >= 1;
                lb[k * NC + 12 + i] = on ? bound_or(lh[i], -INFINITY) : -INFINITY;
                ub[k * NC + 12 + i] = on ? bound_or(uh[i], INFINITY) : INFINITY;
            }
    }
};


struct SlotTable {
    bool fit = false;
    int per_lane = 0;
    int nsoft = 0;
    int total = 0;
    int m_act = 0;
    std::vector<int32_t> kc;
    std::vector<double> lb, ub, zw, Zw;
    int per_blk = 0;
    std::vector<int32_t> kc_blk;
    std::vector<double> lb_blk, ub_blk;

    size_t entries() const { return kc.size(); }
};

namespace slot_detail {

struct Slot { int kc; double lb, ub, zw, Zw; };
const Slot PADDING = {-1, -INFINITY, INFINITY, 0.0, -1.0};

struct Row {
    int kc;
    double lb, ub, szl, sZl, szu, sZu;
    bool fl, fu, sl, su;
    bool soft() const { return sl || su; }
    bool two_sided() const { return fl && fu; }
    int nsoft() const { return (int)sl + (int)su; }
};

inline std::vector<Row> finite_rows(const ConstraintRows &c)
{
    std::vector<Row> rows;
    for (int k = 0; k < c.NS; k++)
        for (int r = 0; r < NC + 1; r++) {
            const bool extra = r == NC;
            if (extra && !(c.alat_on && k >= 1 && k < c.NS - 1)) continue;
            Row row;
            row.kc = k * 16 + r;
            row.lb = extra ? c.alat_lb : c.lb[k * NC + r]; row.ub = extra ? c.alat_ub : c.ub[k * NC + r];
            row.fl = std::isfinite(row.lb); row.fu = std::isfinite(row.ub);
            if (!row.fl && !row.fu) continue;
            row.szl = extra ? c.alat_sz[0] : c.sz[k * NLAM + r]; row.sZl = extra ? c.alat_sZ[0] : c.sZ[k * NLAM + r];
            row.szu = extra ? c.alat_sz[1] : c.sz[k * NLAM + NC + r]; row.sZu = extra ? c.alat_sZ[1] : c.sZ[k * NLAM + NC + r];
            row.sl = row.fl && row.sZl >= 0.0; row.su = row.fu && row.sZu >= 0.0;
            rows.push_back(row);
        }
    return rows;
}

struct Lane {
    std::vector<Slot> ones, twos;
    int nsoft = 0;
    int size() const { return (int)(ones.size() + twos.size()); }
    int tail(int S) const { return (int)twos.size() + std::max(0, (int)ones.size() - S); }
    std::pair<int, int> cost(const Row &r, int S) const
    {
        if (r.soft()) return {nsoft, size()};
        const bool leads = S > 0 && !r.two_sided() && (int)ones.size() < S;
        return {0, tail(S) - (leads ? 1 : 0)};
    }
    void take(const Row &r, int S)
    {
        if (!r.soft()) {
            (S > 0 && !r.two_sided() ? ones : twos).push_back({r.kc, r.lb, r.ub, 0.0, -1.0});
            return;
        }
        const Slot lo = {r.kc, r.lb, INFINITY, r.sl ? r.szl : 0.0, r.sl ? r.sZl : -1.0}, up = {r.kc, -INFINITY, r.ub, r.su ? r.szu : 0.0, r.su ? r.sZu : -1.0};
        if (r.sl) ones.push_back(lo);
        if (r.su) ones.push_back(up);
        if (r.fl && !r.sl) ones.push_back(lo);
        if (r.fu && !r.su) ones.push_back(up);
        nsoft += r.nsoft();
    }
    std::vector<Slot> entries(int S) const
    {
        std::vector<Slot> lead = ones;
        std::stable_partition(lead.begin(), lead.end(), [](const Slot &s) { return s.Zw >= 0.0; });
        std::vector<Slot> e(lead.begin(), lead.begin() + std::min(S, (int)lead.size()));
        if (tail(S) > 0) e.resize(S, PADDING);
        if ((int)lead.size() > S) e.insert(e.end(), lead.begin() + S, lead.end());
        e.insert(e.end(), twos.begin(), twos.end());
        return e;
    }
};

}

inline SlotTable lay_out_slots(const ConstraintRows &c, const std::vector<std::pair<int, int>> &limits)
{
    using namespace slot_detail;
    const std::vector<Row> rows = finite_rows(c);
    SlotTable t;
    int soft_total = 0;
    for (const Row &r : rows) { soft_total += r.nsoft(); t.m_act += (int)r.fl + (int)r.fu + r.nsoft(); }
    for (const auto &lim : limits) {
        const int S = lim.first, NSL = lim.second;
        if ((S == 0) != (soft_total == 0)) continue;
        Lane lanes[64];
        for (const bool soft : {true, false})
            for (const Row &r : rows) {
                if (r.soft() != soft) continue;
                Lane *best = &lanes[0];
                for (Lane &l : lanes)
                    if (l.cost(r, S) < best->cost(r, S)) best = &l;
                best->take(r, S);
            }
        int per_lane = 0, soft_max = 0;
        for (const Lane &l : lanes) { per_lane = std::max(per_lane, S + l.tail(S)); soft_max = std::max(soft_max, l.nsoft); }
        if (soft_max > S || per_lane > NSL) continue;
        per_lane = 0;
        std::vector<Slot> entries[64];
        for (int l = 0; l < 64; l++) { entries[l] = lanes[l].entries(S); per_lane = std::max(per_lane, (int)entries[l].size()); }
        if (per_lane * 64 > MAX_SLOTS) break;
        t.fit = true; t.per_lane = per_lane; t.nsoft = S;
        const size_t n = (size_t)per_lane * 64;
        t.kc.assign(n, PADDING.kc); t.lb.assign(n, PADDING.lb); t.ub.assign(n, PADDING.ub); t.zw.assign(n, PADDING.zw); t.Zw.assign(n, PADDING.Zw);
        for (int l = 0; l < 64; l++)
            for (size_t r = 0; r < entries[l].size(); r++) {
                const Slot &s = entries[l][r];
                const size_t e = l + 64 * r;
                t.kc[e] = s.kc; t.lb[e] = s.lb; t.ub[e] = s.ub; t.zw[e] = s.zw; t.Zw[e] = s.Zw;
                t.total += s.kc >= 0;
            }
        if (S == 0 && t.total > 0 && t.total <= 1024) {
            t.per_blk = ((int)n + 255) / 256;
            const size_t nb = (size_t)t.per_blk * 256;
            t.kc_blk = t.kc; t.lb_blk = t.lb; t.ub_blk = t.ub;
            t.kc_blk.resize(nb, PADDING.kc); t.lb_blk.resize(nb, PADDING.lb); t.ub_blk.resize(nb, PADDING.ub);
        }
        break;
    }
    if (!t.fit) t.m_act = 0;
    return t;
}


struct PatternMismatch {
    bool found;
    int b, k, c;
    bool lower, upper, shared_lower, shared_upper;
};
inline PatternMismatch find_pattern_mismatch(const ConstraintRows &rows, int B, const double *il, const double *iu)
{
    const int NS = rows.NS;
    for (int b = 0; b < B; b++)
        for (int k = 0; k < NS; k++)
            for (int c = 0; c < 12; c++) {
                const size_t i = ((size_t)b * NS + k) * 12 + c;
                const bool lo = std::isfinite(il[i]), up = std::isfinite(iu[i]);
                const bool slo = std::isfinite(rows.lb[k * NC + c]), sup = std::isfinite(rows.ub[k * NC + c]);
                if (lo != slo || up != sup) return {true, b, k, c, lo, up, slo, sup};
            }
    return {false, 0, 0, 0, false, false, false, false};
}

inline void scatter_slot_bounds(const SlotTable &t, int B, int NS, const double *il, const double *iu, std::vector<double> &slb, std::vector<double> &sub)
{
    const size_t n = t.entries();
    slb.resize((size_t)B * n); sub.resize((size_t)B * n);
    for (int b = 0; b < B; b++) {
        const double *l = il + (size_t)b * NS * 12, *u = iu + (size_t)b * NS * 12;
        for (size_t e = 0; e < n; e++) {
            const int kc = t.kc[e], k = kc >> 4, c = kc & 15;
            double lo = t.lb[e], up = t.ub[e];
            if (kc >= 0 && c < 12) {
                if (std::isfinite(lo)) lo = l[k * 12 + c];
                if (std::isfinite(up)) up = u[k * 12 + c];
            }
            slb[(size_t)b * n + e] = lo; sub[(size_t)b * n + e] = up;
        }
    }
}

inline void scatter_stage_bounds(const ConstraintRows &rows, int B, const double *il, const double *iu, std::vector<double> &stl, std::vector<double> &stu)
{
    const int NS = rows.NS;
    stl.resize((size_t)B * NS * NC); stu.resize((size_t)B * NS * NC);
    for (int b = 0; b < B; b++)
        for (int k = 0; k < NS; k++)
            for (int c = 0; c < NC; c++) {
                const size_t i = ((size_t)b * NS + k) * 12 + c, o = ((size_t)b * NS + k) * NC + c;
                stl[o] = (c < 12) ? il[i] : rows.lb[k * NC + c];
                stu[o] = (c < 12) ? iu[i] : rows.ub[k * NC + c];
            }
}


inline void cost_selector(double V[NY][NZ])
{
    memset(V, 0, sizeof(double) * NY * NZ);
    for (int i = 0; i < NX; i++) V[i][i] = 1.0;
    V[10][6] = 1.0; V[11][7] = 1.0;
    V[8][8] = 1.0; V[9][9] = 1.0;
    V[10][8] = -1.0; V[11][9] = -1.0;
}

inline void stage_weight_tables(const double *Wk, double cs, double *Hk, double *Gk)
{
    double V[NY][NZ];
    cost_selector(V);
    double VtW[NZ][NY];
    for (int i = 0; i < NZ; i++)
        for (int j = 0; j < NY; j++) {
            double acc = 0;
            for (int l = 0; l < NY; l++) acc += V[l][i] * Wk[l * NY + j];
            VtW[i][j] = acc;
            Gk[i * 12 + j] = cs * acc;
        }
    for (int i = 0; i < NZ; i++)
        for (int j = 0; j < NZ; j++) {
            double acc = 0;
            for (int l = 0; l < NY; l++) acc += VtW[i][l] * V[l][j];
            Hk[i * 10 + j] = cs * acc;
        }
}

inline void terminal_weight_tables(const double *W_e, double *HN, double *GN)
{
    for (int i = 0; i < NX; i++)
        for (int j = 0; j < NX; j++) {
            HN[i * 10 + j] = W_e[i * NX + j];
            GN[i * 12 + j] = W_e[i * NX + j];
        }
    HN[8 * 10 + 8] = 1.0;
    HN[9 * 10 + 9] = 1.0;
}

inline bool symmetric10(const double *Hk)
{
    for (int i = 0; i < NZ; i++)
        for (int j = 0; j < i; j++)
            if (fabs(Hk[i * 10 + j] - Hk[j * 10 + i]) > 1e-12 * (1 + fabs(Hk[i * 10 + j]))) return false;
    return true;
}

inline bool stages_equal(const double *T, int N, int per_stage)
{
    for (int k = 1; k < N; k++)
        for (int i = 0; i < per_stage; i++)
            if (T[(size_t)k * per_stage + i] != T[i]) return false;
    return true;
}

}
```

ihm2_amd/solver.py:

```python
from __future__ import annotations

import ctypes as C

import numpy as np

from . import _lib
from .constants import NG, NLAM, NU, NX, NY
from .ocp import AcadosOcp, AcadosOcpOptions, OcpData

_SOLVER_TYPE = {"SQP_RTI": 0, "SQP": 1}
_GLOBALIZATION = {"FIXED_STEP": 0, "MERIT_BACKTRACKING": 1}


def _f64(a, shape=None, name="array"):
    a = np.ascontiguousarray(a, dtype=np.float64)
    if shape is not None and a.shape != tuple(shape):
        raise ValueError(f"{name} must have shape {tuple(shape)}, got {a.shape}")
    return a


def _ptr(a):
    return a.ctypes.data_as(_lib.c_double_p)


# ... 199 lines not shown
            a = np.empty(shape, dtype=dtype) if v is True else v
            if a.shape != shape or a.dtype != dtype or not a.flags.c_contiguous:
                raise ValueError(f"{name} must be a C-contiguous {np.dtype(dtype).name} array of shape {shape}")
            out[name] = a
            return a
        u = buf(u0_hist, (n, self.B, NU), np.float64, "u0"); x = buf(x0_hist, (n, self.B, NX), np.float64, "x0")
        st = buf(status_hist, (n, self.B), np.int32, "status"); it = buf(qp_iter_hist, (n, self.B), np.int32, "qp_iter")
        hists = (None if u is None else _ptr(u), None if x is None else _ptr(x),
                 None if st is None else st.ctypes.data_as(_lib.c_int32_p), None if it is None else it.ctypes.data_as(_lib.c_int32_p))
        if sens_u0_hist is None or sens_u0_hist is False:
            _lib.check(self.lib.ihm2mpc_run_steps(self._h, int(model), int(M_sim), float(s_target), n, int(bool(freeze)), float(lap_stop), *hists))
        else:
            k = buf(sens_u0_hist, (n, self.B, NU, NX), np.float64, "sens_u0")
            _lib.check(self.lib.ihm2mpc_run_steps_sens(self._h, int(model), int(M_sim), float(s_target), n, int(bool(freeze)), float(lap_stop),
                                                       *hists, _ptr(k)))
        if wait:
            self.synchronize()
        return out

    def set_sqp_options(self, globalization="MERIT_BACKTRACKING", alpha_min=0.05, alpha_reduction=0.7, eps_sufficient_descent=1e-4,
                        use_sufficient_descent=False, full_step_dual=False, tol=None):
        t = None if tol is None else np.ascontiguousarray(np.broadcast_to(_f64(tol), (4,)))
        _lib.check(self.lib.ihm2mpc_set_sqp_options(self._h, _GLOBALIZATION[globalization], float(alpha_min), float(alpha_reduction),
                                                     float(eps_sufficient_descent), int(bool(use_sufficient_descent)), int(bool(full_step_dual)),
                                                     None if t is None else _ptr(t)))

    def get_sqp_stats(self):
        it = np.empty(self.B, dtype=np.int32); alpha = np.empty(self.B)
        _lib.check(self.lib.ihm2mpc_get_sqp_stats(self._h, it.ctypes.data_as(_lib.c_int32_p), _ptr(alpha)))
        return {"sqp_iter": it, "alpha": alpha}

    def synchronize(self):
        _lib.check(self.lib.ihm2mpc_synchronize(self._h))

    def linearize(self):
        _lib.check(self.lib.ihm2mpc_linearize(self._h))

    def get_linearization(self):
        A = np.empty((self.B, self.N, NX, NX)); Bm = np.empty((self.B, self.N, NX, NU)); b = np.empty((self.B, self.N, NX))
        _lib.check(self.lib.ihm2mpc_get_linearization(self._h, _ptr(A), _ptr(Bm), _ptr(b)))
        return A, Bm, b

    def _get(self, fn, shape):
        out = np.empty(shape, dtype=np.float64)
        _lib.check(fn(self._h, _ptr(out)))
        return out

    def get_x(self):
        return self._get(self.lib.ihm2mpc_get_x, (self.B, self.N + 1, NX))

    def get_u(self):
        return self._get(self.lib.ihm2mpc_get_u, (self.B, self.N, NU))

    def get_u0(self):
        return self._get(self.lib.ihm2mpc_get_u0, (self.B, NU))

    def get_x0(self):
        return self._get(self.lib.ihm2mpc_get_x0, (self.B, NX))

    def get_residuals(self):
        return self._get(self.lib.ihm2mpc_get_residuals, (self.B, 4))

    def build_tracks(self, coeffs_X, coeffs_Y):
        if len(coeffs_X) != self.ntracks or len(coeffs_Y) != self.ntracks:
            raise ValueError(f"{self.ntracks} tracks expected")
        nseg = np.array([len(c) for c in coeffs_X], dtype=np.int32)
        mx = int(nseg.max())
        cX = np.zeros((self.ntracks, mx, 4)); cY = np.zeros((self.ntracks, mx, 4))
        for t in range(self.ntracks):
            cX[t, :nseg[t]] = coeffs_X[t]; cY[t, :nseg[t]] = coeffs_Y[t]
        _lib.check(self.lib.ihm2mpc_build_tracks(self._h, mx, nseg.ctypes.data_as(_lib.c_int32_p), _ptr(cX), _ptr(cY)))
        s_ref = np.empty((self.ntracks, self.nknots)); kappa = np.empty((self.ntracks, self.nknots))
        _lib.check(self.lib.ihm2mpc_get_tracks(self._h, _ptr(s_ref), _ptr(kappa), None, None, None))
        self._s_ref, self._kappa_ref = s_ref, kappa

    def fit_tracks(self, center_lines, curv_weight: float = 2.0):
        if len(center_lines) != self.ntracks:
            raise ValueError(f"{self.ntracks} tracks expected")
        npts = np.array([len(c) for c in center_lines], dtype=np.int32)
        mx = int(npts.max())
        xy = np.zeros((self.ntracks, mx, 2))
        for t, c in enumerate(center_lines):
            xy[t, :npts[t]] = np.asarray(c, dtype=np.float64)
        cX = np.zeros((self.ntracks, mx, 4)); cY = np.zeros((self.ntracks, mx, 4))
        _lib.check(self.lib.ihm2mpc_fit_tracks(self._h, mx, npts.ctypes.data_as(_lib.c_int32_p), _ptr(xy), float(curv_weight), _ptr(cX), _ptr(cY)))
        return [cX[t, :npts[t]].copy() for t in range(self.ntracks)], [cY[t, :npts[t]].copy() for t in range(self.ntracks)]

    def get_tracks(self):
        out = [np.empty((self.ntracks, self.nknots)) for _ in range(5)]
        _lib.check(self.lib.ihm2mpc_get_tracks(self._h, *[_ptr(a) for a in out]))
        return tuple(out)

    def sim_step_dyn10(self, x, u, M_sim: int = 100):
        xn = np.empty((self.B, 15))
        _lib.check(self.lib.ihm2mpc_sim_step_dyn10(self._h, int(M_sim), _ptr(_f64(x, (self.B, 15), "x")), _ptr(_f64(u, (self.B, 5), "u")), _ptr(xn)))
        return xn

    def get_qp_residuals(self):
        return self._get(self.lib.ihm2mpc_get_qp_residuals, (self.B, 4))

    def get_multipliers(self):
        pi = np.empty((self.B, self.N + 1, NX)); lam = np.empty((self.B, self.N + 1, NLAM))
        _lib.check(self.lib.ihm2mpc_get_multipliers(self._h, _ptr(pi), _ptr(lam)))
        return pi, lam

    def get_alat_multipliers(self):
        lam = np.empty((self.B, self.N + 1, 2)); slk = np.empty((self.B, self.N + 1, 2))
        _lib.check(self.lib.ihm2mpc_get_alat_multipliers(self._h, _ptr(lam), _ptr(slk)))
        return lam, slk

    def set_alat_multipliers(self, lam=None, slk=None):
        la = None if lam is None else _f64(lam, (self.B, self.N + 1, 2), "lam")
        sa = None if slk is None else _f64(slk, (self.B, self.N + 1, 2), "slk")
        _lib.check(self.lib.ihm2mpc_set_alat_multipliers(self._h, None if la is None else _ptr(la), None if sa is None else _ptr(sa)))

    def set_slacks(self, sl=None):
        _lib.check(self.lib.ihm2mpc_set_slacks(self._h, None if sl is None else _ptr(_f64(sl, (self.B, self.N + 1, NLAM), "sl"))))

    def get_slacks(self):
        return self._get(self.lib.ihm2mpc_get_slacks, (self.B, self.N + 1, NLAM))

    def get_status(self):
        out = np.empty(self.B, dtype=np.int32)
        _lib.check(self.lib.ihm2mpc_get_status(self._h, out.ctypes.data_as(_lib.c_int32_p)))
        return out

    def get_qp_iter(self):
        out = np.empty(self.B, dtype=np.int32)
        _lib.check(self.lib.ihm2mpc_get_qp_iter(self._h, out.ctypes.data_as(_lib.c_int32_p)))
        return out

    def get_timings(self):
        ms = np.zeros(3)
        _lib.check(self.lib.ihm2mpc_get_timings(self._h, _ptr(ms), 3))
        return {"total_ms": ms[0], "linearize_ms": ms[1], "qp_ms": ms[2]}

    def get_launch_record(self):
        rec = np.zeros(16, dtype=np.int32)
        _lib.check(self.lib.ihm2mpc_get_launch_record(self._h, rec.ctypes.data_as(_lib.c_int32_p)))
        r = [int(v) for v in rec]
        qp = None
        if r[0] == 1:
            qp = "k_qp_wave<%d,%d,%d,%d>" % tuple(r[1:5])
        elif r[0] == 2:
            qp = "k_qp_block<%d,%d,4>" % (r[1], r[4])
        steps, fallback = None, None
        if r[5] == 1:
            steps = "k_steps<%d,%d,%d,%d,%d,%d,%d>" % tuple(r[6:13]) if r[14] == 0 else "k_steps<%d,%d,%d,%d,%d,%d,%d,1>" % tuple(r[6:13])
        elif r[5] == 2:
            steps, fallback = "per_step", {1: "no_instantiation", 2: "not_resident"}.get(r[13])
        lin = (None, "k_linearize", "k_linearize_dyn", "k_linearize_cols", "k_linearize_irk", "k_linearize_lag")[r[15] & 15]
        sim = (None, "k_sim_step_kin", "k_sim_step", "k_sim_irk", "k_sim_step_kin_lag")[(r[15] >> 4) & 15]
        forms = ("general", "plain", "plain_n40", None)
        return {"qp": qp, "steps": steps, "steps_fallback": fallback, "linearize": lin, "sim": sim,
                "qp_form": forms[(r[15] >> 8) & 3] if qp else None, "steps_form": forms[(r[15] >> 12) & 3] if r[5] == 1 else None}

    def set_x0_device(self, dptr: int):
        _lib.check(self.lib.ihm2mpc_set_x0_device(self._h, C.c_void_p(dptr)))

    def get_u0_device(self, dptr: int):
        _lib.check(self.lib.ihm2mpc_get_u0_device(self._h, C.c_void_p(dptr)))

    def get_x_device(self, dptr: int):
        _lib.check(self.lib.ihm2mpc_get_x_device(self._h, C.c_void_p(dptr)))

    def get_u_device(self, dptr: int):
        _lib.check(self.lib.ihm2mpc_get_u_device(self._h, C.c_void_p(dptr)))

    def get_status_device(self, dptr: int):
        _lib.check(self.lib.ihm2mpc_get_status_device(self._h, C.c_void_p(dptr)))

    def set_x0_sensitivities(self, mode: int = 2):
        _lib.check(self.lib.ihm2mpc_set_x0_sensitivities(self._h, int(mode)))
        self._sens_mode = int(mode)

    def get_x0_sensitivities(self):
        full = self._sens_mode == 2
        sx = np.empty((self.B, self.N + 1, NX, NX)) if full else None
        su = np.empty((self.B, self.N, NU, NX)) if full else np.empty((self.B, NU, NX))
        _lib.check(self.lib.ihm2mpc_get_x0_sensitivities(self._h, _ptr(sx) if full else None, _ptr(su)))
        return sx, su

    def get_sens_u0_device(self, dptr: int):
        _lib.check(self.lib.ihm2mpc_get_sens_u0_device(self._h, C.c_void_p(dptr)))

    def eval_adjoint_sensitivities(self, seed_x=None, seed_u=None):
        return self._eval_adjoint(seed_x, seed_u, False)

    def _eval_adjoint(self, seed_x, seed_u, weights: bool):
        B, N = self.B, self.N
        given = seed_x if seed_x is not None else seed_u
        if given is None:
            S, squeeze = 2, False
        else:
            squeeze = np.ndim(given) == 3
            S = 1 if squeeze else int(np.shape(given)[1])
        sx = None if seed_x is None else _f64(np.asarray(seed_x, dtype=np.float64).reshape(B, S, N + 1, NX), (B, S, N + 1, NX), "seed_x")
        su = None if seed_u is None else _f64(np.asarray(seed_u, dtype=np.float64).reshape(B, S, N, NU), (B, S, N, NU), "seed_u")
        out = dict(x0=np.empty((B, S, NX)), yref=np.empty((B, S, N, NY)), yref_e=np.empty((B, S, NX)))
        if weights:
            out.update(W=np.empty((B, S, NY, NY)), W_e=np.empty((B, S, NX, NX)))
        fn = self.lib.ihm2mpc_eval_adjoint_sensitivities_w if weights else self.lib.ihm2mpc_eval_adjoint_sensitivities
        _lib.check(fn(self._h, S, None if sx is None else _ptr(sx), None if su is None else _ptr(su), *[_ptr(v) for v in out.values()]))
        return {k: v[:, 0] for k, v in out.items()} if squeeze else out

    def eval_adjoint_weight_sensitivities(self, seed_x=None, seed_u=None):
        return self._eval_adjoint(seed_x, seed_u, True)

    def du0_dW(self):
        out = dict(W=np.empty((self.B, 2, NY, NY)), W_e=np.empty((self.B, 2, NX, NX)))
        _lib.check(self.lib.ihm2mpc_eval_adjoint_sensitivities_w(self._h, 2, None, None, None, None, None, _ptr(out["W"]), _ptr(out["W_e"])))
        return out

    def du0_ds_target(self):
        g = self.eval_adjoint_sensitivities()
        ramp = np.arange(self.N) / self.N
        return g["yref"][:, :, :, 0] @ ramp + g["yref_e"][:, :, 0]

    def sim_step(self, x, u, model: int = 0, M_sim: int = 100):
        x = _f64(x, (self.B, NX), "x"); u = _f64(u, (self.B, NU), "u")
        out = np.empty((self.B, NX))
        _lib.check(self.lib.ihm2mpc_sim_step(self._h, int(model), int(M_sim), _ptr(x), _ptr(u), _ptr(out)))
        return out

    def set_track_geometry(self, X_ref, Y_ref, phi_ref):
        arrs = [_f64(np.atleast_2d(a), (self.ntracks, self.nknots), n) for a, n in ((X_ref, "X_ref"), (Y_ref, "Y_ref"), (phi_ref, "phi_ref"))]
        _lib.check(self.lib.ihm2mpc_set_track_geometry(self._h, *[_ptr(a) for a in arrs]))

    def sim_step_cart(self, x, u, model: int = -3, M_sim: int = 10, dt_sim: float = 0.01, n_steps: int = 5, v_dyn: float = 3.0):
        x = _f64(x, (self.B, NX), "x"); u = _f64(u, (self.B, NU), "u")
        out = np.empty((self.B, NX))
        _lib.check(self.lib.ihm2mpc_sim_step_cart(self._h, int(model), int(M_sim), float(dt_sim), int(n_steps), float(v_dyn), _ptr(x), _ptr(u), _ptr(out)))
        return out

    def project(self, x_cart, s_guess, s_tol: float = 2.0):
        xc = _f64(x_cart, (self.B, NX), "x_cart"); sg = _f64(s_guess, (self.B,), "s_guess").copy()
        out = np.empty((self.B, NX))
        _lib.check(self.lib.ihm2mpc_project(self._h, _ptr(xc), _ptr(sg), float(s_tol), _ptr(out)))
        return out, sg

    def set_cart_state(self, x_cart, s_guess):
        _lib.check(self.lib.ihm2mpc_set_cart_state(self._h, _ptr(_f64(x_cart, (self.B, NX), "x_cart")), _ptr(_f64(s_guess, (self.B,), "s_guess"))))

    def get_cart_state(self):
        xc = np.empty((self.B, NX)); sg = np.empty(self.B)
        _lib.check(self.lib.ihm2mpc_get_cart_state(self._h, _ptr(xc), _ptr(sg)))
        return xc, sg

    def sim_advance_cart(self, model: int = -3, M_sim: int = 10, dt_sim: float = 0.01, n_steps: int = 5, v_dyn: float = 3.0, s_tol: float = 2.0):
        _lib.check(self.lib.ihm2mpc_sim_advance_cart(self._h, int(model), int(M_sim), float(dt_sim), int(n_steps), float(v_dyn), float(s_tol)))

    def sim_advance(self, model: int = 0, M_sim: int = 100):
        _lib.check(self.lib.ihm2mpc_sim_advance(self._h, int(model), int(M_sim)))

    def alloc_pinned(self, shape):
        n = int(np.prod(shape))
        ptr = C.c_void_p()
        _lib.check(self.lib.ihm2mpc_host_alloc(C.c_uint64(n * 8), C.byref(ptr)))
        self._pinned = getattr(self, "_pinned", []) + [ptr]
        return np.ctypeslib.as_array(C.cast(ptr, _lib.c_double_p), shape=(n,)).reshape(shape)

    def get_u0_async(self, out):
        if out.shape != (self.B, NU) or out.dtype != np.float64 or not out.flags.c_contiguous:
            raise ValueError("out must be a C-contiguous float64 (B, 2) array from alloc_pinned")
        _lib.check(self.lib.ihm2mpc_get_u0_async(self._h, _ptr(out)))

    def set_lap_wrap(self, enable: bool = True):
        _lib.check(self.lib.ihm2mpc_set_lap_wrap(self._h, int(bool(enable))))

    def set_active(self, active=None):
        if active is None:
            _lib.check(self.lib.ihm2mpc_set_active(self._h, None))
        else:
            a = np.ascontiguousarray(active, dtype=np.int32)
            if a.shape != (self.B,):
                raise ValueError(f"active must have shape ({self.B},)")
            _lib.check(self.lib.ihm2mpc_set_active(self._h, a.ctypes.data_as(_lib.c_int32_p)))

    def step(self, s_target: float, model: int = 0, M_sim: int = 100):
        _lib.check(self.lib.ihm2mpc_step(self._h, int(model), int(M_sim), float(s_target)))

    def _set_stage(self, i, stage, field, value):
        v = _f64(np.ravel(value))
        _lib.check(self.lib.ihm2mpc_set_stage(self._h, i, stage, field.encode(), _ptr(v), v.size))

    def _get_stage(self, i, stage, field, n):
        out = np.empty(n)
        _lib.check(self.lib.ihm2mpc_get_stage(self._h, i, stage, field.encode(), _ptr(out), n))
        return out


class AcadosOcpSolver:

    def __init__(self, ocp: AcadosOcp, json_file: str | None = None, verbose: bool = False, *, s_ref=None, kappa_ref=None,
                 device: int = 0):
        n_half = ocp.dims.np // 2
        if s_ref is None:
            s_ref = np.arange(n_half, dtype=np.float64)
            kappa_ref = np.zeros(n_half)
        self.batch = BatchedOcpSolver(ocp, 1, s_ref, kappa_ref, device=device)
        self.i = 0
        self._owner = True

    @classmethod
    def _view(cls, batch: BatchedOcpSolver, i: int) -> "AcadosOcpSolver":
        self = cls.__new__(cls)
        self.batch, self.i, self._owner = batch, i, False
        return self
# ... 150 lines not shown
```

Measured before the change: 1.238 million.

## Add full-slot QP kernel specialization for all-hard two-sided N=40 tables

Adds a FULL template variant of the wave QP body, chosen when every slot lane carries a finite two-sided hard constraint (host-checked). It drops per-slot validity and finiteness branches, packs byte offsets and the CD row selector into s_kc so row dots and cf/gam accumulations use direct LDS addresses, and zeroes cf/gam once per solve instead of per pass, removing barriers. The cost is a new instantiation set, more host-side checks and reliance on static asserts that the factor sweep never overwrites cf/gam.

```diff
diff --git a/ihm2_amd/csrc/api.hip b/ihm2_amd/csrc/api.hip
--- a/ihm2_amd/csrc/api.hip
+++ b/ihm2_amd/csrc/api.hip
@@ -93,6 +93,7 @@
 {
     const int B = h->B;
     h->inst_b_ok = false;
+    h->slots_full = false;
     if (check_instance_pattern(h, h->ih_lb.data(), h->ih_ub.data())) return -1;
     const size_t n = h->slots.entries();
     if ((size_t)B * n > h->i_slot_lb.size()) {
@@ -106,10 +107,11 @@
     if (n && (upload_shared(h, slb.data(), h->i_slot_lb, slb.size()) || upload_shared(h, sub.data(), h->i_slot_ub, sub.size()))) return -1;
     if (upload_shared(h, stl.data(), h->i_st_lb, stl.size()) || upload_shared(h, stu.data(), h->i_st_ub, stu.size())) return -1;
     h->inst_b_ok = true;
-    return 0;
-}
-
-const QpTable qp_catalogue[] = {ihm2_qp_set0(), ihm2_qp_set1(), ihm2_qp_set2(), ihm2_qp_set3(), ihm2_qp_set4(), ihm2_qp_set5(), ihm2_qp_set6()};
+    h->slots_full = ihm2::slot_table_full(h->slots, 5) && ihm2::slot_bounds_full(h->slots, B, slb, sub);
+    return 0;
+}
+
+const QpTable qp_catalogue[] = {ihm2_qp_set0(), ihm2_qp_set1(), ihm2_qp_set2(), ihm2_qp_set3(), ihm2_qp_set4(), ihm2_qp_set5(), ihm2_qp_set6(), ihm2_qp_set7()};
 
 int path_class(const ihm2mpc_handle *h) { return h->rows.alat_on ? 2 : h->path_on ? 1 : 0; }
 
@@ -119,21 +121,32 @@
         for (const QpInst *e = t.inst; e < t.inst + t.n; e++) {
             const QpKey &k = e->key;
             if (k.kind == want.kind && k.nsoft == want.nsoft && k.path == want.path && k.uni == want.uni && k.sqp == want.sqp &&
-                k.irk == want.irk && k.dyn == want.dyn && k.sens == want.sens && k.nf == want.nf && k.nslot >= want.nslot)
+                k.irk == want.irk && k.dyn == want.dyn && k.sens == want.sens && k.nf == want.nf && k.full == want.full && k.nslot >= want.nslot)
                 return e;
         }
     return nullptr;
 }
 
+int qp_form_limit()
+{
+    static const int limit = [] { const char *e = getenv("IHM2MPC_QP_FORM"); return (e && e[0] == '0') ? 0 : (e && e[0] == '1') ? 1 : (e && e[0] == '2') ? 2 : 3; }();
+    return limit;
+}
 int factor_form(const ihm2mpc_handle *h)
 {
-    static const int limit = [] { const char *e = getenv("IHM2MPC_QP_FORM"); return (e && e[0] == '0') ? 0 : (e && e[0] == '1') ? 1 : 2; }();
+    const int limit = qp_form_limit();
     if (limit == 0 || h->cfg.model == IHM2MPC_MODEL_FDYN6 || h->slots.m_act == 0) return 0;
-    return (h->N == 40 && limit == 2) ? 40 : -1;
-}
+    return (h->N == 40 && limit >= 2) ? 40 : -1;
+}
+int slot_form(const ihm2mpc_handle *h) { return (qp_form_limit() == 3 && h->slots_full && factor_form(h) == 40) ? 1 : 0; }
 
 const QpInst *find_form(const ihm2mpc_handle *h, QpKey want)
 {
+    if (slot_form(h)) {
+        want.nf = 40; want.full = 1;
+        if (const QpInst *e = find_inst(want)) return e;
+        want.full = 0;
+    }
     for (int nf = factor_form(h); nf != 0; nf = (nf > 0) ? -1 : 0) {
         want.nf = nf;
         if (const QpInst *e = find_inst(want)) return e;
@@ -180,9 +193,9 @@
     const int form = (k.nf > 0) ? 2 : (k.nf < 0) ? 1 : 0;
     if (k.kind != QP_STEPS) {
         r[0] = k.kind; r[1] = k.nslot; r[2] = k.nsoft; r[3] = k.path; r[4] = k.uni;
-        r[15] = (r[15] & ~0x300) | (form << 8);
+        r[15] = (r[15] & ~0x700) | (form << 8) | ((k.full ? 1 : 0) << 10);
     } else {
-        r[15] = (r[15] & ~0x3000) | ((per_step ? 0 : form) << 12);
+        r[15] = (r[15] & ~0x7000) | ((per_step ? 0 : form) << 12) | ((!per_step && k.full ? 1 : 0) << 14);
         r[5] = per_step ? 2 : 1; r[6] = k.nslot; r[7] = k.nsoft; r[8] = k.path; r[9] = k.uni; r[10] = k.sqp; r[11] = k.irk; r[12] = k.dyn;
         r[13] = per_step; r[14] = k.sens;
     }
@@ -472,6 +485,7 @@
                   h->q_g, B * NS * 10, h->q_rg, B * NS * 10, h->q_P, B * NS * 64, h->q_M, (B * N + 2 * QM_PAD) * 64, h->scratch, B * 24))
         return -1;
     h->slots_fit = true;
+    h->slots_full = false;
     h->sqp_globalization = 0; h->sqp_use_suff = 0; h->sqp_full_step_dual = 0;
     h->sqp_alpha_min = 0.05; h->sqp_alpha_red = 0.7; h->sqp_eps = 1e-4;
     for (int i = 0; i < 4; i++) h->sqp_tol[i] = cfg->nlp_tol;
@@ -657,6 +671,7 @@
 {
     ihm2::SlotTable t = ihm2::lay_out_slots(h->rows, ihm2::slot_limits(path_class(h)));
     h->slots_fit = t.fit;
+    h->slots_full = false;
     if (!t.fit) return 0;
     h->slots = std::move(t);
     const ihm2::SlotTable &s = h->slots;
@@ -677,6 +692,7 @@
             return -1;
     }
     if (h->inst_b) return scatter_instance_bounds(h);
+    h->slots_full = ihm2::slot_table_full(s, 5);
     return 0;
 }
 
@@ -717,6 +733,7 @@
         h->i_lbu.reset(); h->i_ubu.reset(); h->i_lg.reset(); h->i_ug.reset();
         h->ih_lb = std::vector<double>(); h->ih_ub = std::vector<double>();
         h->inst_b = false; h->inst_b_ok = false;
+        h->slots_full = h->bounds_set && h->slots_fit && ihm2::slot_table_full(h->slots, 5);
         return 0;
     }
     if (!lbx || !ubx || !lbu || !ubu || !lg || !ug) return fail("lbx, ubx, lbu, ubu, lg, ug must all be given, or all be NULL (batch-shared bounds again)");
diff --git a/ihm2_amd/csrc/ihm2mpc_internal.h b/ihm2_amd/csrc/ihm2mpc_internal.h
--- a/ihm2_amd/csrc/ihm2mpc_internal.h
+++ b/ihm2_amd/csrc/ihm2mpc_internal.h
@@ -77,6 +77,7 @@
     DevBuf<double> lg, ug;
     ihm2::ConstraintRows rows;
     ihm2::SlotTable slots;
+    bool slots_full;
     bool slots_fit;
     DevBuf<int32_t> slot_kc;
     DevBuf<double> slot_lb, slot_ub;
@@ -253,7 +254,7 @@
 void ihm2_sens_args(const ihm2mpc_handle *h, void *out);
 
 enum { QP_WAVE = 1, QP_BLOCK = 2, QP_STEPS = 3 };
-struct QpKey { int kind, nslot, nsoft, path, uni, sqp, irk, dyn, sens, nf; };
+struct QpKey { int kind, nslot, nsoft, path, uni, sqp, irk, dyn, sens, nf, full; };
 struct QpInst { QpKey key; int threads; const void *kernel; };
 struct QpTable { const QpInst *inst; int n; };
-QpTable ihm2_qp_set0(), ihm2_qp_set1(), ihm2_qp_set2(), ihm2_qp_set3(), ihm2_qp_set4(), ihm2_qp_set5(), ihm2_qp_set6();
+QpTable ihm2_qp_set0(), ihm2_qp_set1(), ihm2_qp_set2(), ihm2_qp_set3(), ihm2_qp_set4(), ihm2_qp_set5(), ihm2_qp_set6(), ihm2_qp_set7();
diff --git a/ihm2_amd/csrc/kernels_qp.hip b/ihm2_amd/csrc/kernels_qp.hip
--- a/ihm2_amd/csrc/kernels_qp.hip
+++ b/ihm2_amd/csrc/kernels_qp.hip
@@ -24,6 +24,7 @@
 #define SWEEP_DL ((SWEEP_RING >= 8) ? 4 : 2)
 
 __device__ __forceinline__ bool fin(double v) { return fabs(v) < INF_BOUND; }
+__device__ __forceinline__ int here(int v) { asm volatile("" : "+v"(v)); return v; }
 
 template <typename OP>
 __device__ __forceinline__ double wave_reduce(double v, OP op)
@@ -112,10 +113,12 @@
     stream_rows<DIR, D, DL, false>(rows, N, e_even, e_odd, pre, body);
 }
 
-template <int NSLOT, int NSOFT, int PATH, int UNI, int NW = 1, int LEAN = 1, int NF = 0>
+template <int NSLOT, int NSOFT, int PATH, int UNI, int NW = 1, int LEAN = 1, int NF = 0, int FULL = 0>
 __device__ __forceinline__ void qp_wave_body(const QpArgs &a, const int b, double *sm, const bool want_res = true)
 {
     static_assert(NF == 0 || NW == 1, "the straight-line factor sweep parks its idle lanes' stores in the tile the block reductions use");
+    static_assert(FULL == 0 || (NSOFT == 0 && PATH == 0 && UNI != 0 && NW == 1 && LEAN != 0 && NF > 0 && NSLOT <= 8),
+                  "the full slot form is written for the all-hard table of the batch-shared rows, one wave, the lean phases and the compiled-in horizon");
     constexpr int NT = 64 * NW;
     const int tid = threadIdx.x, lane = tid & 63, wv = tid >> 6;
 #define BSYNC() do { if (NW == 1) WSYNC(); else __syncthreads(); } while (0)
@@ -131,6 +134,7 @@
     static_assert(qp_sweeps_inside(qp_lds(40, CLS), 40, LEAN != 0, SWEEP_RING, SWEEP_DL) && (LEAN == 0 || qp_sweeps_inside(qp_lds(2, CLS), 2, true, SWEEP_RING, SWEEP_DL)),
                   "the sweeps' unclamped LDS prefetch leaves the block (the earlier form does below N = 4: api.hip refuses those launches)");
     static_assert(NW <= 4, "qp_factor_inside checks the block reductions for four waves");
+    static_assert(FULL == 0 || qp_full_zeroes_kept(qp_lds(NF > 0 ? NF : 2, CLS), NF > 0 ? NF : 2), "a store of the factor sweep reaches gam or cf: the full slot form zeroes them once per solve");
 #define LEN(id) qp_lds_len(id, N, NS, CLS)
     double *z = sm, *gt = z + LEN(QP_Z), *pi = gt + LEN(QP_GT), *pv = pi + LEN(QP_PI), *rb = pv + LEN(QP_PV), *gam = rb + LEN(QP_RB), *cf = gam + LEN(QP_GAM), *dz = cf + LEN(QP_CF);
     double *kff = dz + LEN(QP_DZ), *Kl = kff + LEN(QP_KFF), *Ginv = Kl + LEN(QP_KL), *Prb = Ginv + LEN(QP_GINV), *tile = Prb + LEN(QP_PRB), *hc = tile + LEN(QP_TILE), *ha = hc + LEN(QP_HC);
@@ -268,9 +272,12 @@
     for (int r = 0; r < NSO; r++) { so_zw[r] = 0.0; so_Zw[r] = -1.0; so_s[r] = 1.0; so_ls[r] = 0.0; so_rs[r] = 0.0; so_ds[r] = so_dls[r] = so_pa[r] = 0.0; }
 #define IS_SOFT(r) ((r) < NSOFT && so_Zw[(r) < NSOFT ? (r) : 0] >= 0.0)
 #define ONE_SIDED(r) (NSOFT > 0 && PATH != 2 && (r) < NSOFT)
-#define HAS_L(r) (ONE_SIDED(r) ? true : fin(s_dl[r]))
-#define HAS_U(r) (ONE_SIDED(r) ? false : fin(s_du[r]))
-#define ROW_DOT(r, v) (ONE_SIDED(r) ? s_sg[(r) < NSOFT ? (r) : 0] * row_dot(s_kc[r], (v)) : row_dot(s_kc[r], (v)))
+#define HAS_L(r) (FULL ? true : ONE_SIDED(r) ? true : fin(s_dl[r]))
+#define HAS_U(r) (FULL ? true : ONE_SIDED(r) ? false : fin(s_du[r]))
+#define ROW_DOT(r, v) (FULL ? row_dot_full((r), (v)) : ONE_SIDED(r) ? s_sg[(r) < NSOFT ? (r) : 0] * row_dot(s_kc[r], (v)) : row_dot(s_kc[r], (v)))
+#define NO_SLOT(r) (!FULL && s_kc[r] < 0)
+#define SLOT_W(r) (FULL ? (s_kc[r] & 0xffff) >> 3 : s_kc[r])
+#define SLOT_AT(arr, r) (*(FULL ? reinterpret_cast<double *>(reinterpret_cast<char *>(arr) + (here(s_kc[r]) & 0xffff)) : &(arr)[s_kc[r]]))
 #define ROW_SIGN(r, c) (ONE_SIDED(r) ? s_sg[(r) < NSOFT ? (r) : 0] * (c) : (c))
     double s_sg[NSO];
 #pragma unroll
@@ -280,12 +287,13 @@
 #pragma unroll
     for (int r = 0; r < NSLOT; r++) {
         const int s = tid + NT * r;
-        s_kc[r] = -1; s_dl[r] = -INFINITY; s_du[r] = INFINITY;
+        s_kc[r] = FULL ? 0 : -1; s_dl[r] = -INFINITY; s_du[r] = INFINITY;
         lam_l[r] = lam_u[r] = 0.0; t_l[r] = t_u[r] = 1.0;
         const int kc = (s < a.nslots) ? a.slot_kc[s] : -1;
         if (kc >= 0) {
             const int k = kc >> 4, c = kc & 15;
             s_kc[r] = k * NCK + c;
+            if (FULL) s_kc[r] = ((k * NCK + c) * 8) | ((k * 10 + ((c < 10) ? c : 0)) << 19) | ((c >= 10) ? (int)(0x80000000u | ((unsigned)(c - 10) << 30)) : 0);
             double cz;
             if (c < 8) cz = xb[k * 8 + c];
             else if (c < 10) cz = ub[k * 2 + c - 8];
@@ -334,13 +342,24 @@
         for (int j = 0; j < 10; j++) acc = fma(CDV(k, c - 10, j), v[k * 10 + j], acc);
         return acc;
     };
+    auto row_dot_full = [&](int r, const double *v) -> double {
+        const int pk = here(s_kc[r]);
+        const double *vk = reinterpret_cast<const double *>(reinterpret_cast<const char *>(v) + ((pk >> 16) & 0x3fff));
+        if (pk >= 0) return vk[0];
+        const double *cd = CDl + (((unsigned)pk >> 30) & 1) * 10;
+        double acc = 0.0;
+#pragma unroll
+        for (int j = 0; j < 10; j++) acc = fma(cd[j], vk[j], acc);
+        return acc;
+    };
 
     for (int e = tid; e < NS * 10; e += NT) z[e] = (e < 8) ? a.x0[(size_t)b * 8 + e] - xb[e] : 0.0;
     for (int e = tid; e < NS * 8; e += NT) pi[e] = 0.0;
+    if (FULL) for (int e = tid; e < NS * NCK; e += NT) { cf[e] = 0.0; gam[e] = 0.0; }
     BSYNC();
 #pragma unroll
     for (int r = 0; r < NSLOT; r++) {
-        if (s_kc[r] < 0) continue;
+        if (NO_SLOT(r)) continue;
         const double rz = ROW_DOT(r, z);
         const bool al = HAS_L(r), au = HAS_U(r);
         double tau_c = a.tau0;
@@ -366,13 +385,15 @@
     for (it = 0;; it++) {
         bool exact = (it == 0) || exact_mode, finished = false;
         auto multipliers_to_cf = [&]() {
-            for (int e = tid; e < NS * NCK; e += NT) cf[e] = 0.0;
-            BSYNC();
+            if (!FULL) {
+                for (int e = tid; e < NS * NCK; e += NT) cf[e] = 0.0;
+                BSYNC();
+            }
 #pragma unroll
             for (int r = 0; r < NSLOT; r++) {
-                if (s_kc[r] < 0) continue;
+                if (NO_SLOT(r)) continue;
                 const bool al = HAS_L(r), au = HAS_U(r);
-                SLOT_ACC(cf[s_kc[r]], ROW_SIGN(r, (al ? lam_l[r] : 0.0) - (au ? lam_u[r] : 0.0)));
+                SLOT_ACC(SLOT_AT(cf, r), ROW_SIGN(r, (al ? lam_l[r] : 0.0) - (au ? lam_u[r] : 0.0)));
             }
             BSYNC();
         };
@@ -386,7 +407,7 @@
 #pragma unroll
         for (int r = 0; r < NSLOT; r++) {
             rd_l[r] = rd_u[r] = 0.0;
-            if (s_kc[r] < 0) continue;
+            if (NO_SLOT(r)) continue;
             const double rz = ROW_DOT(r, z);
             const bool al = HAS_L(r), au = HAS_U(r);
             const double sv = IS_SOFT(r) ? so_s[r < NSOFT ? r : 0] : 0.0;
@@ -401,7 +422,7 @@
                 res_gs = nanmax(res_gs, fabs(so_rs[q]));
                 mu_acc += so_ls[q] * so_s[q]; res_m = nanmax(res_m, fabs(so_ls[q] * so_s[q]));
             }
-            if (LEAN == 0) SLOT_ACC(cf[s_kc[r]], ROW_SIGN(r, (al ? lam_l[r] : 0.0) - (au ? lam_u[r] : 0.0)));
+            if (LEAN == 0) SLOT_ACC(SLOT_AT(cf, r), ROW_SIGN(r, (al ? lam_l[r] : 0.0) - (au ? lam_u[r] : 0.0)));
         }
         if constexpr (NW > 1) {
 #pragma unroll
@@ -476,12 +497,14 @@
         BSYNC();
         double alpha = 1.0, alpha_d = 1.0, sigma = 0.0;
         auto slot_coeffs = [&](int pass) {
-            for (int e = tid; e < NS * NCK; e += NT) { cf[e] = 0.0; if (pass == 0) gam[e] = 0.0; }
-            BSYNC();
+            if (!FULL) {
+                for (int e = tid; e < NS * NCK; e += NT) { cf[e] = 0.0; if (pass == 0) gam[e] = 0.0; }
+                BSYNC();
+            }
             const double mu_t = fmax(sigma * mu, mu_floor);
 #pragma unroll
             for (int r = 0; r < NSLOT; r++) {
-                if (s_kc[r] < 0) continue;
+                if (NO_SLOT(r)) continue;
                 const bool al = HAS_L(r), au = HAS_U(r);
                 double c = 0.0;
                 if (IS_SOFT(r)) {
@@ -489,22 +512,22 @@
                     const double lm = al ? lam_l[r] : lam_u[r], tt = al ? t_l[r] : t_u[r], rdv = al ? rd_l[r] : rd_u[r];
                     const double gm = lm / tt, gs = so_ls[q] / so_s[q], D = so_Zw[q] + gm + gs;
                     double c1, c2, rsv;
-                    if (pass == 0) { c1 = (lm * tt + lm * rdv) / tt; c2 = so_ls[q]; rsv = so_rs[q]; gam[s_kc[r]] += gm * (so_Zw[q] + gs) / D; }
+                    if (pass == 0) { c1 = (lm * tt + lm * rdv) / tt; c2 = so_ls[q]; rsv = so_rs[q]; SLOT_AT(gam, r) += gm * (so_Zw[q] + gs) / D; }
                     else { c1 = ((al ? pa_l[r] : pa_u[r]) - mu_t) / tt; c2 = (so_pa[q] - mu_t) / so_s[q]; rsv = 0.0; }
                     c = c1 - gm * (rsv + c1 + c2) / D;
-                    cf[s_kc[r]] += ONE_SIDED(r) ? ROW_SIGN(r, c) : (al ? c : -c);
+                    SLOT_AT(cf, r) += ONE_SIDED(r) ? ROW_SIGN(r, c) : (al ? c : -c);
                     continue;
                 }
                 if (pass == 0) {
                     const double gl = al ? lam_l[r] / t_l[r] : 0.0, gu = au ? lam_u[r] / t_u[r] : 0.0;
                     if (al) c += fma(gl, rd_l[r], lam_l[r]);
                     if (au) c -= fma(gu, rd_u[r], lam_u[r]);
-                    SLOT_ACC(gam[s_kc[r]], gl + gu);
+                    SLOT_ACC(SLOT_AT(gam, r), gl + gu);
                 } else {
                     if (al) c += (pa_l[r] - mu_t) / t_l[r];
                     if (au) c -= (pa_u[r] - mu_t) / t_u[r];
                 }
-                SLOT_ACC(cf[s_kc[r]], ROW_SIGN(r, c));
+                SLOT_ACC(SLOT_AT(cf, r), ROW_SIGN(r, c));
             }
             BSYNC();
         };
@@ -694,7 +717,7 @@
 #pragma unroll
             for (int r = 0; r < NSLOT; r++) {
                 dlam_l[r] = dlam_u[r] = dt_l[r] = dt_u[r] = 0.0;
-                if (s_kc[r] < 0) continue;
+                if (NO_SLOT(r)) continue;
                 const double drz = ROW_DOT(r, dz);
                 if (IS_SOFT(r)) {
                     const int q = r < NSOFT ? r : 0;
@@ -753,7 +776,7 @@
 #pragma unroll
                 for (int r = 0; r < NSLOT; r++) {
                     pa_l[r] = dlam_l[r] * dt_l[r]; pa_u[r] = dlam_u[r] * dt_u[r];
-                    if (s_kc[r] < 0) continue;
+                    if (NO_SLOT(r)) continue;
                     mu_aff = __dadd_rn(mu_aff, __dadd_rn(HAS_L(r) ? __dmul_rn(fma(amax_d, dlam_l[r], lam_l[r]), fma(amax, dt_l[r], t_l[r])) : 0.0,
                                                          HAS_U(r) ? __dmul_rn(fma(amax_d, dlam_u[r], lam_u[r]), fma(amax, dt_u[r], t_u[r])) : 0.0));
                     if (IS_SOFT(r)) {
@@ -822,7 +845,7 @@
         for (int e = tid; e < NS * 8; e += NT) pi[e] = fma(alpha_d, pv[e], pi[e]);
 #pragma unroll
         for (int r = 0; r < NSLOT; r++) {
-            if (s_kc[r] < 0) continue;
+            if (NO_SLOT(r)) continue;
             if (HAS_L(r)) { lam_l[r] = fma(alpha_d, dlam_l[r], lam_l[r]); t_l[r] = fma(alpha, dt_l[r], t_l[r]); }
             if (HAS_U(r)) { lam_u[r] = fma(alpha_d, dlam_u[r], lam_u[r]); t_u[r] = fma(alpha, dt_u[r], t_u[r]); }
             if (IS_SOFT(r)) { const int q = r < NSOFT ? r : 0; so_s[q] = fma(alpha, so_ds[q], so_s[q]); so_ls[q] = fma(alpha_d, so_dls[q], so_ls[q]); }
@@ -857,8 +880,8 @@
         __syncthreads();
 #pragma unroll
         for (int r = 0; r < NSLOT; r++) {
-            if (s_kc[r] < 0) continue;
-            const int k = s_kc[r] / NCK, c = s_kc[r] % NCK;
+            if (NO_SLOT(r)) continue;
+            const int k = SLOT_W(r) / NCK, c = SLOT_W(r) % NCK;
             if (ONE_SIDED(r)) {
                 const int up = (s_sg[r < NSOFT ? r : 0] < 0.0) ? 1 : 0;
                 if (ALAT && c == 14) { lamab[k * 2 + up] = lam_l[r]; if (IS_SOFT(r)) slkab[k * 2 + up] = so_s[r < NSOFT ? r : 0]; }
@@ -887,13 +910,13 @@
 
 #undef BSYNC
 
-template <int NSLOT, int NSOFT, int PATH, int UNI, int NF = 0>
+template <int NSLOT, int NSOFT, int PATH, int UNI, int NF = 0, int FULL = 0>
 __global__ __launch_bounds__(64) void k_qp_wave(QpArgs a)
 {
     extern __shared__ double sm[];
     if ((int)blockIdx.x >= a.B) return;
     if (NF > 0 && a.N != NF) return;
-    qp_wave_body<NSLOT, NSOFT, PATH, UNI, 1, 1, NF>(a, blockIdx.x, sm);
+    qp_wave_body<NSLOT, NSOFT, PATH, UNI, 1, 1, NF, FULL>(a, blockIdx.x, sm);
 }
 
 template <int NSLOT, int UNI, int NW>
@@ -960,7 +983,7 @@
     line_search_body<MODEL, ROLL>(ls, b, it, last);
 }
 
-template <int NSLOT, int NSOFT, int PATH, int UNI, int SQP, int IRK = 0, int DYN = 0, int SENS = 0, int NF = 0>
+template <int NSLOT, int NSOFT, int PATH, int UNI, int SQP, int IRK = 0, int DYN = 0, int SENS = 0, int NF = 0, int FULL = 0>
 __global__ __launch_bounds__(64) void k_steps(const StepArgs *sp, QpArgs a, const LsArgs *lsp)
 {
     static_assert(DYN == 0 || s_count(1) == QP_DYN_RK4_WORDS, "the dynamic models' RK4 integrator parks s_count(1) words per lane in the QP's LDS (qp_lds.hpp: steps_lds_doubles)");
@@ -1078,7 +1101,7 @@
                 dev_prepare(b, lane, N, s.s_target, 1, s.x0, a.x, a.u, s.yref, s.yref_e);
                 __syncthreads();
             }
-            qp_wave_body<NSLOT, NSOFT, PATH, UNI, 1, SQP ? 0 : 1, NF>(a, b, sm, SQP || step + 1 == s.n_steps);
+            qp_wave_body<NSLOT, NSOFT, PATH, UNI, 1, SQP ? 0 : 1, NF, FULL>(a, b, sm, SQP || step + 1 == s.n_steps);
             __syncthreads();
             if constexpr (SENS != 0) {
                 sens_body(*s.sens, b, sm, step);
@@ -1108,13 +1131,16 @@
 }
 
 #ifndef QP_SET
-#error "compile with -DQP_SET=0 (all-hard instantiations), -DQP_SET=1 (soft / track-row instantiations), -DQP_SET=2 (dynamic OCP models in the persistent loop), -DQP_SET=3 (the persistent loop with x0 sensitivities), -DQP_SET=4 (the benchmarked all-hard pair with the straight-line factor sweep), -DQP_SET=5 or -DQP_SET=6 (the all-hard RTI loops with the closed-form actuator lags: general form / straight-line factor sweep)"
+#error "compile with -DQP_SET=0 (all-hard instantiations), -DQP_SET=1 (soft / track-row instantiations), -DQP_SET=2 (dynamic OCP models in the persistent loop), -DQP_SET=3 (the persistent loop with x0 sensitivities), -DQP_SET=4 (the benchmarked all-hard pair with the straight-line factor sweep), -DQP_SET=5 or -DQP_SET=6 (the all-hard RTI loops with the closed-form actuator lags: general form / straight-line factor sweep), -DQP_SET=7 (the pair of set 4 at the horizon 40 with the full slot form)"
 #endif
 #define QP_INSTANCES_(n) QP_INSTANCES_##n
 #define QP_INSTANCES_OF(n) QP_INSTANCES_(n)
 #define QP_INSTANCES QP_INSTANCES_OF(QP_SET)
 
-#if QP_SET == 4 || QP_SET == 6
+#if QP_SET == 7
+#define WAVE(NS, NO, PT, UN) {{QP_WAVE, NS, NO, PT, UN, 0, 0, 0, 0, 40, 1}, 64, (const void *)k_qp_wave<NS, NO, PT, UN, 40, 1>},
+#define STEPS(NS, NO, PT, UN, IR, DY) {{QP_STEPS, NS, NO, PT, UN, 0, IR, DY, 0, 40, 1}, 64, (const void *)k_steps<NS, NO, PT, UN, 0, IR, DY, 0, 40, 1>},
+#elif QP_SET == 4 || QP_SET == 6
 #define WAVE(NS, NO, PT, UN)                                                                          \
     {{QP_WAVE, NS, NO, PT, UN, 0, 0, 0, 0, 40}, 64, (const void *)k_qp_wave<NS, NO, PT, UN, 40>},     \
     {{QP_WAVE, NS, NO, PT, UN, 0, 0, 0, 0, -1}, 64, (const void *)k_qp_wave<NS, NO, PT, UN, -1>},
diff --git a/ihm2_amd/csrc/qp_catalogue.hpp b/ihm2_amd/csrc/qp_catalogue.hpp
--- a/ihm2_amd/csrc/qp_catalogue.hpp
+++ b/ihm2_amd/csrc/qp_catalogue.hpp
@@ -32,6 +32,7 @@
 #define QP_INSTANCES_5(WAVE, BLOCK, STEPS)                                                                                                \
     STEPS(5, 0, 0, 0, 2, 0) STEPS(5, 0, 0, 1, 2, 0) STEPS(8, 0, 0, 0, 2, 0) STEPS(8, 0, 0, 1, 2, 0) STEPS(10, 0, 0, 1, 2, 0)
 #define QP_INSTANCES_6(WAVE, BLOCK, STEPS) STEPS(5, 0, 0, 1, 2, 0)
+#define QP_INSTANCES_7 QP_INSTANCES_4
 
 namespace ihm2 {
 
diff --git a/ihm2_amd/csrc/qp_lds.hpp b/ihm2_amd/csrc/qp_lds.hpp
--- a/ihm2_amd/csrc/qp_lds.hpp
+++ b/ihm2_amd/csrc/qp_lds.hpp
@@ -125,6 +125,13 @@
 }
 QP_LDS_FN QpReach qp_reach_plain_parking(const QpLds &l) { return {l.tile, l.tile + 63 + 4 + 1}; }
 QP_LDS_FN QpReach qp_reach_plain_operand(const QpLds &l, int N, int nck) { return {l.gt - 10, l.gam + N * nck}; }
+QP_LDS_FN QpReach qp_reach_plain_stores(const QpLds &l) { return {l.dz + 10, l.tile.end()}; }
+QP_LDS_FN QpReach qp_reach_plain_store_pv(const QpLds &l, int N) { return {l.pv + N * 8, l.pv + N * 8 + 8}; }
+QP_LDS_FN bool qp_full_zeroes_kept(const QpLds &l, int N)
+{
+    const QpReach s = qp_reach_plain_stores(l), p = qp_reach_plain_store_pv(l, N);
+    return s.lo >= l.cf.end() && qp_inside(s, l.cf.end(), l.total) && qp_inside(p, 0, l.gam) && l.cf == l.gam.end();
+}
 QP_LDS_FN QpReach qp_reach_block_reduce(const QpLds &l, int nw) { return {l.tile, l.tile + nw}; }
 
 QP_LDS_FN bool qp_sweeps_inside(const QpLds &l, int N, bool lean, int d, int dl)
diff --git a/ihm2_amd/csrc/qp_tables.hpp b/ihm2_amd/csrc/qp_tables.hpp
--- a/ihm2_amd/csrc/qp_tables.hpp
+++ b/ihm2_amd/csrc/qp_tables.hpp
@@ -195,6 +195,26 @@
     return t;
 }
 
+inline bool full_bound(double v) { return std::fabs(v) < 1e20; }
+inline bool slot_table_full(const SlotTable &t, int nslot)
+{
+    if (!t.fit || t.nsoft != 0 || t.per_lane != nslot || t.total != 64 * nslot || t.entries() != (size_t)64 * nslot) return false;
+    for (size_t e = 0; e < t.entries(); e++) {
+        const int kc = t.kc[e];
+        if (kc < 0 || (kc & 15) >= 12 || t.Zw[e] >= 0.0) return false;
+        if (!full_bound(t.lb[e]) || !full_bound(t.ub[e])) return false;
+    }
+    return true;
+}
+inline bool slot_bounds_full(const SlotTable &t, int B, const std::vector<double> &slb, const std::vector<double> &sub)
+{
+    const size_t n = (size_t)B * t.entries();
+    if (slb.size() != n || sub.size() != n) return false;
+    for (size_t i = 0; i < n; i++)
+        if (!full_bound(slb[i]) || !full_bound(sub[i])) return false;
+    return true;
+}
+
 
 struct PatternMismatch {
     bool found;
diff --git a/ihm2_amd/solver.py b/ihm2_amd/solver.py
--- a/ihm2_amd/solver.py
+++ b/ihm2_amd/solver.py
@@ -375,8 +375,10 @@
         lin = (None, "k_linearize", "k_linearize_dyn", "k_linearize_cols", "k_linearize_irk", "k_linearize_lag")[r[15] & 15]
         sim = (None, "k_sim_step_kin", "k_sim_step", "k_sim_irk", "k_sim_step_kin_lag")[(r[15] >> 4) & 15]
         forms = ("general", "plain", "plain_n40", None)
+        slots = ("general", "full")
         return {"qp": qp, "steps": steps, "steps_fallback": fallback, "linearize": lin, "sim": sim,
-                "qp_form": forms[(r[15] >> 8) & 3] if qp else None, "steps_form": forms[(r[15] >> 12) & 3] if r[5] == 1 else None}
+                "qp_form": forms[(r[15] >> 8) & 3] if qp else None, "steps_form": forms[(r[15] >> 12) & 3] if r[5] == 1 else None,
+                "qp_slots": slots[(r[15] >> 10) & 1] if qp else None, "steps_slots": slots[(r[15] >> 14) & 1] if r[5] == 1 else None}
 
     def set_x0_device(self, dptr: int):
         _lib.check(self.lib.ihm2mpc_set_x0_device(self._h, C.c_void_p(dptr)))
```

New measurement: 1.258 million (median of 6 runs). +1.6%, better.
